# OlegArenz/gmmvi

Measured on AMD Instinct MI355X. Metric: samples_components_per_sec, higher is better.
Workload: dtype f32; 1 GPU; ns: stm target D=20, K=100 components (100/GPU), 100 samples/component, N=10000 samples/iter, SAMTRON (Stein, fixed K, reuse ratio 0, KL trust regions, improvement-based stepsizes); K=100, D=20, N=10000, parallelism=component-shard x1

## Files before the change

### gmmvi_amd/_lib.py

```python
import ctypes as C
import os

_HERE = os.path.dirname(os.path.abspath(__file__))
LIB_PATH = os.environ.get("GMMVI_HIP_LIB", os.path.join(_HERE, "libgmmvi_hip.so"))

GAUSS, STUDENT_T = 0, 1
SELF_NORMALIZED, OWN_SAMPLES_ONLY, EXPLICIT_ESTIMATE = 1, 2, 4
MAX_DIM = 64
MORE_REGISTER_MAX_DIM = 21
MORE_BLOCKED_MIN_DIM, MORE_BLOCKED_MAX_DIM = 64, 128
MAX_DIM_BLOCKED = 512
MAX_DIM_DIAG = 131072
BLOCKED_ABOVE_DEFAULT = 50


_blocked_above = None


def _atoi(text):
    import re
    m = re.match(r"\s*([+-]?\d+)", text)
    return int(m.group(1)) if m else 0


# ... 34 lines not shown
    "gmmvi_gather_rows": (_i, [_p, _p, _p, _i, _i, _p]),
    "gmmvi_exp_f32": (_i, [_p, _p, _p, _sz]),
    "gmmvi_logaddexp_f32": (_i, [_p, _p, _p, _f, _p, _f, _sz]),
    "gmmvi_segment_lse_f32": (_i, [_p, _i, _p, _p, _p, _i, _p, _sz, _i]),
    "gmmvi_copy_2d_f32": (_i, [_p, _p, _sz, _p, _sz, _i, _i]),
    "gmmvi_copy_batch": (_i, [_p, _i, C.POINTER(_p), C.POINTER(_p), C.POINTER(_sz)]),
    "gmmvi_normalize_logw": (_i, [_p, _p, _i, _p]),
    "gmmvi_add_heuristic_argmax": (_i, [_p, _p, _p, _i, C.c_double, _p]),
    "gmmvi_unpack_gathered": (_i, [_p, _p, _i, _sz, _i, C.POINTER(_sz), C.POINTER(_p)]),
    "gmmvi_fill_strided_f32": (_i, [_p, _p, _sz, _sz, _f]),
    "gmmvi_remove_column_f32": (_i, [_p, _p, _i, _sz, _i, _i]),
    "gmmvi_add_scalar_i32": (_i, [_p, _p, _p, C.c_int32, _sz]),
    "gmmvi_event_create": (_i, [_p, C.POINTER(_p)]),
    "gmmvi_event_destroy": (_i, [_p, _p]),
    "gmmvi_event_record": (_i, [_p, _p]),
    "gmmvi_event_synchronize": (_i, [_p, _p]),
    "gmmvi_host_alloc": (_i, [_p, _sz, C.POINTER(_p)]),
    "gmmvi_vmm_reserve": (_i, [_p, _sz, C.POINTER(_p), C.POINTER(_sz)]),
    "gmmvi_vmm_grow": (_i, [_p, _p, _sz, _sz, _sz]),
    "gmmvi_vmm_release": (_i, [_p, _p, _sz, _sz, _sz]),
    "gmmvi_host_free": (_i, [_p, _p]),
    "gmmvi_download_async": (_i, [_p, _p, _p, _sz]),
    "gmmvi_event_elapsed_ms": (_i, [_p, _p, _p, C.POINTER(_f)]),
    "gmmvi_profile_enable": (_i, [_p, _i]),
    "gmmvi_profile_report": (_i, [_p, C.c_char_p, _sz]),
    "gmmvi_packed_stride": (_sz, [_i]),
    "gmmvi_pack_components": (_i, [_p, _i, _f, _i, _i, _p, _p, _p, _p]),
    "gmmvi_cholesky": (_i, [_p, _i, _i, _p, _p, _p]),
    "gmmvi_mixture_eval": (_i, [_p, _i, _f, _i, _i, _p, _p, _p, _i, _p, _p, _p]),
    "gmmvi_mixture_eval_dual": (_i, [_p, _i, _f, _i, _i, _p, _p, _p, _p, _i, _p, _p, _p, _p]),
    "gmmvi_target_planar": (_i, [_p, _i, _p, _i, _p, _f, _p, _i, _p, _p]),
    "gmmvi_target_logreg": (_i, [_p, _i, _i, _p, _f, _f, _p, _i, _p, _p]),
    "gmmvi_target_logreg_mb": (_i, [_p, _i, _i, _p, _i, _i, _u64, _u32, _f, _f, _p, _i, _p, _p]),
    "gmmvi_target_bnn": (_i, [_p, _i, _i, _i, _i, _p, _p, _u64, _u32, _i, _f, _f, _p, _i, _p, _p]),
    "gmmvi_bnn_predict": (_i, [_p, _i, _i, _i, _p, _i, _p, _i, _p]),
    "gmmvi_target_talos": (_i, [_p, _p, _p, _p, _i, _p, _p]),
    "gmmvi_talos_fk": (_i, [_p, _p, _p, _i, _p, _p]),
    "gmmvi_sample_components": (_i, [_p, _i, _i, _p, _p, _p, _i, _u64, _u64, _i, _p, _p, _p]),
    "gmmvi_philox_normals": (_i, [_p, _u64, _u64, _i, _i, _i, _p]),
    "gmmvi_philox_uniforms": (_i, [_p, _u64, _u64, _i, _i, _p]),
    "gmmvi_stein": (_i, [_p, _i, _i, _p, _p, _i, _p, _p, _p, _p, _p, _i, _i, _p, _p]),
    "gmmvi_more": (_i, [_p, _i, _i, _p, _p, _p, _i, _p, _p, _p, _p, _p, _i, _i, _p, _p, _p]),
    "gmmvi_more_blocked": (_i, [_p, _i, _i, _p, _p, _p, _i, _p, _p, _p, _p, _p, _i, _i, _p, _p, _p]),
    "gmmvi_update_components_kl": (_i, [_p, _i, _i, _p, _p, _p, _p, _p, _f, _f, _p, _p, _p, _p, _p, _p, _p]),
    "gmmvi_update_components_kl_reference": (_i, [_p, _i, _i, _p, _p, _p, _p, _p, _f, _f, _p, _p, _p, _p, _p, _p]),
    "gmmvi_update_components_direct": (_i, [_p, _i, _i, _p, _p, _p, _p, _p, _f, _p, _p, _p]),
    "gmmvi_update_components_iblr": (_i, [_p, _i, _i, _p, _p, _p, _p, _p, _f, _p, _p, _p]),
    "gmmvi_expected_log_ratios": (_i, [_p, _i, _i, _p, _p, _p, _p, _f, _p, _i, _p, _p, _p]),
    "gmmvi_update_weights_kl": (_i, [_p, _i, _p, _p, _p, _f, _p]),
    "gmmvi_update_weights_direct": (_i, [_p, _i, _p, _p, _p, _f]),
    "gmmvi_component_stepsize_improvement": (_i, [_p, _i, _p, _p, _p, _f, _f, _f, _f]),
    "gmmvi_weight_stepsize_improvement": (_i, [_p, _i, _p, _p, _p, _f, _f, _f, _f]),
    "gmmvi_train_iter_samtron": (_i, [_p, _p]),
    "gmmvi_sharded_scratch_floats": (_sz, [_i, _i, _i]),
    "gmmvi_train_iter_sharded_phase": (_i, [_p, _p, _i]),
    "gmmvi_comm_unique_id": (_i, [C.c_char_p]),
    "gmmvi_comm_init": (_i, [_p, C.c_char_p, _i, _i]),
    "gmmvi_comm_destroy": (_i, [_p]),
    "gmmvi_allgather_f32": (_i, [_p, _p, _p, _sz]),
    "gmmvi_allreduce_f32": (_i, [_p, _p, _sz, _i]),
    "gmmvi_combine_partials": (_i, [_p, _i, _i, _i, _p, _p, _p, _p]),
    "gmmvi_diag_packed_stride": (_sz, [_i]),
    "gmmvi_diag_pack": (_i, [_p, _i, _i, _p, _p, _p]),
    "gmmvi_diag_mixture_eval": (_i, [_p, _i, _i, _p, _p, _p, _p, _i, _p, _p, _p, _p]),
    "gmmvi_diag_sample": (_i, [_p, _i, _i, _p, _p, _p, _i, _u64, _u64, _i, _p, _p, _p]),
    "gmmvi_diag_stein": (_i, [_p, _i, _i, _p, _p, _i, _p, _p, _p, _p, _p, _i, _i, _p, _p]),
    "gmmvi_diag_embed": (_i, [_p, _i, _i, _p, _p]),
    "gmmvi_diag_extract": (_i, [_p, _i, _i, _p, _p]),
    "gmmvi_reciprocal_f32": (_i, [_p, _p, _sz, _p]),
    "gmmvi_update_components_diag_kl": (_i, [_p, _i, _i, _p, _p, _p, _p, _p, _f, _f, _p, _p, _p, _p, _p, _p]),
    "gmmvi_update_components_diag_iblr": (_i, [_p, _i, _i, _p, _p, _p, _p, _p, _f, _p, _p, _p]),
    "gmmvi_mmd_scratch_doubles": (_sz, [_i, _i]),
    "gmmvi_mmd_pair_sum": (_i, [_p, _p, _i, _p, _i, _i, _p, _p, _p]),
}

EXPORTED_SYMBOLS = tuple(_PROTOS.keys())


def load():
    global _lib
    if _lib is not None:
        return _lib
    if not os.path.exists(LIB_PATH):
        raise GmmviError(
            f"{LIB_PATH} not found: build it with `make -C gmmvi_amd/csrc` (or __graft_entry__.build()). "
            "There is no CPU fallback for the gmmvi hot path.")
    lib = C.CDLL(LIB_PATH, mode=C.RTLD_GLOBAL)
    for name, (res, args) in _PROTOS.items():
        fn = getattr(lib, name)
        fn.restype = res
        fn.argtypes = args
    _lib = lib
    return lib


def device_count():
    return int(load().gmmvi_device_count())


def check(ctx_handle, rc):
    if rc != 0:
        msg = load().gmmvi_last_error(ctx_handle)
        raise GmmviError(f"libgmmvi_hip error {rc}: {msg.decode() if msg else '?'}")
```

### gmmvi_amd/csrc/api.hip

```cpp
#include "common.h"
#include <cstring>
#include "blocked.h"

std::string g_gmmvi_global_err;

int gmmvi_ws_reserve(gmmvi_ctx* ctx, size_t nbytes) {
    ++ctx->ws_epoch;
    if (nbytes <= ctx->ws_bytes) return GMMVI_OK;
    GMMVI_HIP_CHECK(ctx, hipStreamSynchronize(ctx->stream));
    if (ctx->ws) GMMVI_HIP_CHECK(ctx, hipFree(ctx->ws));
    ctx->ws = nullptr;
    ctx->ws_bytes = 0;
    size_t want = nbytes + nbytes / 2;
    GMMVI_HIP_CHECK(ctx, hipMalloc(&ctx->ws, want));
    ctx->ws_bytes = want;
    return GMMVI_OK;
}

extern "C" {

int gmmvi_device_count(void) {
    int n = 0;
    if (hipGetDeviceCount(&n) != hipSuccess) return 0;
    return n;
}

int gmmvi_ctx_create(gmmvi_ctx** out, int device) {
    if (!out) return gmmvi_fail(nullptr, GMMVI_ERR_ARG, "gmmvi_ctx_create: out is NULL");
    *out = nullptr;
    int n = 0;
    hipError_t e = hipGetDeviceCount(&n);
    if (e != hipSuccess || n == 0)
        return gmmvi_fail(nullptr, GMMVI_ERR_HIP, std::string("no HIP device: ") + hipGetErrorString(e));
    if (device < 0 || device >= n) return gmmvi_fail(nullptr, GMMVI_ERR_ARG, "device index out of range");
    gmmvi_ctx* ctx = new gmmvi_ctx();
    ctx->device = device;
    e = hipSetDevice(device);
    if (e == hipSuccess) e = hipStreamCreateWithFlags(&ctx->stream, hipStreamNonBlocking);
    if (e != hipSuccess) {
        g_gmmvi_global_err = std::string("gmmvi_ctx_create: ") + hipGetErrorString(e);
        delete ctx;
        return GMMVI_ERR_HIP;
    }
    hipDeviceProp_t prop;
    if (hipGetDeviceProperties(&prop, device) == hipSuccess) ctx->num_cus = prop.multiProcessorCount;
    *out = ctx;
    return GMMVI_OK;
}

void gmmvi_ctx_destroy(gmmvi_ctx* ctx) {
    if (!ctx) return;
    gmmvi_comm_destroy(ctx);
    if (ctx->stream) {
        (void)hipStreamSynchronize(ctx->stream);
        (void)hipStreamDestroy(ctx->stream);
    }
    if (ctx->ws) (void)hipFree(ctx->ws);
    if (ctx->arena) (void)hipFree(ctx->arena);
    if (ctx->bimg) (void)hipFree(ctx->bimg);
    if (ctx->up_ring) {
        for (int i = 0; i < gmmvi_ctx::UP_SLOTS; ++i) (void)hipEventDestroy(ctx->up_event[i]);
        (void)hipHostFree(ctx->up_ring);
    }
    if (ctx->defer_ws) (void)hipFree(ctx->defer_ws);
    delete ctx;
}

const char* gmmvi_last_error(gmmvi_ctx* ctx) { return ctx ? ctx->err.c_str() : g_gmmvi_global_err.c_str(); }

int gmmvi_sync(gmmvi_ctx* ctx) {
    GMMVI_HIP_CHECK(ctx, hipStreamSynchronize(ctx->stream));
    return GMMVI_OK;
}

int gmmvi_malloc(gmmvi_ctx* ctx, size_t nbytes, void** out_dev) {
    GMMVI_ARG_CHECK(ctx, out_dev != nullptr);
    *out_dev = nullptr;
    if (nbytes == 0) nbytes = 4;
    GMMVI_HIP_CHECK(ctx, hipSetDevice(ctx->device));
    GMMVI_HIP_CHECK(ctx, hipMalloc(out_dev, nbytes));
    return GMMVI_OK;
}

int gmmvi_free(gmmvi_ctx* ctx, void* dev) {
    if (!dev) return GMMVI_OK;
    GMMVI_HIP_CHECK(ctx, hipFree(dev));
    return GMMVI_OK;
}

int gmmvi_upload(gmmvi_ctx* ctx, void* dst_dev, const void* src_host, size_t nbytes) {
    if (nbytes == 0) return GMMVI_OK;
    GMMVI_ARG_CHECK(ctx, dst_dev && src_host);
    if (nbytes <= gmmvi_ctx::UP_SLOT_BYTES) {
        if (ctx->up_ring == nullptr) {
            GMMVI_HIP_CHECK(ctx, hipHostMalloc((void**)&ctx->up_ring, gmmvi_ctx::UP_SLOTS * gmmvi_ctx::UP_SLOT_BYTES, hipHostMallocDefault));
            for (int i = 0; i < gmmvi_ctx::UP_SLOTS; ++i)
                GMMVI_HIP_CHECK(ctx, hipEventCreateWithFlags(&ctx->up_event[i], hipEventDisableTiming));
        }
        const int slot = ctx->up_next;
        ctx->up_next = (slot + 1) % gmmvi_ctx::UP_SLOTS;
        if (ctx->up_used[slot]) GMMVI_HIP_CHECK(ctx, hipEventSynchronize(ctx->up_event[slot]));
        unsigned char* stage = ctx->up_ring + (size_t)slot * gmmvi_ctx::UP_SLOT_BYTES;
        memcpy(stage, src_host, nbytes);
        GMMVI_HIP_CHECK(ctx, hipMemcpyAsync(dst_dev, stage, nbytes, hipMemcpyHostToDevice, ctx->stream));
        GMMVI_HIP_CHECK(ctx, hipEventRecord(ctx->up_event[slot], ctx->stream));
        ctx->up_used[slot] = true;
        return GMMVI_OK;
    }
    GMMVI_HIP_CHECK(ctx, hipMemcpyAsync(dst_dev, src_host, nbytes, hipMemcpyHostToDevice, ctx->stream));
    GMMVI_HIP_CHECK(ctx, hipStreamSynchronize(ctx->stream));
    return GMMVI_OK;
}

int gmmvi_download(gmmvi_ctx* ctx, void* dst_host, const void* src_dev, size_t nbytes) {
    if (nbytes == 0) return GMMVI_OK;
    GMMVI_ARG_CHECK(ctx, dst_host && src_dev);
    GMMVI_HIP_CHECK(ctx, hipMemcpyAsync(dst_host, src_dev, nbytes, hipMemcpyDeviceToHost, ctx->stream));
// ... 458 lines not shown
```

### gmmvi_amd/csrc/combine.h

```cpp
#pragma once
#include "common.h"

template <int R>
__device__ __forceinline__ float combine_log_values_n(const float* __restrict__ parts, int N, int n) {
    float v[R];
#pragma unroll
    for (int r = 0; r < R; ++r) v[r] = parts[(size_t)r * N + n];
    float m = -3.0e38f;
#pragma unroll
    for (int r = 0; r < R; ++r) m = fmaxf(m, v[r]);
    float s = 0.f;
#pragma unroll
    for (int r = 0; r < R; ++r) s += __expf(v[r] - m);
    return m + __logf(s);
}

__device__ __forceinline__ float combine_log_values(const float* __restrict__ parts, int R, int N, int n) {
    switch (R) {
        case 2: return combine_log_values_n<2>(parts, N, n);
        case 3: return combine_log_values_n<3>(parts, N, n);
        case 4: return combine_log_values_n<4>(parts, N, n);
        case 5: return combine_log_values_n<5>(parts, N, n);
        case 6: return combine_log_values_n<6>(parts, N, n);
        case 7: return combine_log_values_n<7>(parts, N, n);
// ... 39 lines not shown
            for (int r = 0; r < R; ++r) g = fmaf(__expf(lv[r] - lp), gv[r], g);
        } else {
            for (int r = 0; r < Rr; ++r)
                g = fmaf(__expf(j.lp_parts[(size_t)r * ps + n] - lp), j.grad_parts[(size_t)r * gs + (size_t)n * j.D + i], g);
        }
        j.grad_out[(size_t)n * j.D + i] = g;
    }
}

__device__ __forceinline__ void combine_element(const CombineJob& j, long e) {
    switch (j.R) {
        case 2: combine_element_n<2>(j, e); break;
        case 3: combine_element_n<3>(j, e); break;
        case 4: combine_element_n<4>(j, e); break;
        case 5: combine_element_n<5>(j, e); break;
        case 6: combine_element_n<6>(j, e); break;
        case 7: combine_element_n<7>(j, e); break;
        case 8: combine_element_n<8>(j, e); break;
        case 10: combine_element_n<10>(j, e); break;
        case 12: combine_element_n<12>(j, e); break;
        case 16: combine_element_n<16>(j, e); break;
        default: combine_element_n<0>(j, e); break;
    }
}

template <int R>
__device__ __forceinline__ void combine_carried_n(const CombineJob& j) {
    const bool with_grad = j.grad_out != nullptr && j.grad_parts != nullptr;
    const long elems = (long)j.N * (with_grad ? j.D : 1);
    const long stride = (long)j.blocks * blockDim.x;
    for (long e = (long)((int)blockIdx.x - j.first_block) * blockDim.x + threadIdx.x; e < elems; e += stride)
        combine_element_n<R>(j, e);
}

__device__ __forceinline__ bool combine_carried(const CombineJob& j) {
    if (j.blocks == 0 || (int)blockIdx.x < j.first_block) return false;
    if (blockIdx.y == 0 && blockIdx.z == 0) {
        switch (j.R) {
            case 2: combine_carried_n<2>(j); break;
            case 3: combine_carried_n<3>(j); break;
            case 4: combine_carried_n<4>(j); break;
            case 5: combine_carried_n<5>(j); break;
            case 6: combine_carried_n<6>(j); break;
            case 7: combine_carried_n<7>(j); break;
            case 8: combine_carried_n<8>(j); break;
            case 10: combine_carried_n<10>(j); break;
            case 12: combine_carried_n<12>(j); break;
            case 16: combine_carried_n<16>(j); break;
            default: combine_carried_n<0>(j); break;
        }
    }
    return true;
}
```

### gmmvi_amd/csrc/comm.hip

```cpp
#include "common.h"
#include "combine.h"
#include <rccl/rccl.h>

#define GMMVI_NCCL_CHECK(ctx, call)                                                                        \
    do {                                                                                                   \
        ncclResult_t r__ = (call);                                                                         \
        if (r__ != ncclSuccess)                                                                            \
            return gmmvi_fail(ctx, GMMVI_ERR_RCCL, std::string(#call) + ": " + ncclGetErrorString(r__));   \
    } while (0)

__global__ __launch_bounds__(256) void combine_partials_kernel(CombineJob j) {
    combine_element(j, (long)blockIdx.x * blockDim.x + threadIdx.x);
}

int gmmvi_combine_partials_internal(gmmvi_ctx* ctx, int R, int N, int D, const float* lp_parts_dev,
                                    const float* grad_parts_dev, float* lp_out_dev, float* grad_out_dev,
                                    const float* lp2_parts_dev, float* lp2_out_dev, long part_stride) {
    GMMVI_ARG_CHECK(ctx, R >= 1 && N >= 0 && D >= 1 && lp_parts_dev && part_stride >= 0);
    if (N == 0) return GMMVI_OK;
    CombineJob j;
    j.R = R; j.N = N; j.D = D; j.part_stride = part_stride;
    j.lp_parts = lp_parts_dev; j.grad_parts = grad_parts_dev; j.lp2_parts = lp2_parts_dev;
    j.lp_out = lp_out_dev; j.grad_out = grad_out_dev; j.lp2_out = lp2_parts_dev ? lp2_out_dev : nullptr;
    const long elems = (long)N * ((grad_out_dev && grad_parts_dev) ? D : 1);
    hipLaunchKernelGGL(combine_partials_kernel, dim3((unsigned)((elems + 255) / 256)), dim3(256), 0, ctx->stream, j);
    GMMVI_LAUNCH_CHECK(ctx);
    return GMMVI_OK;
}

int gmmvi_defer_reserve(gmmvi_ctx* ctx, size_t nbytes) {
    if (ctx->pending.R > 0) return gmmvi_fail(ctx, GMMVI_ERR_ARG, "gmmvi_defer_reserve: a merge is still pending");
    if (nbytes <= ctx->defer_bytes) return GMMVI_OK;
    GMMVI_HIP_CHECK(ctx, hipStreamSynchronize(ctx->stream));
    if (ctx->defer_ws) GMMVI_HIP_CHECK(ctx, hipFree(ctx->defer_ws));
    ctx->defer_ws = nullptr;
    ctx->defer_bytes = 0;
    const size_t want = nbytes + nbytes / 2;
    GMMVI_HIP_CHECK(ctx, hipMalloc(&ctx->defer_ws, want));
    ctx->defer_bytes = want;
    return GMMVI_OK;
}

int gmmvi_flush_pending_combine(gmmvi_ctx* ctx) {
    if (ctx->pending.R == 0) return GMMVI_OK;
    const CombineJob j = ctx->pending;
    ctx->pending = CombineJob();
    GMMVI_PROF(ctx, "mixture_combine");
    return gmmvi_combine_partials_internal(ctx, j.R, j.N, j.D, j.lp_parts, j.grad_parts, j.lp_out, j.grad_out, j.lp2_parts,
                                           j.lp2_out);
}

CombineJob gmmvi_take_pending_combine(gmmvi_ctx* ctx, int threads, int first_block, bool light) {
    CombineJob j = ctx->pending;
    ctx->pending = CombineJob();
    if (j.R == 0) return j;
    const long elems = (long)j.N * ((j.grad_out && j.grad_parts) ? j.D : 1);
    long blocks;
    if (light) {
        blocks = (elems + 2L * threads - 1) / (2L * threads);
        if (blocks > 16L * ctx->num_cus) blocks = 16L * ctx->num_cus;
    } else {
        blocks = ctx->num_cus - first_block % ctx->num_cus;
        if (blocks < ctx->num_cus / 4) blocks += ctx->num_cus;
        const long useful = (elems + threads - 1) / threads;
        if (blocks > useful) blocks = useful;
    }
    if (blocks < 1) blocks = 1;
    j.first_block = first_block;
    j.blocks = (int)blocks;
    return j;
}

extern "C" {

int gmmvi_comm_unique_id(char* out_id_128) {
    if (!out_id_128) return gmmvi_fail(nullptr, GMMVI_ERR_ARG, "gmmvi_comm_unique_id: NULL buffer");
    static_assert(sizeof(ncclUniqueId) == 128, "ncclUniqueId is expected to be 128 bytes");
    ncclUniqueId id;
    ncclResult_t r = ncclGetUniqueId(&id);
    if (r != ncclSuccess) return gmmvi_fail(nullptr, GMMVI_ERR_RCCL, std::string("ncclGetUniqueId: ") + ncclGetErrorString(r));
    memcpy(out_id_128, &id, 128);
    return GMMVI_OK;
}

int gmmvi_comm_init(gmmvi_ctx* ctx, const char* unique_id_128, int n_ranks, int rank) {
    GMMVI_ARG_CHECK(ctx, unique_id_128 && n_ranks >= 1 && rank >= 0 && rank < n_ranks);
    if (ctx->comm) return gmmvi_fail(ctx, GMMVI_ERR_STATE, "communicator already initialised");
    ncclUniqueId id;
    memcpy(&id, unique_id_128, 128);
    GMMVI_HIP_CHECK(ctx, hipSetDevice(ctx->device));
    ncclComm_t comm;
    GMMVI_NCCL_CHECK(ctx, ncclCommInitRank(&comm, n_ranks, id, rank));
    ctx->comm = (void*)comm;
    ctx->n_ranks = n_ranks;
    ctx->rank = rank;
    return GMMVI_OK;
}

int gmmvi_comm_destroy(gmmvi_ctx* ctx) {
    if (ctx && ctx->comm) {
        (void)hipStreamSynchronize(ctx->stream);
        ncclCommDestroy((ncclComm_t)ctx->comm);
        ctx->comm = nullptr;
        ctx->n_ranks = 1;
        ctx->rank = 0;
    }
    return GMMVI_OK;
}

int gmmvi_allgather_f32(gmmvi_ctx* ctx, const float* send_dev, float* recv_dev, size_t count_per_rank) {
    GMMVI_ARG_CHECK(ctx, send_dev && recv_dev);
    if (ctx->n_ranks == 1 || !ctx->comm) {
        if (send_dev != recv_dev)
            GMMVI_HIP_CHECK(ctx, hipMemcpyAsync(recv_dev, send_dev, count_per_rank * sizeof(float),
                                                hipMemcpyDeviceToDevice, ctx->stream));
        return GMMVI_OK;
    }
    GMMVI_NCCL_CHECK(ctx, ncclAllGather(send_dev, recv_dev, count_per_rank, ncclFloat, (ncclComm_t)ctx->comm,
                                        ctx->stream));
    return GMMVI_OK;
}

int gmmvi_allreduce_f32(gmmvi_ctx* ctx, float* buf_dev, size_t count, int op) {
    GMMVI_ARG_CHECK(ctx, buf_dev && (op == 0 || op == 1));
    if (ctx->n_ranks == 1 || !ctx->comm) return GMMVI_OK;
    GMMVI_NCCL_CHECK(ctx, ncclAllReduce(buf_dev, buf_dev, count, ncclFloat, op == 0 ? ncclSum : ncclMax,
// ... 12 lines not shown
```

### gmmvi_amd/csrc/common.h

```cpp
#pragma once
#include <hip/hip_runtime.h>
#include <cstdio>
#include <cstring>
#include <cstdint>
#include <string>
#include <vector>
#include "../../include/gmmvi_hip.h"
#include "iter_prep.h"

struct CombineJob {
    int R = 0, N = 0, D = 0;
    long part_stride = 0;
    int first_block = 0, blocks = 0;
    const float* lp_parts = nullptr;
    const float* grad_parts = nullptr;
    const float* lp2_parts = nullptr;
    float* lp_out = nullptr;
    float* grad_out = nullptr;
    float* lp2_out = nullptr;
};

struct SampleJob {
    int K = 0, D = 0, uniform_count = 0;
    const float* means = nullptr; const float* chols = nullptr; const int32_t* offsets = nullptr;
    unsigned long long seed = 0, first_index = 0;
    float* X = nullptr; int32_t* mapping = nullptr; int32_t mapping_base = 0;
};

struct Riders {
    int first_block = 0;
    int prep_blocks = 0;
    int sample_blocks = 0;
    PrepArgs prep;
    SampleJob sample;
};

inline size_t riders_lds_bytes(const Riders& r) {
    return r.sample_blocks > 0 ? ((size_t)r.sample.D * r.sample.D + r.sample.D + 256 * (size_t)(r.sample.D | 1)) * sizeof(float) : 0;
}

struct gmmvi_ctx {
    int device = 0;
    hipStream_t stream = nullptr;
    std::string err;
    void* ws = nullptr;
    size_t ws_bytes = 0;
    uint64_t ws_epoch = 0;
    void* arena = nullptr;
    size_t arena_bytes = 0;
    static constexpr int UP_SLOTS = 64;
    static constexpr size_t UP_SLOT_BYTES = 64 * 1024;
    unsigned char* up_ring = nullptr;
    hipEvent_t up_event[UP_SLOTS] = {};
    bool up_used[UP_SLOTS] = {};
    int up_next = 0;
    void* bimg = nullptr;
    size_t bimg_bytes = 0;
    bool defer_combine = false;
    CombineJob pending;
    Riders riders;
    void* defer_ws = nullptr;
    size_t defer_bytes = 0;
    void* comm = nullptr;
    int n_ranks = 1, rank = 0;
    int num_cus = 256;
    unsigned func_attr_done = 0;
    bool prof = false;
    const char* prof_tag = nullptr;
    struct ProfRec { const char* name; hipEvent_t start, stop; double units; };
    std::vector<ProfRec> prof_recs;
};

struct GmmviProfScope {
    gmmvi_ctx* ctx; hipEvent_t stop = nullptr;
    GmmviProfScope(gmmvi_ctx* c, const char* name, double units = 0.0) : ctx(c) {
        if (!c->prof) return;
        hipEvent_t start;
        if (hipEventCreate(&start) != hipSuccess || hipEventCreate(&stop) != hipSuccess) { stop = nullptr; return; }
        (void)hipEventRecord(start, c->stream);
        c->prof_recs.push_back({name, start, stop, units});
    }
    ~GmmviProfScope() { if (stop) (void)hipEventRecord(stop, ctx->stream); }
};
#define GMMVI_PROF(ctx, name) GmmviProfScope prof_scope__(ctx, name)
#define GMMVI_PROF_UNITS(ctx, name, units) GmmviProfScope prof_scope__(ctx, name, units)

extern std::string g_gmmvi_global_err;

inline int gmmvi_fail(gmmvi_ctx* ctx, int code, const std::string& msg) {
    if (ctx) ctx->err = msg; else g_gmmvi_global_err = msg;
    return code;
}

#define GMMVI_HIP_CHECK(ctx, call)                                                                    \
    do {                                                                                              \
        hipError_t e__ = (call);                                                                      \
        if (e__ != hipSuccess)                                                                        \
            return gmmvi_fail(ctx, GMMVI_ERR_HIP,                                                     \
                              std::string(#call) + ": " + hipGetErrorString(e__) + " (" + __FILE__ +  \
                                  ":" + std::to_string(__LINE__) + ")");                              \
    } while (0)

#define GMMVI_ARG_CHECK(ctx, cond)                                                                    \
    do {                                                                                              \
        if (!(cond))                                                                                  \
            return gmmvi_fail(ctx, GMMVI_ERR_ARG, std::string("invalid argument: ") + #cond + " (" +  \
                                                      __FILE__ + ":" + std::to_string(__LINE__) + ")"); \
    } while (0)

#define GMMVI_LAUNCH_CHECK(ctx) GMMVI_HIP_CHECK(ctx, hipGetLastError())

int gmmvi_ws_reserve(gmmvi_ctx* ctx, size_t nbytes);
int gmmvi_pack_register_layout(gmmvi_ctx* ctx, int K, int D, const float* means_dev, const float* chols_dev, float* packed_dev);
int gmmvi_sample_components_bounded(gmmvi_ctx* ctx, int K, int D, const float* means_dev, const float* chols_dev,
                                    const int32_t* offsets_dev, int N, int max_per_component, uint64_t seed,
                                    uint64_t first_index, int stream_id, const float* eps_dev, float* X_out_dev,
                                    int32_t* mapping_out_dev);
int gmmvi_sample_components_prep(gmmvi_ctx* ctx, int K, int D, const float* means_dev, const float* chols_dev,
                                 const int32_t* offsets_dev, int N, int max_per_component, uint64_t seed, uint64_t first_index,
                                 float* X_out_dev, int32_t* mapping_out_dev, int32_t mapping_base, const PrepArgs& prep);
int gmmvi_combine_partials_internal(gmmvi_ctx* ctx, int R, int N, int D, const float* lp_parts_dev,
                                    const float* grad_parts_dev, float* lp_out_dev, float* grad_out_dev,
                                    const float* lp2_parts_dev, float* lp2_out_dev, long part_stride = 0);
int gmmvi_defer_reserve(gmmvi_ctx* ctx, size_t nbytes);
int gmmvi_flush_pending_combine(gmmvi_ctx* ctx);
CombineJob gmmvi_take_pending_combine(gmmvi_ctx* ctx, int threads, int first_block, bool light = false);
Riders gmmvi_take_pending_riders(gmmvi_ctx* ctx, int first_block, int threads, bool prep_only = false);
int gmmvi_flush_pending_riders(gmmvi_ctx* ctx);
struct SteinSlab;
int gmmvi_stein_partials(gmmvi_ctx* ctx, int K, int D, const float* packed_dev, const float* X_dev, int N, const float* ld_dev,
                         const float* qgrad_dev, const float* bg_dev, const float* tgrad_dev, int flags, SteinSlab* slab);
int gmmvi_stein_finalize_slab(gmmvi_ctx* ctx, int K, int D, const SteinSlab& slab, int N, int flags, const float* packed_dev,
                              float* H_neg_out_dev, float* g_neg_out_dev);
int gmmvi_update_components_kl_from_slab(gmmvi_ctx* ctx, int K, int D, const SteinSlab& slab, int N, int stein_flags,
                                         const float* packed_old_dev, float* H_neg_dev, float* g_neg_dev, float* means_dev,
                                         float* chols_dev, const float* stepsizes_dev, float temperature, float l2_init,
                                         float* last_eta_dev, float* l2_dev, float* num_received_updates_dev,
                                         int32_t* success_out_dev, float* packed_out_dev);
int gmmvi_update_weights_internal(gmmvi_ctx* ctx, int mode, int K, float* logw_dev, const float* E_dev,
                                  const float* stepsize_dev, float beta, float* kl_eta_out_dev, float* exp_out_dev);

inline int gmmvi_padded_dim(int D) {
    static const int dps[] = {2, 4, 8, 10, 12, 16, 20, 24, 32, 40, 50, 64};
    for (int dp : dps) if (D <= dp) return dp;
    return -1;
}

#define GMMVI_DISPATCH_DP(DPVAL, ...)                  \
    switch (DPVAL) {                                   \
        case 2:  { constexpr int DP = 2;  __VA_ARGS__; } break;  \
        case 4:  { constexpr int DP = 4;  __VA_ARGS__; } break;  \
        case 8:  { constexpr int DP = 8;  __VA_ARGS__; } break;  \
        case 10: { constexpr int DP = 10; __VA_ARGS__; } break;  \
        case 12: { constexpr int DP = 12; __VA_ARGS__; } break;  \
        case 16: { constexpr int DP = 16; __VA_ARGS__; } break;  \
        case 20: { constexpr int DP = 20; __VA_ARGS__; } break;  \
        case 24: { constexpr int DP = 24; __VA_ARGS__; } break;  \
        case 32: { constexpr int DP = 32; __VA_ARGS__; } break;  \
        case 40: { constexpr int DP = 40; __VA_ARGS__; } break;  \
        case 50: { constexpr int DP = 50; __VA_ARGS__; } break;  \
        case 64: { constexpr int DP = 64; __VA_ARGS__; } break;  \
        default: return gmmvi_fail(ctx, GMMVI_ERR_ARG, "unsupported dimension (D must be <= 64)"); \
    }

#ifndef GMMVI_MFMA_DENSITY_FROM_DP
#define GMMVI_MFMA_DENSITY_FROM_DP 32
#endif

template <int DP>
struct Pack {
    static constexpr int T = DP * (DP - 1) / 2;
    static constexpr int MU = 0;
    static constexpr int RD = DP;
    static constexpr int LROW = 2 * DP;
    static constexpr int LCOL = 2 * DP + T;
    static constexpr int CONST = 2 * DP + 2 * T;
    static constexpr bool FRAGS = DP >= GMMVI_MFMA_DENSITY_FROM_DP;
    static constexpr int MT = (DP + 15) / 16;
    static constexpr int KS = (DP + 3) / 4;
    __host__ __device__ static constexpr int nf(int mt) { return 4 * mt + 4 < KS ? 4 * mt + 4 : KS; }
    __host__ __device__ static constexpr int nbk(int mt) { return KS - 4 * mt > 0 ? KS - 4 * mt : 0; }
    __host__ __device__ static constexpr int fwd_base(int mt) { int a = 0; for (int m = 0; m < mt; ++m) a += nf(m); return a; }
    __host__ __device__ static constexpr int bwd_base(int mt) { int a = 0; for (int m = 0; m < mt; ++m) a += nbk(m); return a; }
    __host__ __device__ static constexpr int fwd_index(int mt, int s) { return fwd_base(mt) + s; }
// ... 74 lines not shown
```

### gmmvi_amd/csrc/density.hip

```cpp
#include "common.h"
#include "combine.h"
#include "riders.h"
#include "subst.h"
#include "subst_phased.h"
#include "subst_pk.h"
#include "blocked.h"
#include <cmath>
#include <cstdlib>

template <int DP>
__global__ __launch_bounds__(64) void pack_kernel(int family, float nu, int K, int D, const float* __restrict__ means,
                                                  const float* __restrict__ chols, float* __restrict__ packed,
                                                  float* __restrict__ inv_chols) {
    using P = Pack<DP>;
    const int k = blockIdx.x;
    const int t = threadIdx.x;
    const float* L = chols + (size_t)k * D * D;
    float* out = packed + (size_t)k * P::STRIDE;
    for (int i = t; i < DP; i += 64) {
        out[P::MU + i] = i < D ? means[(size_t)k * D + i] : 0.f;
        out[P::RD + i] = i < D ? 1.f / L[i * D + i] : 1.f;
    }
    for (int e = t; e < DP * DP; e += 64) {
        int i = e / DP, j = e % DP;
// ... 22 lines not shown
#pragma unroll
        for (int i = 0; i < DP; ++i) {
            float sacc = (i == t) ? 1.f : 0.f;
            if (i < D && t < D) {
                for (int j = 0; j < i; ++j) sacc -= L[i * D + j] * x[j];
                x[i] = sacc / L[i * D + i];
            } else {
                x[i] = 0.f;
            }
        }
        if (t < DP) {
#pragma unroll
            for (int i = 0; i < DP; ++i) Li[i * DP + t] = (i >= t) ? x[i] : 0.f;
        }
    }
    __syncthreads();
    if (P::FRAGS) gmmvi_write_inverse_fragments(out, DP, D, Li, DP, t, 64);
    if (inv_chols != nullptr) {
        float* inv = inv_chols + (size_t)k * D * D;
        for (int e = t; e < D * D; e += 64) inv[e] = Li[(e / D) * DP + (e % D)];
    }
}

__global__ __launch_bounds__(64) void cholesky_kernel(int D, const float* __restrict__ covs, float* __restrict__ chols,
                                                      int32_t* __restrict__ ok) {
    extern __shared__ float sm[];
    const int k = blockIdx.x, t = threadIdx.x;
    const int ld = D + 1;
    for (int e = t; e < D * D; e += 64) sm[(e / D) * ld + (e % D)] = covs[(size_t)k * D * D + e];
    __syncthreads();
    bool good = true;
    for (int j = 0; j < D; ++j) {
        float s = 0.f;
        if (t >= j && t < D) {
            s = sm[t * ld + j];
            for (int c = 0; c < j; ++c) s -= sm[t * ld + c] * sm[j * ld + c];
        }
        float p = __shfl(s, j);
        if (!(p > 0.f)) { good = false; break; }
        float d = sqrtf(p);
        __syncthreads();
        if (t == j) sm[t * ld + j] = d;
        else if (t > j && t < D) sm[t * ld + j] = s / d;
        __syncthreads();
    }
    for (int e = t; e < D * D; e += 64) {
        int i = e / D, j = e % D;
        float v = (j <= i) ? sm[i * ld + j] : 0.f;
        chols[(size_t)k * D * D + e] = good ? v : __builtin_nanf("");
    }
    if (t == 0 && ok) ok[k] = good ? 1 : 0;
}

typedef float me_f32x4 __attribute__((ext_vector_type(4)));
#define ME_LDS_BARRIER()                                       \
    do {                                                       \
        asm volatile("s_waitcnt lgkmcnt(0)" ::: "memory");     \
        __builtin_amdgcn_s_barrier();                          \
        asm volatile("" ::: "memory");                         \
    } while (0)
__host__ __device__ constexpr int me_rem_rows(int dp) { return (dp % 16 != 0 && dp % 16 <= 4 && dp > 16) ? dp % 16 : 0; }
template <int R>
__device__ __forceinline__ float me_row_bcast(float v) {
    return __int_as_float(__builtin_amdgcn_update_dpp(0, __float_as_int(v), 0x150 + R, 0xf, 0xf, false));
}
template <int N, int I = 0, class F>
__device__ __forceinline__ void me_static_rows(F&& f) {
    if constexpr (I < N) {
        f(std::integral_constant<int, I>{});
        me_static_rows<N, I + 1>(f);
    }
}
#ifndef GMMVI_ME_THREADS
#define GMMVI_ME_THREADS 1024
#define GMMVI_ME_MINW 1
#endif
#ifndef GMMVI_ME_WIDE_DP
#define GMMVI_ME_WIDE_DP 40
#endif
#ifdef GMMVI_ME_STAMPS
__device__ long long g_me_wg[2 * 8192];
__device__ unsigned long long g_me_hw[8192];
extern "C" int gmmvi_debug_wg_times(long long* out, int n) {
    return hipMemcpyFromSymbol(out, HIP_SYMBOL(g_me_wg), sizeof(long long) * (size_t)n) == hipSuccess ? 0 : -1;
}
extern "C" int gmmvi_debug_wg_hw(unsigned long long* out, int n) {
    return hipMemcpyFromSymbol(out, HIP_SYMBOL(g_me_hw), sizeof(unsigned long long) * (size_t)n) == hipSuccess ? 0 : -1;
}
__device__ long long g_me_ph[1024 * 16 * 16];
extern "C" int gmmvi_debug_wg_phases(long long* out, int n) {
    return hipMemcpyFromSymbol(out, HIP_SYMBOL(g_me_ph), sizeof(long long) * (size_t)n) == hipSuccess ? 0 : -1;
}
#endif
template <int DP, int FAMILY, bool GRAD>
__global__ __launch_bounds__(DP >= GMMVI_ME_WIDE_DP ? 512 : GMMVI_ME_THREADS, GMMVI_ME_MINW) void mixture_eval_kernel(float nu, int K_total, int D, const float* __restrict__ packed,
                                                            const float* __restrict__ logw, const float* __restrict__ X,
                                                            int N, float* __restrict__ ld_out, float* __restrict__ lp_out,
                                                            float* __restrict__ grad_out, const float* __restrict__ logw2,
                                                            float* __restrict__ lp2_out, CombineJob carried, Riders riders) {
    using PK = Pack<DP>;
    extern __shared__ __align__(16) float sm[];
    if (combine_carried(carried) || riders_carried<DP>(riders, sm)) return;
    const int kchunk = (K_total + gridDim.y - 1) / gridDim.y;
    const int k_lo = blockIdx.y * kchunk;
    const int K = min(K_total, k_lo + kchunk);
    if (gridDim.y > 1) {
        if (lp_out) lp_out += (size_t)blockIdx.y * N;
        if (lp2_out) lp2_out += (size_t)blockIdx.y * N;
        if (GRAD && grad_out) grad_out += (size_t)blockIdx.y * N * D;
    }
    const int lane = threadIdx.x & 63;
    const int wave = __builtin_amdgcn_readfirstlane(threadIdx.x >> 6);
    const int nwaves = blockDim.x >> 6;
    const int n0 = blockIdx.x * 64;
    const int n_here = min(64, N - n0);
    const int n = n0 + lane;
    const bool valid = lane < n_here;
    float* sm_merge = sm;
#ifdef GMMVI_ME_STAMPS
    if (threadIdx.x == 0) {
        g_me_wg[2 * (blockIdx.y * gridDim.x + blockIdx.x)] = wall_clock64();
        unsigned hw, xcc;
        asm volatile("s_getreg_b32 %0, hwreg(HW_REG_HW_ID)" : "=s"(hw));
        asm volatile("s_getreg_b32 %0, hwreg(HW_REG_XCC_ID)" : "=s"(xcc));
        g_me_hw[blockIdx.y * gridDim.x + blockIdx.x] = ((unsigned long long)xcc << 32) | hw;
    }
    unsigned long long stamp[16];
    int nstamp = 0, nbackward = 0;
    const long long wc0 = wall_clock64();
#define ME_STAMP() do { asm volatile("s_waitcnt lgkmcnt(0)" ::: "memory"); if (nstamp < 16) stamp[nstamp++] = __builtin_amdgcn_s_memtime(); } while (0)
    ME_STAMP();
#else
#define ME_STAMP()
#endif

    const int ldx = D | 1;
    float x[DP];
    if (DP % 4 == 0 && D == DP && (reinterpret_cast<uintptr_t>(X) & 15) == 0) {
        const float4* xrow = reinterpret_cast<const float4*>(X + (size_t)min(n, N - 1) * D);
#pragma unroll
        for (int q4 = 0; q4 < DP / 4; ++q4) {
            const float4 v4 = xrow[q4];
            x[4 * q4] = v4.x; x[4 * q4 + 1] = v4.y; x[4 * q4 + 2] = v4.z; x[4 * q4 + 3] = v4.w;
        }
        if (!valid) {
#pragma unroll
            for (int i = 0; i < DP; ++i) x[i] = 0.f;
        }
    } else if (DP % 2 == 0 && D == DP && (reinterpret_cast<uintptr_t>(X) & 7) == 0) {
        const float2* xrow = reinterpret_cast<const float2*>(X + (size_t)min(n, N - 1) * D);
#pragma unroll
        for (int q2 = 0; q2 < DP / 2; ++q2) {
            const float2 v2 = xrow[q2];
            x[2 * q2] = v2.x; x[2 * q2 + 1] = v2.y;
        }
        if (!valid) {
#pragma unroll
            for (int i = 0; i < DP; ++i) x[i] = 0.f;
        }
    } else {
        for (int e = threadIdx.x; e < n_here * D; e += blockDim.x) sm_merge[(e / D) * ldx + (e % D)] = X[(size_t)n0 * D + e];
        __syncthreads();
#pragma unroll
        for (int i = 0; i < DP; ++i) x[i] = (valid && i < D) ? sm_merge[lane * ldx + i] : 0.f;
        __syncthreads();
    }

    float m = -3.0e38f, s = 0.f;
    float m2 = -3.0e38f, s2 = 0.f;
    const bool dual = logw2 != nullptr;
    float acc[GRAD ? DP : 1];
    if (GRAD) {
#pragma unroll
        for (int i = 0; i < DP; ++i) acc[i] = 0.f;
    }
    const float nud = nu + (float)D;
    ME_STAMP();

    for (int k = k_lo + wave; k < K; k += nwaves) {
        ME_STAMP();
        const sp_block_ptr blk = sp_block(packed + (size_t)k * PK::STRIDE);
        const float lw = ((sp_const_f32)(uintptr_t)logw)[k];
        const float lw2 = dual ? ((sp_const_f32)(uintptr_t)logw2)[k] : 0.f;
        float z[DP], vrd[DP], q, cst;
        float pc[2][32];
        SpPass<DP>::forward(blk, x, z, vrd, q, cst, pc);
        sp_block_ptr blkb = blk;
        asm volatile("" : "+s"(blkb));
        if constexpr (GRAD) SpPass<DP>::backward_prefetch(blkb, pc);
        float ld, coef;
        if (FAMILY == GMMVI_GAUSS) {
            ld = fmaf(-0.5f, q, cst);
            coef = -1.f;
        } else {
            ld = cst - 0.5f * nud * log1pf(q / nu);
            coef = -nud / (nu + q);
        }
        const float a = ld + lw;
        const float mn = fmaxf(m, a);
        const float sc = __expf(m - mn);
        const float e = __expf(a - mn);
        s = fmaf(s, sc, e);
        m = mn;
        if (dual) {
            const float a2 = ld + lw2;
            const float mn2 = fmaxf(m2, a2);
            s2 = fmaf(s2, __expf(m2 - mn2), __expf(a2 - mn2));
            m2 = mn2;
        }
        if constexpr (GRAD) {
            SpPass<DP>::backward(blkb, z, vrd, pc);
            const float ec = e * coef;
#pragma unroll
            for (int i = 0; i < DP; ++i) acc[i] = fmaf(acc[i], sc, ec * z[i]);
            sp_pin<DP>(acc);
        }
        if (ld_out != nullptr && valid) ld_out[(size_t)k * N + n] = ld;
    }
    ME_STAMP();
    if (lp_out == nullptr && !GRAD) return;

    constexpr int NQ = (DP + 3) / 4;
    float* sm_m = sm_merge;
    float* sm_s = sm_merge + nwaves * 64;
    me_f32x4* sm_acc = reinterpret_cast<me_f32x4*>(sm_merge + 2 * nwaves * 64);
    float* outt = sm_merge + 2 * nwaves * 64 + (GRAD ? (size_t)nwaves * NQ * 256 : 0);
    float* sm_m2 = outt + (GRAD ? 64 * ldx : 0);
    float* sm_s2 = sm_m2 + nwaves * 64;
    sm_m[wave * 64 + lane] = m;
    if (dual) sm_m2[wave * 64 + lane] = m2;
    ME_LDS_BARRIER();
    ME_STAMP();
    float M = -3.0e38f, M2 = -3.0e38f;
    for (int w = 0; w < nwaves; ++w) M = fmaxf(M, sm_m[w * 64 + lane]);
    const float f = __expf(m - M);
    sm_s[wave * 64 + lane] = s * f;
    if (dual) {
        for (int w = 0; w < nwaves; ++w) M2 = fmaxf(M2, sm_m2[w * 64 + lane]);
        sm_s2[wave * 64 + lane] = s2 * __expf(m2 - M2);
    }
    if (GRAD) {
#pragma unroll
        for (int q4 = 0; q4 < NQ; ++q4) {
            me_f32x4 v4;
#pragma unroll
            for (int c = 0; c < 4; ++c) v4[c] = 4 * q4 + c < DP ? acc[4 * q4 + c] * f : 0.f;
            sm_acc[(wave * NQ + q4) * 64 + lane] = v4;
        }
    }
    ME_STAMP();
    ME_LDS_BARRIER();
    ME_STAMP();
    float S = 0.f;
    for (int w = 0; w < nwaves; ++w) S += sm_s[w * 64 + lane];
    if (wave == 0 && valid && lp_out != nullptr) lp_out[n] = M + __logf(S);
    if (dual && wave == (nwaves > 1 ? 1 : 0) && valid && lp2_out != nullptr) {
        float S2 = 0.f;
        for (int w = 0; w < nwaves; ++w) S2 += sm_s2[w * 64 + lane];
        lp2_out[n] = M2 + __logf(S2);
    }
    if (GRAD && grad_out != nullptr) {
        const float inv = 1.f / S;
        for (int q4 = wave; q4 < NQ; q4 += nwaves) {
            me_f32x4 g4 = {0.f, 0.f, 0.f, 0.f};
            for (int w = 0; w < nwaves; ++w) g4 += sm_acc[(w * NQ + q4) * 64 + lane];
#pragma unroll
            for (int c = 0; c < 4; ++c)
                if (4 * q4 + c < D) outt[lane * ldx + 4 * q4 + c] = g4[c] * inv;
        }
        ME_STAMP();
        ME_LDS_BARRIER();
        ME_STAMP();
        for (int e = threadIdx.x; e < n_here * D; e += blockDim.x)
            grad_out[(size_t)n0 * D + e] = outt[(e / D) * ldx + (e % D)];
    }
#ifdef GMMVI_ME_STAMPS
    ME_STAMP();
    if (threadIdx.x == 0) g_me_wg[2 * (blockIdx.y * gridDim.x + blockIdx.x) + 1] = wall_clock64();
    if (GRAD && logw2 && blockIdx.x == 60 && blockIdx.y == 1 && threadIdx.x == 64 * 3 && (g_me_wg[2 * 8192 - 1]++ & 15) == 12) {
        const long long wc1 = wall_clock64();
        printf("me stamps (shader cycles; kernel %lld x 10 ns by the 100 MHz clock):", wc1 - wc0);
        for (int i = 1; i < nstamp; ++i) printf(" %llu", stamp[i] - stamp[i - 1]);
        printf("  total %llu, backward passes %d\n", stamp[nstamp - 1] - stamp[0], nbackward);
    }
#endif
}

template <int DP, int FAMILY, bool GRAD>
__global__ __launch_bounds__(DP > 24 ? 512 : 1024) void mixture_eval_pk_kernel(float nu, int K_total, int D, const float* __restrict__ packed,
                                                               const float* __restrict__ logw, const float* __restrict__ X, int N,
                                                               float* __restrict__ ld_out, float* __restrict__ lp_out,
                                                               float* __restrict__ grad_out, const float* __restrict__ logw2,
                                                               float* __restrict__ lp2_out, CombineJob carried, Riders riders) {
    using PK = Pack<DP>;
    static_assert(DP % 2 == 0, "padded dimensions are even");
    constexpr int NP2 = DP / 2;
    extern __shared__ __align__(16) float sm[];
    if (combine_carried(carried) || riders_carried<DP>(riders, sm)) return;
    const int kchunk = (K_total + gridDim.y - 1) / gridDim.y;
    const int k_lo = blockIdx.y * kchunk;
    const int K = min(K_total, k_lo + kchunk);
    if (gridDim.y > 1) {
        if (lp_out) lp_out += (size_t)blockIdx.y * N;
        if (lp2_out) lp2_out += (size_t)blockIdx.y * N;
        if (GRAD && grad_out) grad_out += (size_t)blockIdx.y * N * D;
    }
    const int lane = threadIdx.x & 63;
    const int wave = __builtin_amdgcn_readfirstlane(threadIdx.x >> 6);
    const int nwaves = blockDim.x >> 6;
    const int n0 = blockIdx.x * 128;
    const int nA = n0 + lane, nB = n0 + 64 + lane;
    const bool validA = nA < N, validB = nB < N;
#ifdef GMMVI_ME_STAMPS
    const int wg_lin = blockIdx.y * gridDim.x + blockIdx.x;
    if (threadIdx.x == 0 && wg_lin < 8192) {
        g_me_wg[2 * wg_lin] = wall_clock64();
        unsigned hw, xcc;
        asm volatile("s_getreg_b32 %0, hwreg(HW_REG_HW_ID)" : "=s"(hw));
        asm volatile("s_getreg_b32 %0, hwreg(HW_REG_XCC_ID)" : "=s"(xcc));
        g_me_hw[wg_lin] = ((unsigned long long)xcc << 32) | hw;
    }
    int pk_ns = 0;
#define PK_STAMP() do { if (lane == 0 && wg_lin < 1024 && pk_ns < 16) g_me_ph[(wg_lin * 16 + wave) * 16 + pk_ns] = wall_clock64(); ++pk_ns; } while (0)
    PK_STAMP();
#else
#define PK_STAMP()
#endif

    me_f32x4* xs4 = reinterpret_cast<me_f32x4*>(sm);
    {
        const int n_here = min(128, N - n0);
        for (int e = threadIdx.x; e < 128 * DP; e += blockDim.x) {
            const int sl = e / DP, i = e - sl * DP;
            const float v = (sl < n_here && i < D) ? X[(size_t)(n0 + sl) * D + i] : 0.f;
            sm[(((i >> 1) * 64) + (sl & 63)) * 4 + ((i & 1) << 1) + (sl >> 6)] = v;
        }
    }
    float* sm_merge = sm + NP2 * 64 * 4;
    ME_LDS_BARRIER();
    PK_STAMP();

    pk_f32x2 mld = pk_splat(-3.0e38f), s = pk_splat(0.f), mld2 = pk_splat(-3.0e38f), s2 = pk_splat(0.f);
    const bool dual = logw2 != nullptr;
    pk_f32x2 acc[GRAD ? DP : 1];
    if (GRAD) {
#pragma unroll
// ... 69 lines not shown
    sm_max[wave * 64 + lane] = mld;
    if (dual) sm_max[(nwaves + wave) * 64 + lane] = mld2;
    ME_LDS_BARRIER();
    PK_STAMP();
    pk_f32x2 M = mld, M2 = mld2;
    for (int wv = 0; wv < nwaves; ++wv) {
        const pk_f32x2 o = sm_max[wv * 64 + lane];
        M = pk_f32x2{fmaxf(M.x, o.x), fmaxf(M.y, o.y)};
    }
    if (dual) {
        for (int wv = 0; wv < nwaves; ++wv) {
            const pk_f32x2 o = sm_max[(nwaves + wv) * 64 + lane];
            M2 = pk_f32x2{fmaxf(M2.x, o.x), fmaxf(M2.y, o.y)};
        }
        s2 = s2 * pk_f32x2{__expf(mld2.x - M2.x), __expf(mld2.y - M2.y)};
    }
    {
        const pk_f32x2 f = pk_f32x2{__expf(mld.x - M.x), __expf(mld.y - M.y)};
        s = s * f;
        if (GRAD) {
#pragma unroll
            for (int i = 0; i < DP; ++i) acc[i] = acc[i] * f;
        }
    }
#pragma unroll
    for (int half = 8; half >= 1; half >>= 1) {
        if (half < nwaves) {
            const bool writer = wave >= half && wave < 2 * half;
            const bool reader = wave < half && wave + half < nwaves;
            const int slot_w = half == half0 ? wave - half : wave;
            const int slot_r = half == half0 ? wave : wave + half;
            if (writer) {
                pk_f32x2* dst = slots + (size_t)slot_w * NV * 64 + lane;
                dst[0] = s;
                dst[64] = s2;
                if (GRAD) {
#pragma unroll
                    for (int i = 0; i < DP; ++i) dst[(2 + i) * 64] = acc[i];
                }
            }
            ME_LDS_BARRIER();
            if (reader) {
                const pk_f32x2* src = slots + (size_t)slot_r * NV * 64 + lane;
                s = s + src[0];
                s2 = s2 + src[64];
                if (GRAD) {
#pragma unroll
                    for (int i = 0; i < DP; ++i) acc[i] = acc[i] + src[(2 + i) * 64];
                }
            }
        }
    }
    PK_STAMP();
    if (wave != 0) return;
    if (lp_out != nullptr) {
        if (validA) lp_out[nA] = M.x + __logf(s.x);
        if (validB) lp_out[nB] = M.y + __logf(s.y);
    }
    if (dual && lp2_out != nullptr) {
        if (validA) lp2_out[nA] = M2.x + __logf(s2.x);
        if (validB) lp2_out[nB] = M2.y + __logf(s2.y);
    }
    if (GRAD && grad_out != nullptr) {
        const pk_f32x2 inv = pk_f32x2{1.f / s.x, 1.f / s.y};
#pragma unroll
        for (int i = 0; i < DP; ++i) acc[i] = acc[i] * inv;
        if (D == DP && DP % 4 == 0 && (reinterpret_cast<uintptr_t>(grad_out) & 15) == 0) {
#pragma unroll
            for (int q4 = 0; q4 < DP / 4; ++q4) {
                if (validA) reinterpret_cast<float4*>(grad_out + (size_t)nA * D)[q4] =
                    make_float4(acc[4 * q4].x, acc[4 * q4 + 1].x, acc[4 * q4 + 2].x, acc[4 * q4 + 3].x);
                if (validB) reinterpret_cast<float4*>(grad_out + (size_t)nB * D)[q4] =
                    make_float4(acc[4 * q4].y, acc[4 * q4 + 1].y, acc[4 * q4 + 2].y, acc[4 * q4 + 3].y);
            }
        } else {
#pragma unroll
            for (int i = 0; i < DP; ++i) {
                if (i < D) {
                    if (validA) grad_out[(size_t)nA * D + i] = acc[i].x;
                    if (validB) grad_out[(size_t)nB * D + i] = acc[i].y;
                }
            }
        }
    }
    PK_STAMP();
#ifdef GMMVI_ME_STAMPS
    if (threadIdx.x == 0 && wg_lin < 8192) g_me_wg[2 * wg_lin + 1] = wall_clock64();
#endif
#undef PK_STAMP
}


#define ME_WAVE_LDS_SYNC()                                     \
    do {                                                       \
        asm volatile("s_waitcnt lgkmcnt(0)" ::: "memory");     \
        __builtin_amdgcn_wave_barrier();                       \
    } while (0)

template <int DP, int FAMILY, bool GRAD, int NTS>
__global__ __launch_bounds__(512) void mixture_eval_mfma_kernel(float nu, int K_total, int D, const float* __restrict__ packed,
                                                                const float* __restrict__ logw, const float* __restrict__ X,
                                                                int N, float* __restrict__ ld_out, float* __restrict__ lp_out,
                                                                float* __restrict__ grad_out, const float* __restrict__ logw2,
                                                                float* __restrict__ lp2_out, CombineJob carried, Riders riders) {
    using PK = Pack<DP>;
    constexpr int MT = PK::MT, KS = PK::KS;
    extern __shared__ __align__(16) float sm[];
    if (combine_carried(carried) || riders_carried<DP>(riders, sm)) return;
    constexpr int TS = 16 * NTS;
    constexpr int KSP = ((KS + 3) / 4) * 4;
    constexpr int ZW = 4 * KSP + 4;
    const int kchunk = (K_total + gridDim.y - 1) / gridDim.y;
    const int k_lo = blockIdx.y * kchunk;
    const int K = min(K_total, k_lo + kchunk);
    if (gridDim.y > 1) {
        if (lp_out) lp_out += (size_t)blockIdx.y * N;
        if (lp2_out) lp2_out += (size_t)blockIdx.y * N;
        if (GRAD && grad_out) grad_out += (size_t)blockIdx.y * N * D;
    }
    const int lane = threadIdx.x & 63;
    const int wave = __builtin_amdgcn_readfirstlane(threadIdx.x >> 6);
    const int nwaves = blockDim.x >> 6;
    const int g = lane >> 4, n16 = lane & 15;
    const int n0 = blockIdx.x * TS;
    const int n_here = min(TS, N - n0);
    float* Zw = sm + (size_t)wave * (GRAD ? NTS * 16 * ZW : 0);
    float* sm_merge = sm + (size_t)nwaves * (GRAD ? NTS * 16 * ZW : 0);

    const int ldx = D | 1;
    for (int e = threadIdx.x; e < n_here * D; e += blockDim.x) sm_merge[(e / D) * ldx + (e % D)] = X[(size_t)n0 * D + e];
    __syncthreads();
    float xb[NTS][KS];
#pragma unroll
    for (int t = 0; t < NTS; ++t)
#pragma unroll
        for (int s = 0; s < KS; ++s)
            xb[t][s] = (16 * t + n16 < n_here && 4 * s + g < D) ? sm_merge[(16 * t + n16) * ldx + 4 * s + g] : 0.f;
    __syncthreads();
// ... 649 lines not shown
    GMMVI_LAUNCH_CHECK(ctx);
    if (defer) {
        CombineJob& j = ctx->pending;
        j.R = ky; j.N = N; j.D = D;
        j.lp_parts = lp_k; j.grad_parts = grad_k; j.lp2_parts = lp2_k;
        j.lp_out = lp; j.grad_out = grad; j.lp2_out = lp2_k ? lp2 : nullptr;
    } else if (ky > 1 && want_merge) {
        GMMVI_PROF(ctx, "mixture_combine");
        int rc = gmmvi_combine_partials_internal(ctx, ky, N, D, lp_k, grad_k, lp, grad, lp2_k, lp2);
        if (rc != GMMVI_OK) return rc;
    }
    return GMMVI_OK;
}

template <int DP>
static int launch_mixture_eval_pk(gmmvi_ctx* ctx, int family, float nu, int K, int D, const float* packed,
                                  const float* logw, const float* X, int N, float* ld, float* lp, float* grad,
                                  const float* logw2, float* lp2) {
    const bool want_grad = grad != nullptr;
    const bool want_merge = want_grad || lp != nullptr;
    static const int env_ky = getenv("GMMVI_ME_PK_KY") ? atoi(getenv("GMMVI_ME_PK_KY")) : 0;
    static const int env_nw = getenv("GMMVI_ME_PK_NW") ? atoi(getenv("GMMVI_ME_PK_NW")) : 0;
    const int tiles = (N + 127) / 128;
    const long cus = ctx->num_cus;
    auto chunks_for = [&](long slots) {
        long c = slots / tiles;
        if (c > (K + 3) / 4) c = (K + 3) / 4;
        return (int)(c < 1 ? 1 : c);
    };
    auto fill = [&](int c, long slots) {
        const long wgs = (long)tiles * c, rounds = (wgs + slots - 1) / slots;
        return (double)wgs / (double)(rounds * slots);
    };
    const int ky16 = chunks_for(cus), ky8 = chunks_for(2 * cus);
    bool wide = fill(ky16, cus) + 0.05 >= fill(ky8, 2 * cus);
    int ky = wide ? ky16 : ky8;
    if (DP > 24) ky = want_grad ? ky16 : ky8;
    if (env_ky > 0) ky = env_ky;
    if (ky > K) ky = K;
    if (ky < 1) ky = 1;
    const int kchunk = (K + ky - 1) / ky;
    ky = (K + kchunk - 1) / kchunk;
    int nw = wide && DP <= 24 ? 16 : 8;
    if (env_nw > 0) nw = env_nw;
    if (DP > 24 && nw > 8) nw = 8;
    if (nw > kchunk) nw = kchunk;
    if (nw > 16) nw = 16;
    const int nv = (want_grad ? DP : 0) + 2;
    size_t shmem = (size_t)(DP / 2) * 64 * 16 + (size_t)nw * 64 * 8 * (logw2 ? 2 : 1) +
                   (want_merge ? (size_t)(nw > 8 ? 8 : 4) * nv * 64 * 8 : 0);
    float* lp_k = lp;
    float* grad_k = grad;
    float* lp2_k = lp2;
    const bool defer = ctx->defer_combine && ky > 1 && want_merge;
    if (defer) {
        int rc = gmmvi_flush_pending_combine(ctx);
        if (rc != GMMVI_OK) return rc;
    }
    if (ky > 1 && want_merge) {
        size_t need = ((size_t)ky * N * (logw2 ? 2 : 1) + (want_grad ? (size_t)ky * N * D : 0)) * sizeof(float);
        int rc = defer ? gmmvi_defer_reserve(ctx, need) : gmmvi_ws_reserve(ctx, need);
        if (rc != GMMVI_OK) return rc;
        lp_k = (float*)(defer ? ctx->defer_ws : ctx->ws);
        lp2_k = logw2 ? lp_k + (size_t)ky * N : nullptr;
        grad_k = want_grad ? lp_k + (size_t)ky * N * (logw2 ? 2 : 1) : nullptr;
    }
    const Riders riders = gmmvi_take_pending_riders(ctx, tiles, nw * 64);
    const CombineJob carried = gmmvi_take_pending_combine(ctx, nw * 64, tiles + riders.prep_blocks + riders.sample_blocks);
    if (riders_lds_bytes(riders) > shmem) shmem = riders_lds_bytes(riders);
    dim3 grid(tiles + carried.blocks + riders.prep_blocks + riders.sample_blocks, ky), block(nw * 64);
    {
        GMMVI_PROF_UNITS(ctx, sweep_prof_name(ctx, want_grad, logw2 != nullptr), (double)N * K);
#define GMMVI_LAUNCH_MEPK(FAM, G)                                                                                      \
    do {                                                                                                               \
        if (shmem > 64 * 1024)                                                                                         \
            GMMVI_HIP_CHECK(ctx, hipFuncSetAttribute((const void*)mixture_eval_pk_kernel<DP, FAM, G>,               \
                                                     hipFuncAttributeMaxDynamicSharedMemorySize, (int)shmem));         \
        hipLaunchKernelGGL((mixture_eval_pk_kernel<DP, FAM, G>), grid, block, shmem, ctx->stream, nu, K, D, packed, \
                           logw, X, N, ld, lp_k, grad_k, logw2, lp2_k, carried, riders);                                         \
    } while (0)
        if constexpr (DP <= 40) {
            if (family == GMMVI_GAUSS) {
                if (want_grad) GMMVI_LAUNCH_MEPK(GMMVI_GAUSS, true); else GMMVI_LAUNCH_MEPK(GMMVI_GAUSS, false);
            } else {
                if (want_grad) GMMVI_LAUNCH_MEPK(GMMVI_STUDENT_T, true); else GMMVI_LAUNCH_MEPK(GMMVI_STUDENT_T, false);
            }
        } else {
            if (want_grad) return gmmvi_fail(ctx, GMMVI_ERR_ARG, "mixture_eval_pk: no gradient instance for this dimension");
            if (family == GMMVI_GAUSS) GMMVI_LAUNCH_MEPK(GMMVI_GAUSS, false); else GMMVI_LAUNCH_MEPK(GMMVI_STUDENT_T, false);
        }
#undef GMMVI_LAUNCH_MEPK
    }
    GMMVI_LAUNCH_CHECK(ctx);
    if (defer) {
        CombineJob& j = ctx->pending;
        j.R = ky; j.N = N; j.D = D;
        j.lp_parts = lp_k; j.grad_parts = grad_k; j.lp2_parts = lp2_k;
        j.lp_out = lp; j.grad_out = grad; j.lp2_out = lp2_k ? lp2 : nullptr;
    } else if (ky > 1 && want_merge) {
        GMMVI_PROF(ctx, "mixture_combine");
        int rc = gmmvi_combine_partials_internal(ctx, ky, N, D, lp_k, grad_k, lp, grad, lp2_k, lp2);
        if (rc != GMMVI_OK) return rc;
    }
    return GMMVI_OK;
}

template <int DP>
static int launch_mixture_eval(gmmvi_ctx* ctx, int family, float nu, int K, int D, const float* packed,
                               const float* logw, const float* X, int N, float* ld, float* lp, float* grad,
                               const float* logw2 = nullptr, float* lp2 = nullptr) {
    using PK = Pack<DP>;
    {
        static const int env_pk = getenv("GMMVI_ME_PK") ? atoi(getenv("GMMVI_ME_PK")) : -1;
        static const long env_pk_min = getenv("GMMVI_ME_PK_MIN") ? atol(getenv("GMMVI_ME_PK_MIN")) : 4096;
        static const int env_pk_wide = getenv("GMMVI_ME_PK_WIDE") ? atoi(getenv("GMMVI_ME_PK_WIDE")) : 1;
        const long passes = (long)((N + 127) / 128) * K;
        const bool shape_ok = !PK::FRAGS || (env_pk_wide && (grad == nullptr || DP <= 40));
        if constexpr (DP <= 50) {
            if (shape_ok && env_pk != 0 && (env_pk == 1 || passes >= env_pk_min))
                return launch_mixture_eval_pk<DP>(ctx, family, nu, K, D, packed, logw, X, N, ld, lp, grad, logw2, lp2);
        }
    }
    if constexpr (PK::FRAGS) {
        static const int env_ws = getenv("GMMVI_ME_WS") ? atoi(getenv("GMMVI_ME_WS")) : -1;
        const bool ws = env_ws >= 0 ? env_ws != 0 : true;
        if (ws && N >= 2048 && K >= 16) {
            if (grad != nullptr) return launch_mixture_eval_mfma_ws<DP, 2>(ctx, family, nu, K, D, packed, logw, X, N, ld, lp, grad, logw2, lp2);
            if (env_ws == 2) return launch_mixture_eval_mfma_ws<DP, 4>(ctx, family, nu, K, D, packed, logw, X, N, ld, lp, grad, logw2, lp2);
        }
        if constexpr (DP >= 40) {
            if (grad != nullptr) return launch_mixture_eval_mfma<DP, 2>(ctx, family, nu, K, D, packed, logw, X, N, ld, lp, grad, logw2, lp2);
        }
        return launch_mixture_eval_mfma<DP, 4>(ctx, family, nu, K, D, packed, logw, X, N, ld, lp, grad, logw2, lp2);
    } else {
    const bool want_grad = grad != nullptr;
    const bool want_merge = want_grad || lp != nullptr;
    static const int env_nw = getenv("GMMVI_ME_NW") ? atoi(getenv("GMMVI_ME_NW")) : 0;
    static const int env_ky = getenv("GMMVI_ME_KY") ? atoi(getenv("GMMVI_ME_KY")) : 0;
    auto lds_floats = [&](int nw) {
        size_t merge = (size_t)nw * 64 * ((want_grad ? (DP + 3) / 4 * 4 : 0) + 2) + (want_grad ? 64 * (size_t)(D | 1) : 0) +
                       (logw2 ? (size_t)nw * 128 : 0);
        size_t stage = 64 * (size_t)(D | 1);
        return merge > stage ? merge : stage;
    };
    const int tiles = (N + 63) / 64;
    const int nw_max = DP >= GMMVI_ME_WIDE_DP ? 8 : 16;
    int ky = 1, nw = K < nw_max ? K : nw_max;
    if (env_ky > 0) ky = env_ky < K ? env_ky : K;
    else if (K >= 16 && 2L * tiles <= 3L * ctx->num_cus) {
        ky = (int)((2L * ctx->num_cus + tiles / 2) / tiles);
        if (ky > K / 8) ky = K / 8;
        if (ky < 1) ky = 1;
        if (ky > 1) nw = 8;
    }
    const int kchunk = (K + ky - 1) / ky;
    ky = (K + kchunk - 1) / kchunk;
    if (nw > kchunk) nw = kchunk;
    if (env_nw > 0) nw = env_nw < kchunk ? env_nw : kchunk;
    if (nw > nw_max) nw = nw_max;
    while (nw > 1 && lds_floats(nw) * 4 > 96 * 1024) --nw;
    size_t shmem = lds_floats(nw) * 4;
    static const size_t env_shmem_min = getenv("GMMVI_ME_SHMEM_MIN") ? (size_t)atol(getenv("GMMVI_ME_SHMEM_MIN")) : 0;
    if (shmem < env_shmem_min) shmem = env_shmem_min;
    float* lp_k = lp;
    float* grad_k = grad;
    float* lp2_k = lp2;
    const bool defer = ctx->defer_combine && ky > 1 && want_merge;
    if (defer) {
        int rc = gmmvi_flush_pending_combine(ctx);
        if (rc != GMMVI_OK) return rc;
    }
    if (ky > 1 && want_merge) {
        size_t need = ((size_t)ky * N * (logw2 ? 2 : 1) + (want_grad ? (size_t)ky * N * D : 0)) * sizeof(float);
        int rc = defer ? gmmvi_defer_reserve(ctx, need) : gmmvi_ws_reserve(ctx, need);
        if (rc != GMMVI_OK) return rc;
        lp_k = (float*)(defer ? ctx->defer_ws : ctx->ws);
        lp2_k = logw2 ? lp_k + (size_t)ky * N : nullptr;
        grad_k = want_grad ? lp_k + (size_t)ky * N * (logw2 ? 2 : 1) : nullptr;
    }
    const Riders riders = gmmvi_take_pending_riders(ctx, tiles, nw * 64);
    const CombineJob carried = gmmvi_take_pending_combine(ctx, nw * 64, tiles + riders.prep_blocks + riders.sample_blocks);
    if (riders_lds_bytes(riders) > shmem) shmem = riders_lds_bytes(riders);
    dim3 grid(tiles + carried.blocks + riders.prep_blocks + riders.sample_blocks, ky), block(nw * 64);
    {
        GMMVI_PROF_UNITS(ctx, sweep_prof_name(ctx, want_grad, logw2 != nullptr), (double)N * K);
#define GMMVI_LAUNCH_ME(FAM, G)                                                                                     \
    do {                                                                                                            \
        if (shmem > 64 * 1024)                                                                                      \
            GMMVI_HIP_CHECK(ctx, hipFuncSetAttribute((const void*)mixture_eval_kernel<DP, FAM, G>,               \
                                                     hipFuncAttributeMaxDynamicSharedMemorySize, (int)shmem));      \
        hipLaunchKernelGGL((mixture_eval_kernel<DP, FAM, G>), grid, block, shmem, ctx->stream, nu, K, D, packed, \
                           logw, X, N, ld, lp_k, grad_k, logw2, lp2_k, carried, riders);                                      \
    } while (0)
        if (family == GMMVI_GAUSS) {
            if (want_grad) GMMVI_LAUNCH_ME(GMMVI_GAUSS, true); else GMMVI_LAUNCH_ME(GMMVI_GAUSS, false);
        } else {
            if (want_grad) GMMVI_LAUNCH_ME(GMMVI_STUDENT_T, true); else GMMVI_LAUNCH_ME(GMMVI_STUDENT_T, false);
        }
#undef GMMVI_LAUNCH_ME
    }
    GMMVI_LAUNCH_CHECK(ctx);
    if (defer) {
        CombineJob& j = ctx->pending;
        j.R = ky; j.N = N; j.D = D;
        j.lp_parts = lp_k; j.grad_parts = grad_k; j.lp2_parts = lp2_k;
        j.lp_out = lp; j.grad_out = grad; j.lp2_out = lp2_k ? lp2 : nullptr;
    } else if (ky > 1 && want_merge) {
        GMMVI_PROF(ctx, "mixture_combine");
        int rc = gmmvi_combine_partials_internal(ctx, ky, N, D, lp_k, grad_k, lp, grad, lp2_k, lp2);
        if (rc != GMMVI_OK) return rc;
    }
    return GMMVI_OK;
    }
}

int gmmvi_pack_register_layout(gmmvi_ctx* ctx, int K, int D, const float* means_dev, const float* chols_dev, float* packed_dev) {
    GMMVI_ARG_CHECK(ctx, K >= 1 && D >= 1 && D <= GMMVI_MAX_DIM && means_dev && chols_dev && packed_dev);
    int dp = gmmvi_padded_dim(D);
    GMMVI_DISPATCH_DP(dp, hipLaunchKernelGGL((pack_kernel<DP>), dim3(K), dim3(64), 0, ctx->stream, (int)GMMVI_GAUSS, 0.f, K, D,
                                             means_dev, chols_dev, packed_dev, (float*)nullptr));
    GMMVI_LAUNCH_CHECK(ctx);
    return GMMVI_OK;
}

extern "C" {

int gmmvi_pack_components(gmmvi_ctx* ctx, int family, float nu, int K, int D, const float* means_dev,
                          const float* chols_dev, float* packed_dev, float* inv_chols_dev) {
    GMMVI_ARG_CHECK(ctx, K >= 0 && D >= 1 && D <= GMMVI_BLOCKED_MAX_DIM);
    GMMVI_ARG_CHECK(ctx, family == GMMVI_GAUSS || family == GMMVI_STUDENT_T);
    if (K == 0) return GMMVI_OK;
    GMMVI_ARG_CHECK(ctx, means_dev && chols_dev && packed_dev);
    if (gmmvi_is_blocked_dim(D)) return gmmvi_blocked_pack(ctx, family, nu, K, D, means_dev, chols_dev, packed_dev, inv_chols_dev);
    int dp = gmmvi_padded_dim(D);
    GMMVI_PROF(ctx, "pack_components");
    GMMVI_DISPATCH_DP(dp, hipLaunchKernelGGL((pack_kernel<DP>), dim3(K), dim3(64), 0, ctx->stream, family, nu, K, D,
                                             means_dev, chols_dev, packed_dev, inv_chols_dev));
    GMMVI_LAUNCH_CHECK(ctx);
    return GMMVI_OK;
}

int gmmvi_cholesky(gmmvi_ctx* ctx, int K, int D, const float* covs_dev, float* chols_dev, int32_t* ok_dev) {
    GMMVI_ARG_CHECK(ctx, K >= 0 && D >= 1 && D <= GMMVI_BLOCKED_MAX_DIM);
    if (K == 0) return GMMVI_OK;
    GMMVI_ARG_CHECK(ctx, covs_dev && chols_dev);
    if (gmmvi_is_blocked_dim(D)) return gmmvi_blocked_cholesky(ctx, K, D, covs_dev, chols_dev, ok_dev);
    hipLaunchKernelGGL(cholesky_kernel, dim3(K), dim3(64), (size_t)D * (D + 1) * 4, ctx->stream, D, covs_dev,
                       chols_dev, ok_dev);
    GMMVI_LAUNCH_CHECK(ctx);
    return GMMVI_OK;
}

int gmmvi_mixture_eval(gmmvi_ctx* ctx, int family, float nu, int K, int D, const float* packed_dev,
                       const float* logw_dev, const float* X_dev, int N, float* ld_out_dev, float* lp_out_dev,
                       float* grad_out_dev) {
    GMMVI_ARG_CHECK(ctx, K >= 1 && D >= 1 && D <= GMMVI_BLOCKED_MAX_DIM && N >= 0);
    GMMVI_ARG_CHECK(ctx, family == GMMVI_GAUSS || family == GMMVI_STUDENT_T);
    if (N == 0) return GMMVI_OK;
    GMMVI_ARG_CHECK(ctx, packed_dev && logw_dev && X_dev);
    GMMVI_ARG_CHECK(ctx, ld_out_dev || lp_out_dev || grad_out_dev);
    if (gmmvi_is_blocked_dim(D))
        return gmmvi_blocked_mixture_eval(ctx, family, nu, K, D, packed_dev, logw_dev, nullptr, X_dev, N, ld_out_dev, lp_out_dev,
                                          grad_out_dev, nullptr);
    int dp = gmmvi_padded_dim(D);
    GMMVI_DISPATCH_DP(dp, return launch_mixture_eval<DP>(ctx, family, nu, K, D, packed_dev, logw_dev, X_dev, N,
                                                         ld_out_dev, lp_out_dev, grad_out_dev));
// ... 21 lines not shown
```

### gmmvi_amd/csrc/fused.hip

```cpp
#include "common.h"
#include "stepsize_rules.h"
#include "iter_prep.h"
#include "stein_finalize.h"

namespace {
struct Arena {
    float *ld, *lq, *qgrad, *bg, *H, *g, *E;
    int32_t *mapping, *success;
};

}

static int arena_reserve(gmmvi_ctx* ctx, size_t floats) {
    if (floats * sizeof(float) <= ctx->arena_bytes) return GMMVI_OK;
    GMMVI_HIP_CHECK(ctx, hipStreamSynchronize(ctx->stream));
    if (ctx->arena) GMMVI_HIP_CHECK(ctx, hipFree(ctx->arena));
    ctx->arena = nullptr;
    ctx->arena_bytes = 0;
    size_t want = floats * sizeof(float) * 3 / 2;
    GMMVI_HIP_CHECK(ctx, hipMalloc(&ctx->arena, want));
    ctx->arena_bytes = want;
    return GMMVI_OK;
}

#define GMMVI_TRY(call)                \
    do {                               \
        int rc__ = (call);             \
        if (rc__ != GMMVI_OK) return rc__; \
    } while (0)

static int train_iter_samtron_body(gmmvi_ctx* ctx, const gmmvi_samtron_plan* p);

extern "C" int gmmvi_train_iter_samtron(gmmvi_ctx* ctx, const gmmvi_samtron_plan* p) {
    GMMVI_ARG_CHECK(ctx, ctx != nullptr);
    int rc = gmmvi_flush_pending_combine(ctx);
    if (rc == GMMVI_OK) rc = train_iter_samtron_body(ctx, p);
    if (rc != GMMVI_OK) {
        ctx->pending = CombineJob();
        ctx->riders.prep_blocks = ctx->riders.sample_blocks = 0;
        ctx->defer_combine = false;
        ctx->prof_tag = nullptr;
    }
    return rc;
}

static int train_iter_samtron_body(gmmvi_ctx* ctx, const gmmvi_samtron_plan* p) {
    GMMVI_ARG_CHECK(ctx, p != nullptr);
    GMMVI_ARG_CHECK(ctx, (p->target_kind >= 0 && p->target_kind <= 2) || p->target_kind == 4);
    GMMVI_ARG_CHECK(ctx, p->target_kind != 2 || (p->logreg_A && p->logreg_M >= 1 && p->logreg_prior_std > 0.f));
    GMMVI_ARG_CHECK(ctx, p->target_kind != 4 || (p->talos_model && p->talos_context && p->D == 34));
    const int K = p->K, D = p->D, N = p->N;
    GMMVI_ARG_CHECK(ctx, K >= 1 && D >= 1 && D < GMMVI_MAX_DIM && N >= 1);
    GMMVI_ARG_CHECK(ctx, p->means && p->chols && p->logw && p->packed && p->packed_new && p->stepsizes && p->last_eta &&
                             p->l2 && p->num_updates && p->offsets && p->bg_logw && p->db_samples && p->db_tlp &&
                             p->db_tgrad && p->db_mapping && p->reward_next && p->wstate);
    GMMVI_ARG_CHECK(ctx, p->n_old >= 0 && p->max_per_component >= 0 && p->phase >= 0 && p->phase <= 2);
    GMMVI_ARG_CHECK(ctx, p->n_old == 0 || (p->bg_packed != nullptr && p->bg_K >= 1 && p->bg_old != nullptr && p->bg_logw_new != nullptr));
    const int n_old = p->n_old;
    const int Na = n_old + N;
    const size_t KN = (size_t)K * Na, ND = (size_t)Na * D;
    const size_t floats = KN + 4 * (size_t)Na + ND + (size_t)K * D * D + (size_t)K * D + 3 * (size_t)K + Na + 64;
    GMMVI_TRY(arena_reserve(ctx, floats));
    Arena a;
    float* base = (float*)ctx->arena;
    a.ld = base; base += KN;
    a.lq = base; base += Na;
    a.bg = base; base += Na;
    a.qgrad = base; base += ND;
    a.H = base; base += (size_t)K * D * D;
    a.g = base; base += (size_t)K * D;
    a.E = base; base += K;
    a.success = (int32_t*)base; base += K;
    a.mapping = (int32_t*)base; base += Na;
    float* bg_a = base; base += Na;
    float* bg_b = base; base += Na;

    const int phase = p->phase;
    float* x = p->db_samples;
    float* xa = x - (size_t)n_old * D;
    const float* tlp_a = p->db_tlp - n_old;
    const float* tgrad_a = p->db_tgrad - (size_t)n_old * D;
    if (phase != 2) {
    PrepArgs prep_later{};
    bool prep_pending = false;
    {
        PrepArgs q{};
        if (p->db_means && p->db_chols && p->db_packed) {
            q.cdst[0] = (uint32_t*)p->db_means; q.csrc[0] = (const uint32_t*)p->means; q.cwords[0] = (size_t)K * D;
            q.cdst[1] = (uint32_t*)p->db_chols; q.csrc[1] = (const uint32_t*)p->chols; q.cwords[1] = (size_t)K * D * D;
            q.cdst[2] = (uint32_t*)p->db_packed; q.csrc[2] = (const uint32_t*)p->packed;
            q.cwords[2] = (size_t)K * gmmvi_packed_stride(D);
        }
        q.K = K; q.cs_mode = p->component_stepsize_mode; q.stepsizes = p->stepsizes;
        q.reward_prev = p->reward_prev; q.reward_last = p->reward_last;
        q.cs_min = p->cs_min; q.cs_max = p->cs_max; q.cs_inc = p->cs_inc; q.cs_dec = p->cs_dec;
        q.ws_mode = p->weight_stepsize_mode; q.logw = p->logw; q.wstate = p->wstate;
        q.ws_min = p->ws_min; q.ws_max = p->ws_max; q.ws_inc = p->ws_inc; q.ws_dec = p->ws_dec;
        const int max_pc = p->max_per_component > 0 ? p->max_per_component : (N + K - 1) / K;
        if (p->presampled && n_old == 0) {
            prep_later = q;
            prep_pending = true;
        } else {
            GMMVI_TRY(gmmvi_sample_components_prep(ctx, K, D, p->means, p->chols, p->offsets, N, max_pc, p->seed,
                                                   p->first_index, x, p->db_mapping, p->mapping_base, q));
        }
    }
    if (p->bg_packed == nullptr) {
        ctx->defer_combine = true;
        ctx->prof_tag = "sweep_dual";
        int rc_dual = gmmvi_mixture_eval_dual(ctx, GMMVI_GAUSS, 0.f, K, D, p->packed, p->logw, p->bg_logw, x, N, a.ld, a.lq,
                                              a.qgrad, a.bg);
        ctx->defer_combine = false;
        ctx->prof_tag = nullptr;
        GMMVI_TRY(rc_dual);
    } else {
        ctx->prof_tag = "sweep_background";
        int rc_bg = gmmvi_mixture_eval(ctx, GMMVI_GAUSS, 0.f, p->bg_K, D, p->bg_packed, p->bg_logw, x, N, nullptr, bg_a + n_old,
                                       nullptr);
        if (rc_bg == GMMVI_OK)
            rc_bg = gmmvi_mixture_eval(ctx, GMMVI_GAUSS, 0.f, K, D, p->packed, p->bg_logw_new, xa, Na, nullptr, bg_b, nullptr);
        ctx->prof_tag = nullptr;
        GMMVI_TRY(rc_bg);
        GMMVI_HIP_CHECK(ctx, hipMemcpyAsync(bg_a, p->bg_old, (size_t)n_old * sizeof(float), hipMemcpyDeviceToDevice, ctx->stream));
        GMMVI_TRY(gmmvi_logaddexp_f32(ctx, a.bg, bg_a, p->bg_log_share_old, bg_b, p->bg_log_share_new, (size_t)Na));
        ctx->defer_combine = true;
        ctx->prof_tag = "sweep_model";
        int rc_m = gmmvi_mixture_eval(ctx, GMMVI_GAUSS, 0.f, K, D, p->packed, p->logw, xa, Na, a.ld, a.lq, a.qgrad);
        ctx->defer_combine = false;
        ctx->prof_tag = nullptr;
        GMMVI_TRY(rc_m);
    }
    if (prep_pending) {
        ctx->riders.prep = prep_later;
        ctx->riders.prep_blocks = K < 64 ? K : 64;
    }
    if (p->target_kind == 1) {
        GMMVI_TRY(gmmvi_target_planar(ctx, D, p->planar_prior_std, p->planar_goals_count, p->planar_goals,
                                      p->planar_likelihood_std, x, N, p->db_tlp, p->db_tgrad));
    } else if (p->target_kind == 2) {
        GMMVI_TRY(gmmvi_target_logreg(ctx, D, p->logreg_M, p->logreg_A, p->logreg_prior_mean, p->logreg_prior_std, x, N,
                                      p->db_tlp, p->db_tgrad));
    } else if (p->target_kind == 4) {
        GMMVI_TRY(gmmvi_target_talos(ctx, p->talos_model, p->talos_context, x, N, p->db_tlp, p->db_tgrad));
    } else {
        ctx->prof_tag = "sweep_target";
        int rc_t = gmmvi_mixture_eval(ctx, p->target_family, p->target_nu, p->target_K, D, p->target_packed,
                                      p->target_logw, x, N, nullptr, p->db_tlp, p->db_tgrad);
        ctx->prof_tag = nullptr;
        GMMVI_TRY(rc_t);
    }
    GMMVI_TRY(gmmvi_flush_pending_combine(ctx));
    GMMVI_TRY(gmmvi_flush_pending_riders(ctx));
    SteinSlab slab{nullptr, nullptr, 0};
    GMMVI_TRY(gmmvi_stein_partials(ctx, K, D, p->packed, xa, Na, a.ld, a.qgrad, a.bg, tgrad_a, p->stein_flags, &slab));
    GMMVI_TRY(gmmvi_update_components_kl_from_slab(ctx, K, D, slab, Na, p->stein_flags, p->packed, a.H, a.g, p->means, p->chols,
                                                   p->stepsizes, p->temperature, p->l2_init, p->last_eta, p->l2, p->num_updates,
                                                   p->success_out ? p->success_out : a.success, p->packed_new));
    }
    if (phase == 1) return GMMVI_OK;
    ctx->defer_combine = true;
    ctx->prof_tag = "sweep_post";
    int rc_post = gmmvi_mixture_eval(ctx, GMMVI_GAUSS, 0.f, K, D, p->packed_new, p->logw, xa, Na, a.ld, a.lq, nullptr);
    ctx->defer_combine = false;
    ctx->prof_tag = nullptr;
    GMMVI_TRY(rc_post);
    if (p->presample_next && n_old == 0) {
        const int max_pc = p->max_per_component > 0 ? p->max_per_component : (N + K - 1) / K;
        SampleJob& sj = ctx->riders.sample;
        sj.K = K; sj.D = D; sj.uniform_count = (long)K * max_pc == N ? max_pc : 0;
        sj.means = p->means; sj.chols = p->chols; sj.offsets = p->offsets;
        sj.seed = p->seed; sj.first_index = p->first_index + (uint64_t)N;
        sj.X = x + (size_t)N * D; sj.mapping = p->db_mapping + N; sj.mapping_base = p->mapping_base + K;
        ctx->riders.sample_blocks = K * ((max_pc + 255) / 256);
    }
    GMMVI_TRY(gmmvi_expected_log_ratios(ctx, K, Na, a.ld, a.bg, tlp_a, a.lq, p->temperature, p->logw,
                                        (p->stein_flags & GMMVI_SELF_NORMALIZED) ? 1 : 0, a.E, p->reward_next, nullptr));
    GMMVI_TRY(gmmvi_flush_pending_riders(ctx));
    if (K > 1) {
        GMMVI_TRY(gmmvi_update_weights_internal(ctx, p->weight_update_mode == 0 ? 0 : 1, K, p->logw, a.E, p->wstate,
                                                p->temperature, nullptr, p->weight_slot));
    }
    return GMMVI_OK;
}


namespace {
struct ShardArena { float *ld, *lq, *bg, *qgrad, *H, *g, *E; int32_t* success; };
}
extern "C" size_t gmmvi_sharded_scratch_floats(int K, int D, int N) {
    if (K < 1 || D < 1 || N < 1) return 0;
    return (size_t)K * N + 2 * (size_t)N + (size_t)N * D + (size_t)K * D * D + (size_t)K * D + 2 * (size_t)K + 64;
}
static void shard_arena(float* base, int K, int D, int N, ShardArena& a) {
    a.ld = base; base += (size_t)K * N;
    a.lq = base; base += N;
    a.bg = base; base += N;
    a.qgrad = base; base += (size_t)N * D;
    a.H = base; base += (size_t)K * D * D;
    a.g = base; base += (size_t)K * D;
    a.E = base; base += K;
    a.success = (int32_t*)base;
}

static int sharded_phase_body(gmmvi_ctx* ctx, const gmmvi_sharded_plan* p, int phase) {
    const int R = p->n_ranks, K = p->K, D = p->D, N = p->N;
    const int Nl = N / R, Kt = K * R;
    const size_t s1 = (size_t)Nl * (2 * D + 1) + 2 * (size_t)K, s2 = (size_t)N * (D + 2), s3 = (size_t)N;
    float* my1 = p->e1 + (size_t)p->rank * s1;
    float* x_loc = my1;
    float* tlp_loc = my1 + (size_t)Nl * D;
    float* tgrad_loc = tlp_loc + Nl;
    float* E_loc = tgrad_loc + (size_t)Nl * D;
    float* reward_loc = E_loc + K;
    float* my2 = p->e2 + (size_t)p->rank * s2;
    float* my3 = p->e3 + (size_t)p->rank * s3;
    float* logw_loc = p->logw_all + (size_t)p->rank * K;
    ShardArena a;
    shard_arena(p->scratch, K, D, N, a);
    const int max_pc = p->max_per_component > 0 ? p->max_per_component : (Nl + K - 1) / K;
    if (phase == 1) {
        if (!p->presampled)
            GMMVI_TRY(gmmvi_sample_components_bounded(ctx, K, D, p->means, p->chols, p->offsets, Nl, max_pc, p->seed, p->first_index, 0,
                                                      nullptr, x_loc, nullptr));
        if (p->target_kind == 1) {
            GMMVI_TRY(gmmvi_target_planar(ctx, D, p->planar_prior_std, p->planar_goals_count, p->planar_goals,
                                          p->planar_likelihood_std, x_loc, Nl, tlp_loc, tgrad_loc));
        } else if (p->target_kind == 2) {
            GMMVI_TRY(gmmvi_target_logreg(ctx, D, p->logreg_M, p->logreg_A, p->logreg_prior_mean, p->logreg_prior_std, x_loc, Nl,
                                          tlp_loc, tgrad_loc));
// ... 108 lines not shown
```

### gmmvi_amd/csrc/stein.hip

```cpp
#include "common.h"
#include "blocked.h"
#include "wave_reduce.h"
#include "stein_finalize.h"
#include "stein_tile.h"
#include <cstdlib>

typedef float f32x4 __attribute__((ext_vector_type(4)));

__device__ __forceinline__ float wave_max(float v) { return gmmvi_wave_max(v); }

template <int DP>
__global__ __launch_bounds__(1024) void stein_finalize_kernel(int D, int R, int N, int flags, const float* __restrict__ part,
                                                             const float* __restrict__ part_m, float* __restrict__ H_neg,
                                                             float* __restrict__ g_neg, const float* __restrict__ packed) {
    extern __shared__ float fin_lds[];
    stein_finalize_component<DP>(fin_lds, blockIdx.x, D, R, N, flags, part, part_m, H_neg, g_neg, packed);
}

template <int DP>
static int launch_stein_finalize(gmmvi_ctx* ctx, int K, int D, int R, int N, int flags, const float* part,
                                 const float* part_m, float* H_neg, float* g_neg, const float* packed) {
    const size_t shmem = stein_finalize_lds_floats(DP, D, R) * sizeof(float);
    static size_t attr = 64 * 1024;
    if (shmem > attr) {
        GMMVI_HIP_CHECK(ctx, hipFuncSetAttribute((const void*)stein_finalize_kernel<DP>,
                                                 hipFuncAttributeMaxDynamicSharedMemorySize, (int)shmem));
        attr = shmem;
    }
    const int threads = Pack<DP>::FRAGS ? 1024 : 256;
    GMMVI_PROF(ctx, "stein_finalize");
    hipLaunchKernelGGL(stein_finalize_kernel<DP>, dim3(K), dim3(threads), shmem, ctx->stream, D, R, N, flags, part, part_m, H_neg,
                       g_neg, packed);
    GMMVI_LAUNCH_CHECK(ctx);
    return GMMVI_OK;
}

template <int DP, int VW>
__device__ __forceinline__ void sm_load_row(const float* __restrict__ row, int D, float (&v)[DP]) {
#pragma unroll
    for (int f = 0; f < DP; f += VW) {
        if (VW > 1 || f < SteinTile<DP>::PREV + 1 || f < D) {
            if constexpr (VW == 4) {
                const float4 t = *reinterpret_cast<const float4*>(row + f);
                v[f] = t.x; v[f + 1] = t.y; v[f + 2] = t.z; v[f + 3] = t.w;
            } else if constexpr (VW == 2) {
                const float2 t = *reinterpret_cast<const float2*>(row + f);
                v[f] = t.x; v[f + 1] = t.y;
            } else {
                v[f] = row[f];
            }
        } else {
            v[f] = 0.f;
        }
    }
}

template <int DP, bool EXACT>
__device__ __forceinline__ void sm_store_rows(float* t, int D, const float (&v)[DP]) {
#pragma unroll
    for (int f = 0; f < DP; ++f)
        if (EXACT || f < SteinTile<DP>::PREV + 1 || f < D) t[f * SM_RS] = v[f];
}

template <int DP, int VW>
__global__ __launch_bounds__(256, (SteinTile<DP>::MT <= 2 ? 2 : 1))
void stein_moment_kernel(int K, int D_rt, int N, int wave_range, int stacks, int R, const float* __restrict__ packed,
                         const float* __restrict__ X, const float* __restrict__ TG, const float* __restrict__ QG,
                         const float* __restrict__ ld, const float* __restrict__ bg, const int32_t* __restrict__ mapping,
                         int map_offset, int own_rt, float* __restrict__ part, float* __restrict__ part_m) {
    using ST = SteinTile<DP>;
    constexpr int MT = ST::MT, NT = ST::NT, NB = ST::NB;
    constexpr bool EXACT = VW > 1;
    const int D = EXACT ? DP : D_rt;
    const bool own = EXACT ? false : own_rt != 0;
    extern __shared__ float sm[];
    __shared__ float sm_m[4][NB];
    const int tid = threadIdx.x;
    const int lane = tid & 63;
    const int wave = __builtin_amdgcn_readfirstlane(tid >> 6);
    const int D1 = D + 1;
    const int per_xcd = (stacks * R + 7) / 8;
    const int item = ((int)blockIdx.x & 7) * per_xcd + ((int)blockIdx.x >> 3);
    if (item >= stacks * R) return;
    const int range_id = item / stacks;
    const int k0 = (item - range_id * stacks) * NB;
    const int nb = min(NB, K - k0);
    const int rows_g = D1 + 1, rows_x = D1;
    constexpr int rows_e = NB + 1;
    const int wave_floats = (rows_g + rows_x + rows_e) * SM_RS;
    const int wave_stride = max(wave_floats, 16 * MT * (16 * NT + 1));
    float* Tg = sm + (size_t)wave * wave_stride;
    float* Tx = Tg + rows_g * SM_RS;
    float* Te = Tx + rows_x * SM_RS;
    for (int e = lane; e < SM_RS; e += 64) { Tg[D1 * SM_RS + e] = 0.f; Te[NB * SM_RS + e] = 0.f; Tx[D * SM_RS + e] = 1.f; }

    const int q = lane >> 4, c16 = lane & 15;
    int a_off[MT], x_off[NT], e_off[NT], cidx[NT];
    float mu[NT];
#pragma unroll
    for (int mt = 0; mt < MT; ++mt) {
        const int row = 16 * mt + c16;
        a_off[mt] = (row < D1 ? row : D1) * SM_RS + 4 * q;
    }
#pragma unroll
    for (int nt = 0; nt < NT; ++nt) {
        const int c = 16 * nt + c16;
        const int comp = c / D1, j = c - comp * D1;
        const bool valid = comp < nb;
        cidx[nt] = valid ? comp : NB;
        x_off[nt] = (valid ? j : 0) * SM_RS + 4 * q;
        e_off[nt] = (valid ? comp : NB) * SM_RS + 4 * q;
        mu[nt] = (valid && j < D) ? packed[(size_t)(k0 + comp) * Pack<DP>::STRIDE + j] : 0.f;
    }
    const int w_begin = min(N, (range_id * 4 + wave) * wave_range);
    const int w_end = min(N, w_begin + wave_range);

    float c_lim[NB];
#pragma unroll
    for (int c = 0; c < NB; ++c) c_lim[c] = c < nb ? 3.0e38f : -3.0e38f;
    auto log_weights = [&](int n0, float (&a)[NB]) {
        const int n = min(n0 + lane, N - 1);
        const float lim = (n0 + lane < w_end) ? 3.0e38f : -3.0e38f;
// ... 99 lines not shown
                    const int i = el / D1, j = el - i * D1;
                    const float* src = sm + i * CW + c * D1 + j;
                    dst[el] = fmaf(src[3 * wave_stride], f3, fmaf(src[2 * wave_stride], f2, fmaf(src[wave_stride], f1, src[0] * f0)));
                }
                if (tid == 0) part_m[(size_t)(k0 + c) * R + range_id] = Mall;
            }
        }
    } else {
        if (lane == 0) {
    #pragma unroll
            for (int c = 0; c < NB; ++c) sm_m[wave][c] = M[c];
        }
        __syncthreads();
        float Mall[NB], fsc[NB];
    #pragma unroll
        for (int c = 0; c < NB; ++c) {
            Mall[c] = fmaxf(fmaxf(sm_m[0][c], sm_m[1][c]), fmaxf(sm_m[2][c], sm_m[3][c]));
            fsc[c] = __expf(M[c] - Mall[c]);
        }
        constexpr int CW = 16 * NT + 1;
        float* C = sm;
        for (int w = 0; w < 4; ++w) {
            if (wave == w) {
    #pragma unroll
                for (int nt = 0; nt < NT; ++nt) {
                    float fs = 1.f;
    #pragma unroll
                    for (int c = 0; c < NB; ++c) fs = (cidx[nt] == c) ? fsc[c] : fs;
    #pragma unroll
                    for (int mt = 0; mt < MT; ++mt)
    #pragma unroll
                        for (int r = 0; r < 4; ++r) {
                            float* dst = C + (16 * mt + 4 * q + r) * CW + 16 * nt + c16;
                            const float v = acc[mt][nt][r] * fs;
                            *dst = (w == 0) ? v : *dst + v;
                        }
                }
            }
            __syncthreads();
        }
        const int DD = D1 * D1;
        for (int el = tid; el < nb * DD; el += 256) {
            const int comp = el / DD, rem = el - comp * DD;
            const int i = rem / D1, j = rem - i * D1;
            part[((size_t)(k0 + comp) * R + range_id) * DD + rem] = C[i * CW + comp * D1 + j];
        }
        if (tid < nb) part_m[(size_t)(k0 + tid) * R + range_id] = Mall[tid];
    }
}

template <int DP, int VW>
static int launch_stein_moment(gmmvi_ctx* ctx, int K, int D, const float* packed, const float* X, int N, const float* ld,
                               const float* qgrad, const float* bg, const float* tgrad, const int32_t* mapping,
                               int map_offset, int flags, float* H_neg, float* g_neg, SteinSlab* slab_out) {
    using ST = SteinTile<DP>;
    const int D1 = D + 1;
    const int stacks = (K + ST::NB - 1) / ST::NB;
    const int wgs_per_cu = ST::MT == 1 ? 2 : 1;
    static const int env_wgs = getenv("GMMVI_STEIN_WGS_PER_CU") ? atoi(getenv("GMMVI_STEIN_WGS_PER_CU")) : 0;
    int R = ((env_wgs > 0 ? env_wgs : wgs_per_cu) * ctx->num_cus) / stacks;
    if (R > (N + 255) / 256) R = (N + 255) / 256;
    if (R < 1) R = 1;
    int wave_range = (((N + R - 1) / R + 3) / 4 + 3) / 4 * 4;
    R = (N + 4 * wave_range - 1) / (4 * wave_range);
    const size_t part_floats = (size_t)K * R * D1 * D1;
    int rc = gmmvi_ws_reserve(ctx, (part_floats + (size_t)K * R) * sizeof(float));
    if (rc != GMMVI_OK) return rc;
    float* part = (float*)ctx->ws;
    float* part_m = part + part_floats;
    const int per_xcd = (stacks * R + 7) / 8;
    {
        size_t floats = (size_t)(2 * D1 + ST::NB + 2) * SM_RS;
        if (floats < (size_t)16 * ST::MT * (16 * ST::NT + 1)) floats = (size_t)16 * ST::MT * (16 * ST::NT + 1);
        const size_t shmem = 4 * floats * sizeof(float);
        static size_t attr = 64 * 1024;
        if (shmem > attr) {
            GMMVI_HIP_CHECK(ctx, hipFuncSetAttribute((const void*)stein_moment_kernel<DP, VW>,
                                                     hipFuncAttributeMaxDynamicSharedMemorySize, (int)shmem));
            attr = shmem;
        }
        GMMVI_PROF(ctx, "stein_partial");
        hipLaunchKernelGGL((stein_moment_kernel<DP, VW>), dim3(8 * per_xcd), dim3(256), shmem, ctx->stream, K, D, N, wave_range,
                           stacks, R, packed, X, tgrad, qgrad, ld, bg, mapping, map_offset,
                           (flags & GMMVI_OWN_SAMPLES_ONLY) ? 1 : 0, part, part_m);
    }
    GMMVI_LAUNCH_CHECK(ctx);
    if (slab_out != nullptr) {
        slab_out->part = part; slab_out->part_m = part_m; slab_out->R = R;
        return GMMVI_OK;
    }
    return launch_stein_finalize<DP>(ctx, K, D, R, N, flags, part, part_m, H_neg, g_neg, packed);
}

static int stein_moment(gmmvi_ctx* ctx, int K, int D, const float* packed, const float* X, int N, const float* ld,
                        const float* qgrad, const float* bg, const float* tgrad, const int32_t* mapping, int map_offset,
                        int flags, float* H_neg, float* g_neg, SteinSlab* slab_out) {
    const int dp = gmmvi_padded_dim(D);
    const uintptr_t bases = reinterpret_cast<uintptr_t>(X) | reinterpret_cast<uintptr_t>(tgrad) | reinterpret_cast<uintptr_t>(qgrad);
    const int vw_nat = (dp % 4 == 0) ? 4 : 2;
    const bool fast = D == dp && !(flags & GMMVI_OWN_SAMPLES_ONLY) && bases % (4 * vw_nat) == 0;
#define GMMVI_SM(DPV)                                                                                                  \
    case DPV:                                                                                                          \
        if (fast)                                                                                                      \
            return launch_stein_moment<DPV, (DPV % 4 == 0 ? 4 : 2)>(ctx, K, D, packed, X, N, ld, qgrad, bg, tgrad, mapping, \
                                                                    map_offset, flags, H_neg, g_neg, slab_out);         \
        return launch_stein_moment<DPV, 1>(ctx, K, D, packed, X, N, ld, qgrad, bg, tgrad, mapping, map_offset, flags, H_neg, g_neg, slab_out)
    switch (dp) {
        GMMVI_SM(2); GMMVI_SM(4); GMMVI_SM(8); GMMVI_SM(10); GMMVI_SM(12); GMMVI_SM(16); GMMVI_SM(20); GMMVI_SM(24);
        GMMVI_SM(32); GMMVI_SM(40); GMMVI_SM(50); GMMVI_SM(64);
        default: break;
    }
#undef GMMVI_SM
    return gmmvi_fail(ctx, GMMVI_ERR_ARG, "gmmvi_stein: unsupported dimension (D must be <= 63)");
}

extern "C" int gmmvi_stein(gmmvi_ctx* ctx, int K, int D, const float* packed_dev, const float* X_dev, int N,
                           const float* ld_dev, const float* qgrad_dev, const float* bg_dev, const float* tgrad_dev,
                           const int32_t* mapping_dev, int map_offset, int flags, float* H_neg_out_dev,
                           float* g_neg_out_dev) {
    GMMVI_ARG_CHECK(ctx, K >= 1 && D >= 1 && (D < GMMVI_MAX_DIM || gmmvi_is_blocked_dim(D)) && N >= 1);
    GMMVI_ARG_CHECK(ctx, packed_dev && X_dev && qgrad_dev && tgrad_dev && H_neg_out_dev && g_neg_out_dev);
    if (flags & GMMVI_OWN_SAMPLES_ONLY) GMMVI_ARG_CHECK(ctx, mapping_dev != nullptr);
    else GMMVI_ARG_CHECK(ctx, ld_dev && bg_dev);
    if (gmmvi_is_blocked_dim(D))
        return gmmvi_blocked_stein(ctx, K, D, packed_dev, X_dev, N, ld_dev, qgrad_dev, bg_dev, tgrad_dev, mapping_dev,
                                   map_offset, flags, H_neg_out_dev, g_neg_out_dev);
    return stein_moment(ctx, K, D, packed_dev, X_dev, N, ld_dev, qgrad_dev, bg_dev, tgrad_dev, mapping_dev, map_offset, flags,
                        H_neg_out_dev, g_neg_out_dev, nullptr);
}

int gmmvi_stein_partials(gmmvi_ctx* ctx, int K, int D, const float* packed_dev, const float* X_dev, int N, const float* ld_dev,
                         const float* qgrad_dev, const float* bg_dev, const float* tgrad_dev, int flags, SteinSlab* slab) {
    GMMVI_ARG_CHECK(ctx, K >= 1 && D >= 1 && D < GMMVI_MAX_DIM && !gmmvi_is_blocked_dim(D) && N >= 1 && slab != nullptr);
    GMMVI_ARG_CHECK(ctx, packed_dev && X_dev && qgrad_dev && tgrad_dev && ld_dev && bg_dev && !(flags & GMMVI_OWN_SAMPLES_ONLY));
    return stein_moment(ctx, K, D, packed_dev, X_dev, N, ld_dev, qgrad_dev, bg_dev, tgrad_dev, nullptr, 0, flags, nullptr, nullptr,
                        slab);
}

int gmmvi_stein_finalize_slab(gmmvi_ctx* ctx, int K, int D, const SteinSlab& slab, int N, int flags, const float* packed_dev,
                              float* H_neg_out_dev, float* g_neg_out_dev) {
    switch (gmmvi_padded_dim(D)) {
#define GMMVI_FIN(DPV) case DPV: return launch_stein_finalize<DPV>(ctx, K, D, slab.R, N, flags, slab.part, slab.part_m,       \
                                                                  H_neg_out_dev, g_neg_out_dev, packed_dev)
        GMMVI_FIN(2); GMMVI_FIN(4); GMMVI_FIN(8); GMMVI_FIN(10); GMMVI_FIN(12); GMMVI_FIN(16); GMMVI_FIN(20); GMMVI_FIN(24);
        GMMVI_FIN(32); GMMVI_FIN(40); GMMVI_FIN(50); GMMVI_FIN(64);
#undef GMMVI_FIN
        default: return gmmvi_fail(ctx, GMMVI_ERR_ARG, "stein_finalize: unsupported dimension");
    }
}
```

### gmmvi_amd/csrc/weights.hip

```cpp
#include "common.h"
#include "riders.h"
#include "stepsize_rules.h"
#include "wave_reduce.h"
#include "combine.h"
#include <cfloat>

namespace {

__device__ __forceinline__ float wsum(float v) { return gmmvi_wave_sum(v); }
__device__ __forceinline__ float wmax(float v) { return gmmvi_wave_max(v); }

__device__ float block_max(float v, float* red) {
    v = wmax(v);
    __syncthreads();
    if ((threadIdx.x & 63) == 0) red[threadIdx.x >> 6] = v;
    __syncthreads();
    return fmaxf(fmaxf(red[0], red[1]), fmaxf(red[2], red[3]));
}
__device__ float block_sum(float v, float* red) {
    v = wsum(v);
    __syncthreads();
    if ((threadIdx.x & 63) == 0) red[threadIdx.x >> 6] = v;
    __syncthreads();
    return (red[0] + red[1]) + (red[2] + red[3]);
}

template <int R>
__device__ __forceinline__ void elr_accumulate(int N, const float* __restrict__ row, const float* __restrict__ bg,
                                               const float* __restrict__ tlp, const float* __restrict__ logq, int Rrt, float beta,
                                               float& m, float& s, float& se, float& s2) {
    constexpr int B = 4;
    for (int n0 = threadIdx.x; n0 < N; n0 += 1024 * B) {
        float av[B], rv[B];
#pragma unroll
        for (int u = 0; u < B; ++u) {
            const int n = min(n0 + 1024 * u, N - 1);
            av[u] = row[n] - bg[n];
            float lq;
            if constexpr (R == 0) lq = logq[n];
            else if constexpr (R > 0) lq = combine_log_values_n<R>(logq, N, n);
            else lq = combine_log_values(logq, Rrt, N, n);
            rv[u] = tlp[n] - beta * lq;
        }
#pragma unroll
        for (int u = 0; u < B; ++u) {
            if (n0 + 1024 * u < N) {
                const float a = av[u], rho = rv[u];
                const float mn = fmaxf(m, a);
                const float sc = __expf(m - mn), e = __expf(a - mn);
                s = fmaf(s, sc, e);
                se = fmaf(se, sc, e * rho);
                s2 = fmaf(s2, sc * sc, e * e);
                m = mn;
            }
// ... 4 lines not shown
__device__ __forceinline__ void elr_body(int N, const float* __restrict__ ld, const float* __restrict__ bg,
                                         const float* __restrict__ tlp, const float* __restrict__ logq, int logq_R,
                                         float beta, const float* __restrict__ logw, int self_normalized,
                                         float* __restrict__ E_out, float* __restrict__ reward_out,
                                         float* __restrict__ ess_out) {
    __shared__ float red[4][16];
    const int k = blockIdx.x;
    const float* row = ld + (size_t)k * N;
    float m = -3.0e38f, s = 0.f, se = 0.f, s2 = 0.f;
    switch (logq_R) {
        case 0: elr_accumulate<0>(N, row, bg, tlp, logq, 0, beta, m, s, se, s2); break;
        case 2: elr_accumulate<2>(N, row, bg, tlp, logq, 2, beta, m, s, se, s2); break;
        case 3: elr_accumulate<3>(N, row, bg, tlp, logq, 3, beta, m, s, se, s2); break;
        case 4: elr_accumulate<4>(N, row, bg, tlp, logq, 4, beta, m, s, se, s2); break;
        case 5: elr_accumulate<5>(N, row, bg, tlp, logq, 5, beta, m, s, se, s2); break;
        case 6: elr_accumulate<6>(N, row, bg, tlp, logq, 6, beta, m, s, se, s2); break;
        case 7: elr_accumulate<7>(N, row, bg, tlp, logq, 7, beta, m, s, se, s2); break;
        case 8: elr_accumulate<8>(N, row, bg, tlp, logq, 8, beta, m, s, se, s2); break;
        case 10: elr_accumulate<10>(N, row, bg, tlp, logq, 10, beta, m, s, se, s2); break;
        case 12: elr_accumulate<12>(N, row, bg, tlp, logq, 12, beta, m, s, se, s2); break;
        case 16: elr_accumulate<16>(N, row, bg, tlp, logq, 16, beta, m, s, se, s2); break;
        default: elr_accumulate<-1>(N, row, bg, tlp, logq, logq_R, beta, m, s, se, s2); break;
    }
    const float mw = wmax(m);
    const float f = __expf(m - mw);
    s = wsum(s * f); se = wsum(se * f); s2 = wsum(s2 * f * f);
    const int lane = threadIdx.x & 63, wave = threadIdx.x >> 6;
    if (lane == 0) { red[0][wave] = mw; red[1][wave] = s; red[2][wave] = se; red[3][wave] = s2; }
    __syncthreads();
    if (threadIdx.x == 0) {
        float M = -3.0e38f;
        for (int w = 0; w < 16; ++w) M = fmaxf(M, red[0][w]);
        float S = 0.f, SE = 0.f, S2 = 0.f;
        for (int w = 0; w < 16; ++w) {
            const float g = __expf(red[0][w] - M);
            S = fmaf(red[1][w], g, S); SE = fmaf(red[2][w], g, SE); S2 = fmaf(red[3][w], g * g, S2);
        }
        const float E = self_normalized ? SE / S : SE * __expf(M) / (float)N;
        if (E_out) E_out[k] = E;
        if (reward_out) reward_out[k] = beta * logw[k] + E;
        if (ess_out) ess_out[k] = (S * S) / S2;
    }
}

__global__ __launch_bounds__(1024) void elr_kernel(int N, const float* __restrict__ ld, const float* __restrict__ bg,
                                                   const float* __restrict__ tlp, const float* __restrict__ logq, int logq_R,
                                                   float beta, const float* __restrict__ logw, int self_normalized,
                                                   float* __restrict__ E_out, float* __restrict__ reward_out,
                                                   float* __restrict__ ess_out) {
    elr_body(N, ld, bg, tlp, logq, logq_R, beta, logw, self_normalized, E_out, reward_out, ess_out);
}

template <int DP>
__global__ __launch_bounds__(1024) void elr_riders_kernel(int N, const float* __restrict__ ld, const float* __restrict__ bg,
                                                          const float* __restrict__ tlp, const float* __restrict__ logq,
                                                          int logq_R, float beta, const float* __restrict__ logw,
                                                          int self_normalized, float* __restrict__ E_out,
                                                          float* __restrict__ reward_out, float* __restrict__ ess_out,
                                                          Riders riders) {
    extern __shared__ __align__(16) float sm_riders[];
    if (riders_carried<DP>(riders, sm_riders)) return;
    elr_body(N, ld, bg, tlp, logq, logq_R, beta, logw, self_normalized, E_out, reward_out, ess_out);
}

__device__ float wave_lse(const float* v, int K) {
    const int t = threadIdx.x;
    float m = -3.0e38f;
    for (int i = t; i < K; i += 64) m = fmaxf(m, v[i]);
    m = wmax(m);
    float s = 0.f;
    for (int i = t; i < K; i += 64) s += __expf(v[i] - m);
    s = wsum(s);
    return m + __logf(s);
}

__device__ float weights_kl(float eta, float beta, const float* lw, const float* E, float* nl, int K) {
    const int t = threadIdx.x;
    const float a = (eta + 1.f) / (beta + eta), b = 1.f / (beta + eta);
    for (int i = t; i < K; i += 64) nl[i] = a * lw[i] + b * E[i];
    __syncthreads();
    float l = wave_lse(nl, K);
    for (int i = t; i < K; i += 64) nl[i] = fmaxf(nl[i] - l, -69.07f);
    __syncthreads();
    l = wave_lse(nl, K);
    float kl = 0.f;
    for (int i = t; i < K; i += 64) {
        const float v = nl[i] - l;
        nl[i] = v;
        kl = fmaf(__expf(v), v - lw[i], kl);
    }
    __syncthreads();
    return wsum(kl);
}

template <int NE>
__device__ __forceinline__ float weights_kl_reg(float eta, float beta, const float (&lw)[NE], const float (&E)[NE],
                                               const bool (&h)[NE], float (&v)[NE]) {
    const float a = (eta + 1.f) / (beta + eta), b = 1.f / (beta + eta);
    float nv[NE];
#pragma unroll
    for (int e = 0; e < NE; ++e) nv[e] = a * lw[e] + b * E[e];
    auto lse = [&](const float (&x)[NE]) {
        float m = -3.0e38f;
#pragma unroll
        for (int e = 0; e < NE; ++e)
            if (h[e]) m = fmaxf(m, x[e]);
        m = wmax(m);
        float s = 0.f;
#pragma unroll
        for (int e = 0; e < NE; ++e)
            if (h[e]) s += __expf(x[e] - m);
        s = wsum(s);
        return m + __logf(s);
    };
// ... 102 lines not shown
        }
    }
    if (!updated) {
        for (int i = t; i < K; i += 64) nl[i] = lw[i];
        __syncthreads();
    }
    const float l = wave_lse(nl, K);
    for (int i = t; i < K; i += 64) {
        const float v = nl[i] - l;
        logw[i] = v;
        if (exp_out) exp_out[i] = expf(v);
    }
    if (t == 0 && kl_eta_out) { kl_eta_out[0] = kl; kl_eta_out[1] = eta; }
}

__global__ void component_stepsize_kernel(int K, float* __restrict__ stepsizes, const float* __restrict__ prev,
                                          const float* __restrict__ last, float mn, float mx, float inc, float dec) {
    const int k = blockIdx.x * blockDim.x + threadIdx.x;
    if (k >= K) return;
    stepsizes[k] = component_stepsize_rule(stepsizes[k], prev[k], last[k], mn, mx, inc, dec);
}

__global__ __launch_bounds__(64) void weight_stepsize_kernel(int K, const float* __restrict__ logw,
                                                             const float* __restrict__ rewards_last, float* __restrict__ state,
                                                             float mn, float mx, float inc, float dec) {
    weight_stepsize_wave(K, logw, rewards_last, state, mn, mx, inc, dec, threadIdx.x);
}

}

extern "C" {

int gmmvi_expected_log_ratios(gmmvi_ctx* ctx, int K, int N, const float* ld_dev, const float* bg_dev,
                              const float* tlp_dev, const float* logq_dev, float beta, const float* logw_dev,
                              int self_normalized, float* E_out_dev, float* reward_out_dev, float* ess_out_dev) {
    GMMVI_ARG_CHECK(ctx, K >= 1 && N >= 1);
    GMMVI_ARG_CHECK(ctx, ld_dev && bg_dev && tlp_dev && logq_dev && logw_dev);
    int logq_R = 0;
    {
        const CombineJob& j = ctx->pending;
        if (j.R > 0 && j.lp_out == logq_dev && j.N == N && !j.grad_out && !j.lp2_out) {
            logq_R = j.R;
            logq_dev = j.lp_parts;
            ctx->pending = CombineJob();
        } else {
            int rc = gmmvi_flush_pending_combine(ctx);
            if (rc != GMMVI_OK) return rc;
        }
    }
    GMMVI_PROF(ctx, "expected_log_ratios");
    const Riders riders = gmmvi_take_pending_riders(ctx, K, 1024);
    if (riders.prep_blocks + riders.sample_blocks > 0) {
        const int dp = gmmvi_padded_dim(riders.sample_blocks > 0 ? riders.sample.D : 2);
        GMMVI_DISPATCH_DP(dp, hipLaunchKernelGGL((elr_riders_kernel<DP>), dim3(K + riders.prep_blocks + riders.sample_blocks),
                                                 dim3(1024), riders_lds_bytes(riders), ctx->stream, N, ld_dev, bg_dev, tlp_dev,
                                                 logq_dev, logq_R, beta, logw_dev, self_normalized, E_out_dev, reward_out_dev,
                                                 ess_out_dev, riders));
    } else {
        hipLaunchKernelGGL(elr_kernel, dim3(K), dim3(1024), 0, ctx->stream, N, ld_dev, bg_dev, tlp_dev, logq_dev, logq_R, beta,
                           logw_dev, self_normalized, E_out_dev, reward_out_dev, ess_out_dev);
    }
    GMMVI_LAUNCH_CHECK(ctx);
    return GMMVI_OK;
}

}

int gmmvi_update_weights_internal(gmmvi_ctx* ctx, int mode, int K, float* logw_dev, const float* E_dev,
                                  const float* stepsize_dev, float beta, float* kl_eta_out_dev, float* exp_out_dev) {
    GMMVI_ARG_CHECK(ctx, K >= 1 && K <= 4096);
    GMMVI_ARG_CHECK(ctx, logw_dev && E_dev && stepsize_dev);
    GMMVI_PROF(ctx, "update_weights");
    hipLaunchKernelGGL(update_weights_kernel, dim3(1), dim3(64), (size_t)3 * K * sizeof(float), ctx->stream, mode, K,
                       logw_dev, E_dev, stepsize_dev, beta, kl_eta_out_dev, exp_out_dev);
    GMMVI_LAUNCH_CHECK(ctx);
    return GMMVI_OK;
}

extern "C" {

int gmmvi_update_weights_kl(gmmvi_ctx* ctx, int K, float* logw_dev, const float* E_dev, const float* stepsize_dev,
                            float beta, float* kl_eta_out_dev) {
    return gmmvi_update_weights_internal(ctx, 0, K, logw_dev, E_dev, stepsize_dev, beta, kl_eta_out_dev, nullptr);
}

int gmmvi_update_weights_direct(gmmvi_ctx* ctx, int K, float* logw_dev, const float* E_dev,
                                const float* stepsize_dev, float beta) {
    return gmmvi_update_weights_internal(ctx, 1, K, logw_dev, E_dev, stepsize_dev, beta, nullptr, nullptr);
}

int gmmvi_component_stepsize_improvement(gmmvi_ctx* ctx, int K, float* stepsizes_dev, const float* rewards_prev_dev,
                                         const float* rewards_last_dev, float min_stepsize, float max_stepsize,
                                         float inc_factor, float dec_factor) {
    GMMVI_ARG_CHECK(ctx, K >= 1 && stepsizes_dev && rewards_prev_dev && rewards_last_dev);
    GMMVI_PROF(ctx, "component_stepsize");
    hipLaunchKernelGGL(component_stepsize_kernel, dim3((K + 127) / 128), dim3(128), 0, ctx->stream, K, stepsizes_dev,
                       rewards_prev_dev, rewards_last_dev, min_stepsize, max_stepsize, inc_factor, dec_factor);
    GMMVI_LAUNCH_CHECK(ctx);
    return GMMVI_OK;
}

int gmmvi_weight_stepsize_improvement(gmmvi_ctx* ctx, int K, const float* logw_dev, const float* rewards_last_dev,
                                      float* state_dev, float min_stepsize, float max_stepsize, float inc_factor,
                                      float dec_factor) {
    GMMVI_ARG_CHECK(ctx, K >= 1 && logw_dev && rewards_last_dev && state_dev);
    GMMVI_PROF(ctx, "weight_stepsize");
// ... 8 lines not shown
```

### gmmvi_amd/optimization/fused.py

```python
import ctypes as C
import os

import numpy as np

from .. import _lib, hip_ops
from .gmmvi_modules.sample_selector import VipsSampleSelector
from .gmmvi_modules.ng_estimator import SteinNgEstimator
from .gmmvi_modules.ng_based_component_updater import KLConstrainedNgBasedComponentUpdater
from .gmmvi_modules.component_stepsize_adaptation import (FixedComponentStepsizeAdaptation,
                                                          ImprovementBasedComponentStepsizeAdaptation)
from .gmmvi_modules.weight_stepsize_adaptation import (FixedWeightStepsizeAdaptation,
                                                       ImprovementBasedWeightStepsizeAdaptation)
from .gmmvi_modules.weight_updater import DirectWeightUpdater, TrustRegionBasedWeightUpdater
from .gmmvi_modules.component_adaptation import FixedComponentAdaptation

_f, _i, _p = C.c_float, C.c_int32, C.c_void_p


class SamtronPlan(C.Structure):
    _fields_ = [
        ("K", _i), ("D", _i), ("N", _i), ("target_kind", _i), ("target_family", _i), ("target_K", _i),
        ("target_nu", _f), ("target_packed", _p), ("target_logw", _p), ("planar_prior_std", _p), ("planar_goals", _p),
        ("planar_goals_count", _i), ("planar_likelihood_std", _f),
        ("means", _p), ("chols", _p), ("logw", _p), ("packed", _p), ("packed_new", _p),
        ("stepsizes", _p), ("last_eta", _p), ("l2", _p), ("num_updates", _p), ("success_out", _p),
        ("offsets", _p), ("max_per_component", _i), ("n_old", _i), ("bg_K", _i), ("bg_packed", _p), ("bg_logw", _p),
        ("bg_old", _p), ("bg_logw_new", _p), ("bg_log_share_old", _f), ("bg_log_share_new", _f),
        ("seed", C.c_uint64), ("first_index", C.c_uint64),
        ("db_samples", _p), ("db_tlp", _p), ("db_tgrad", _p), ("db_mapping", _p), ("mapping_base", _i),
        ("db_means", _p), ("db_chols", _p), ("db_packed", _p),
        ("reward_prev", _p), ("reward_last", _p), ("reward_next", _p), ("weight_slot", _p), ("wstate", _p),
        ("temperature", _f), ("l2_init", _f),
        ("component_stepsize_mode", _i), ("cs_min", _f), ("cs_max", _f), ("cs_inc", _f), ("cs_dec", _f),
        ("weight_stepsize_mode", _i), ("ws_min", _f), ("ws_max", _f), ("ws_inc", _f), ("ws_dec", _f),
        ("weight_update_mode", _i), ("stein_flags", _i), ("presample_next", _i), ("presampled", _i), ("phase", _i),
        ("logreg_A", _p), ("logreg_M", _i), ("logreg_prior_mean", _f), ("logreg_prior_std", _f),
        ("talos_model", _p), ("talos_context", _p),
    ]


class SamtronFastPath:
    def __init__(self, gmmvi):
        self.g = gmmvi
        self.plan = SamtronPlan()
        self.enabled = os.environ.get("GMMVI_FAST_PATH", "1") != "0"
        self._static_ok = None
        self.explicit_estimate = os.environ.get("GMMVI_EXPLICIT_ESTIMATE", "0") == "1"
        self.presample = os.environ.get("GMMVI_PRESAMPLE", "1") != "0"
        self._presample_token = None
        self.prefetch_counts = os.environ.get("GMMVI_PREFETCH_COUNTS", "1") != "0"
        self._prefetch = None
        self._pinned = None
        self._event = None
        lib = _lib.load()
        lib.gmmvi_train_iter_samtron.restype = C.c_int
        lib.gmmvi_train_iter_samtron.argtypes = [C.c_void_p, C.POINTER(SamtronPlan)]
        self._fn = lib.gmmvi_train_iter_samtron

    def _check_static(self):
        g = self.g
        sel, est, upd = g.sample_selector, g.ng_estimator, g.ng_based_updater
        wu, cs, ws = g.weight_updater, g.component_stepsize_adapter, g.weight_stepsize_adapter
        tgt = sel.target_distribution
        ok = (type(sel) is VipsSampleSelector and type(est) is SteinNgEstimator
              and type(upd) is KLConstrainedNgBasedComponentUpdater
              and type(cs) in (FixedComponentStepsizeAdaptation, ImprovementBasedComponentStepsizeAdaptation)
              and type(ws) in (FixedWeightStepsizeAdaptation, ImprovementBasedWeightStepsizeAdaptation)
              and type(wu) in (DirectWeightUpdater, TrustRegionBasedWeightUpdater)
              and hasattr(tgt, "_fast_path_target")
              and not est._only_use_own_samples
              and est._use_self_normalized_importance_weights == wu.use_self_normalized_importance_weights
              and g.sample_db.keep_samples and g.model.num_dimensions < _lib.MAX_DIM
              and g.model.num_dimensions <= _lib.blocked_above()
              and not g.model.diagonal_covs)
        return bool(ok)

    def eligible(self):
        ok = self._eligible()
        if not ok and self._prefetch is not None:
            self.drop_prefetch()
        return ok

    def _eligible(self):
        if not self.enabled:
            return False
        if self._static_ok is None:
            self._static_ok = self._check_static()
        if not self._static_ok:
            return False
        g = self.g
        sel, db = g.sample_selector, g.sample_db
        if sel.eps_override is not None or not sel.fuse_background:
            return False
        if g.ng_based_updater.want_info or g.weight_updater.want_info:
            return False
        n_new = sel.desired_samples_per_component * g.model.num_components
        if db.max_samples is not None and n_new + db._samples.n > db.max_samples:
            return False
        return sel.desired_samples_per_component >= 1

    def _state_token(self):
        g = self.g
        sel, db, model = g.sample_selector, g.sample_db, g.model.model
        return (db._samples.n, db._means.n, db._epoch, int(db._num_samples_written), db._samples.buf.ptr, model.num_components,
                id(model._packed), model.means.ptr, model.chol_cov.ptr, sel.desired_samples_per_component,
                sel.reused_samples_per_component)

    def drop_prefetch(self):
        pf, self._prefetch = self._prefetch, None
        if pf is not None:
# ... 68 lines not shown
        p.num_updates, p.success_out = m.num_received_updates.ptr, success.ptr
        p.seed = int(model.seed) & 0xFFFFFFFFFFFFFFFF
        p.reward_prev, p.reward_last = m.reward_slot(1).ptr, m.reward_slot(0).ptr
        p.reward_next = m.next_reward_slot().ptr
        p.weight_slot = m.next_weight_slot().ptr
        ws, cs, wu = g.weight_stepsize_adapter, g.component_stepsize_adapter, g.weight_updater
        p.wstate = ws._state.ptr
        p.temperature, p.l2_init = float(g.temperature), float(m.initial_regularizer)
        if type(cs) is ImprovementBasedComponentStepsizeAdaptation:
            p.component_stepsize_mode = 1
            p.cs_min, p.cs_max = cs.min_stepsize, cs.max_stepsize
            p.cs_inc, p.cs_dec = cs.stepsize_inc_factor, cs.stepsize_dec_factor
        else:
            p.component_stepsize_mode = 0
        if type(ws) is ImprovementBasedWeightStepsizeAdaptation:
            p.weight_stepsize_mode = 1
            p.ws_min, p.ws_max = ws.min_stepsize, ws.max_stepsize
            p.ws_inc, p.ws_dec = ws.stepsize_inc_factor, ws.stepsize_dec_factor
        else:
            p.weight_stepsize_mode = 0
        p.weight_update_mode = 0 if type(wu) is TrustRegionBasedWeightUpdater else 1
        p.stein_flags = _lib.SELF_NORMALIZED if g.ng_estimator._use_self_normalized_importance_weights else 0
        if self.explicit_estimate:
            p.stein_flags |= _lib.EXPLICIT_ESTIMATE

    def step(self):
        g = self.g
        m = g.model
        model = m.model
        ctx = model.ctx
        sel, db = g.sample_selector, g.sample_db
        k, d = model.num_components, model.num_dimensions
        p = self.plan

        stride = db._packed.inner[0]
        packed_cur = model.packed
        packed_new = ctx.empty((k, stride))
        success = ctx.empty((k,), np.int32)
        self._fill_static(p, packed_cur, packed_new, success)

        counts, n_old = self._new_sample_counts()
        n = int(counts.sum())
        key = counts.tobytes()
        offsets = np.concatenate([[0], np.cumsum(counts)]).astype(np.int32)
        offsets_dev = ctx.cached_const(("offsets", offsets.tobytes()), lambda: ctx.asarray(offsets, np.int32))
        if getattr(sel, "_mapping_key", None) != key:
            sel._mapping_key = key
            sel._last_mapping_host = np.repeat(np.arange(k, dtype=np.int32), counts)
        sel._last_counts = counts

        presample_next = (self.presample and n_old == 0 and sel.reused_samples_per_component == 0
                          and type(g.num_component_adapter) is FixedComponentAdaptation
                          and (db.max_samples is None or db._samples.n + 2 * n <= db.max_samples))
        for grow, rows in ((db._samples, 2 * n if presample_next else n), (db._target_lnpdfs, n), (db._target_grads, n),
                           (db._mapping_dev, 2 * n if presample_next else n), (db._means, k), (db._chols, k), (db._packed, k)):
            grow.reserve(rows)
        s0, c0 = db._samples.n, db._means.n

        db._mapping_host.append(sel._last_mapping_host + np.int32(c0))
        db._segments.append((s0, c0, counts))
        if n_old == 0:
            bg_logw = ctx.cached_const(("bg_logw", key), lambda: ctx.asarray(np.log(counts / counts.sum()).astype(np.float32)))
            p.n_old, p.bg_K, p.bg_packed = 0, 0, None
        else:
            mix = self._bg_mix() if callable(self._bg_mix) else self._bg_mix
            assert int(mix.active.max()) < c0, "the reused samples come from earlier appends"
            self._bg_keepalive = (mix.packed, mix.logw_dev)
            bg_packed_ptr, bg_logw = mix.packed.ptr, mix.logw_dev
            bg_logw_new = ctx.cached_const(("bg_logw", key), lambda: ctx.asarray(np.log(counts / counts.sum()).astype(np.float32)))
            self._bg_logw_new_keepalive = bg_logw_new
            p.n_old, p.bg_K, p.bg_packed = n_old, len(mix.active), bg_packed_ptr
            p.bg_old, p.bg_logw_new = self._bg_old.ptr, bg_logw_new.ptr
            p.bg_log_share_old, p.bg_log_share_new = db.log_shares(n_old, n)
        p.max_per_component = int(counts.max())

        p.K, p.D, p.N = k, d, n
        p.offsets, p.bg_logw = offsets_dev.ptr, bg_logw.ptr
        p.first_index = int(db._num_samples_written)
        p.db_samples = db._samples.buf.ptr + s0 * d * 4
        p.db_tlp = db._target_lnpdfs.buf.ptr + s0 * 4
        p.db_tgrad = db._target_grads.buf.ptr + s0 * d * 4
        p.db_mapping, p.mapping_base = db._mapping_dev.buf.ptr + s0 * 4, c0
        p.db_means = db._means.buf.ptr + c0 * d * 4
        p.db_chols = db._chols.buf.ptr + c0 * d * d * 4
        p.db_packed = db._packed.buf.ptr + c0 * stride * 4

        here = (db._samples.buf.ptr, db._mapping_dev.buf.ptr, s0, c0, n, k, key, int(db._num_samples_written),
                int(model.seed), model.means.ptr, model.chol_cov.ptr, offsets_dev.ptr)
        tok, self._presample_token = self._presample_token, None
        p.presampled = int(tok is not None and n_old == 0 and tok[0] == here and tok[1] is model._packed)
        p.presample_next = int(presample_next)

        prefetch_next = self.prefetch_counts and sel.reused_samples_per_component > 0
        p.phase = 1 if prefetch_next else 0
        try:
            ctx.check(self._fn(ctx.handle, C.byref(p)))
        except Exception:
            db._mapping_host.n -= len(sel._last_mapping_host)
            db._segments.pop()
            db._seg_start, db._seg_size, db._seg_info = [], [], {}
            raise

        for grow, rows in ((db._samples, n), (db._target_lnpdfs, n), (db._target_grads, n), (db._mapping_dev, n),
                           (db._means, k), (db._chols, k), (db._packed, k)):
            grow.n += rows
        db._num_samples_written += n
        if n_old > 0:
            db._bg_cache = None
        model._packed = packed_new
        model._eval_cache = None
        if prefetch_next:
            caches = (db._bg_cache, db._pd)
            ess, bg_old_next, bg_mix_next, n_old_next = self._issue_counts()
            pinned = self._pinned_floats(k)
            ctx.check(ctx.lib.gmmvi_download_async(ctx.handle, pinned[0], ess.ptr, 4 * k))
            ctx.record(self._event)
            p.phase = 2
            ctx.check(self._fn(ctx.handle, C.byref(p)))
            p.phase = 0
            self._prefetch = {"ess": ess, "bg_old": bg_old_next, "bg_mix": bg_mix_next, "n_old": n_old_next,
                              "db_caches": caches, "token": None}
        m.commit_rewards()
        if k > 1:
            m._t_weight += 1
        if presample_next:
            self._presample_token = ((db._samples.buf.ptr, db._mapping_dev.buf.ptr, s0 + n, c0 + k, n, k, key,
                                      int(db._num_samples_written), int(model.seed), model.means.ptr, model.chol_cov.ptr,
                                      offsets_dev.ptr), packed_new)
        g.ng_based_updater.last_success = success
        g.num_updates.assign_add(1)
        if self._prefetch is not None:
            self._prefetch["token"] = self._state_token()
```

### include/gmmvi_hip.h

```cpp
#ifndef GMMVI_HIP_H
#define GMMVI_HIP_H

#include <stddef.h>
#include <stdint.h>

#ifdef __cplusplus
extern "C" {
#endif

typedef struct gmmvi_ctx gmmvi_ctx;

enum gmmvi_status {
    GMMVI_OK = 0,
    GMMVI_ERR_HIP = -1,
    GMMVI_ERR_ARG = -2,
    GMMVI_ERR_RCCL = -3,
    GMMVI_ERR_STATE = -4
};

enum gmmvi_family {
    GMMVI_GAUSS = 0,
    GMMVI_STUDENT_T = 1
};

// ... 138 lines not shown
int gmmvi_update_weights_direct(gmmvi_ctx* ctx, int K, float* logw_dev, const float* E_dev,
                                const float* stepsize_dev, float beta);
int gmmvi_component_stepsize_improvement(gmmvi_ctx* ctx, int K, float* stepsizes_dev, const float* rewards_prev_dev,
                                         const float* rewards_last_dev, float min_stepsize, float max_stepsize,
                                         float inc_factor, float dec_factor);
int gmmvi_weight_stepsize_improvement(gmmvi_ctx* ctx, int K, const float* logw_dev, const float* rewards_last_dev,
                                      float* state_dev, float min_stepsize, float max_stepsize, float inc_factor,
                                      float dec_factor);

typedef struct gmmvi_samtron_plan {
    int32_t K, D, N;
    int32_t target_kind;
    int32_t target_family, target_K;
    float target_nu;
    const float* target_packed;
    const float* target_logw;
    const float* planar_prior_std;
    const float* planar_goals;
    int32_t planar_goals_count;
    float planar_likelihood_std;
    float* means; float* chols; float* logw;
    const float* packed;
    float* packed_new;
    float* stepsizes; float* last_eta; float* l2; float* num_updates;
    int32_t* success_out;
    const int32_t* offsets;
    int32_t max_per_component;
    int32_t n_old;
    int32_t bg_K;
    const float* bg_packed;
    const float* bg_logw;
    const float* bg_old;
    const float* bg_logw_new;
    float bg_log_share_old, bg_log_share_new;
    uint64_t seed, first_index;
    float* db_samples; float* db_tlp; float* db_tgrad; int32_t* db_mapping; int32_t mapping_base;
    float* db_means; float* db_chols; float* db_packed;
    const float* reward_prev; const float* reward_last; float* reward_next; float* weight_slot;
    float* wstate;
    float temperature, l2_init;
    int32_t component_stepsize_mode;
    float cs_min, cs_max, cs_inc, cs_dec;
    int32_t weight_stepsize_mode;
    float ws_min, ws_max, ws_inc, ws_dec;
    int32_t weight_update_mode;
    int32_t stein_flags;
    int32_t presample_next, presampled;
    int32_t phase;
    const float* logreg_A;
    int32_t logreg_M;
    float logreg_prior_mean, logreg_prior_std;
    const float* talos_model;
    const float* talos_context;
} gmmvi_samtron_plan;
int gmmvi_train_iter_samtron(gmmvi_ctx* ctx, const gmmvi_samtron_plan* plan);

typedef struct gmmvi_sharded_plan {
    int32_t n_ranks, rank;
    int32_t K, D, N;
    int32_t target_kind, target_family, target_K;
    float target_nu;
    const float* target_packed; const float* target_logw;
    const float* planar_prior_std; const float* planar_goals;
    int32_t planar_goals_count; float planar_likelihood_std;
    float* means; float* chols; const float* packed; float* packed_new;
    float* stepsizes; float* last_eta; float* l2; float* num_updates; int32_t* success_out;
    float* logw_all;
    const float* bg_logw;
    const int32_t* offsets;
    int32_t max_per_component;
    uint64_t seed, first_index;
    float* e1;
    float* e2;
    float* e3;
    float* x_all; float* tlp_all; float* tgrad_all;
    float* E_all; float* reward_all;
    int32_t has_pending;
    float* reward_col_pending;
    const float* reward_prev; const float* reward_last;
    const float* reward_last_all;
    float* wstate;
    float temperature, l2_init;
    int32_t component_stepsize_mode; float cs_min, cs_max, cs_inc, cs_dec;
    int32_t weight_stepsize_mode; float ws_min, ws_max, ws_inc, ws_dec;
    int32_t stein_flags;
    int32_t presample_next, presampled;
    float* scratch;
    const float* logreg_A;
    int32_t logreg_M;
    float logreg_prior_mean, logreg_prior_std;
    const float* talos_model;
    const float* talos_context;
} gmmvi_sharded_plan;
size_t gmmvi_sharded_scratch_floats(int K, int D, int N);
int gmmvi_train_iter_sharded_phase(gmmvi_ctx* ctx, const gmmvi_sharded_plan* plan, int phase );

int gmmvi_comm_unique_id(char* out_id_128);
int gmmvi_comm_init(gmmvi_ctx* ctx, const char* unique_id_128, int n_ranks, int rank);
int gmmvi_comm_destroy(gmmvi_ctx* ctx);
int gmmvi_allgather_f32(gmmvi_ctx* ctx, const float* send_dev, float* recv_dev, size_t count_per_rank);
int gmmvi_allreduce_f32(gmmvi_ctx* ctx, float* buf_dev, size_t count, int op );
int gmmvi_combine_partials(gmmvi_ctx* ctx, int R, int N, int D, const float* lp_parts_dev,
                           const float* grad_parts_dev, float* lp_out_dev, float* grad_out_dev);

int gmmvi_diag_embed(gmmvi_ctx* ctx, int K, int D, const float* diag_dev, float* dense_out_dev);
int gmmvi_diag_extract(gmmvi_ctx* ctx, int K, int D, const float* dense_dev, float* diag_out_dev);
int gmmvi_reciprocal_f32(gmmvi_ctx* ctx, const float* src_dev, size_t n, float* dst_dev);
size_t gmmvi_diag_packed_stride(int D);
// ... 30 lines not shown
```

Before: 4.811 billion samples*components/s.

## Fold target evaluation into presample riders and self-merge partials via tickets

```diff
diff --git a/gmmvi_amd/_lib.py b/gmmvi_amd/_lib.py
--- a/gmmvi_amd/_lib.py
+++ b/gmmvi_amd/_lib.py
@@ -110,6 +110,8 @@
     "gmmvi_component_stepsize_improvement": (_i, [_p, _i, _p, _p, _p, _f, _f, _f, _f]),
     "gmmvi_weight_stepsize_improvement": (_i, [_p, _i, _p, _p, _p, _f, _f, _f, _f]),
     "gmmvi_train_iter_samtron": (_i, [_p, _p]),
+    "gmmvi_samtron_early_target_ok": (_i, [_p, _p]),
+    "gmmvi_debug_merge_tickets": (_i, [_p, _p, _i]),
     "gmmvi_sharded_scratch_floats": (_sz, [_i, _i, _i]),
     "gmmvi_train_iter_sharded_phase": (_i, [_p, _p, _i]),
     "gmmvi_comm_unique_id": (_i, [C.c_char_p]),
diff --git a/gmmvi_amd/csrc/api.hip b/gmmvi_amd/csrc/api.hip
--- a/gmmvi_amd/csrc/api.hip
+++ b/gmmvi_amd/csrc/api.hip
@@ -1,5 +1,6 @@
 #include "common.h"
 #include <cstring>
+#include <cstdlib>
 #include "blocked.h"
 
 std::string g_gmmvi_global_err;
@@ -44,6 +45,8 @@
     }
     hipDeviceProp_t prop;
     if (hipGetDeviceProperties(&prop, device) == hipSuccess) ctx->num_cus = prop.multiProcessorCount;
+    const char* six = getenv("GMMVI_SIX_LAUNCHES");
+    ctx->six_launches = !(six && six[0] == '0');
     *out = ctx;
     return GMMVI_OK;
 }
@@ -63,6 +66,7 @@
         (void)hipHostFree(ctx->up_ring);
     }
     if (ctx->defer_ws) (void)hipFree(ctx->defer_ws);
+    if (ctx->tickets) (void)hipFree(ctx->tickets);
     delete ctx;
 }
 
diff --git a/gmmvi_amd/csrc/combine.h b/gmmvi_amd/csrc/combine.h
--- a/gmmvi_amd/csrc/combine.h
+++ b/gmmvi_amd/csrc/combine.h
@@ -115,3 +115,39 @@
     }
     return true;
 }
+
+template <int R>
+__device__ __forceinline__ void combine_rows_n(const CombineJob& j, int n0, int rows) {
+    const bool with_grad = j.grad_out != nullptr && j.grad_parts != nullptr;
+    const int width = with_grad ? j.D : 1;
+    const long lo = (long)n0 * width, hi = (long)min(n0 + rows, j.N) * width;
+    for (long e = lo + threadIdx.x; e < hi; e += blockDim.x) combine_element_n<R>(j, e);
+}
+
+__device__ __forceinline__ void combine_tile(const SelfMerge& sm, int n0, int rows, unsigned* flag) {
+    __threadfence();
+    __syncthreads();
+    if (threadIdx.x == 0) {
+        const unsigned ticket = atomicAdd(&sm.tickets[blockIdx.x], 1u);
+        const unsigned last = ticket == gridDim.y - 1 ? 1u : 0u;
+        if (last) atomicExch(&sm.tickets[blockIdx.x], 0u);
+        *flag = last;
+    }
+    __syncthreads();
+    if (*flag == 0u) return;
+    __threadfence();
+    const CombineJob& j = sm.job;
+    switch (j.R) {
+        case 2: combine_rows_n<2>(j, n0, rows); break;
+        case 3: combine_rows_n<3>(j, n0, rows); break;
+        case 4: combine_rows_n<4>(j, n0, rows); break;
+        case 5: combine_rows_n<5>(j, n0, rows); break;
+        case 6: combine_rows_n<6>(j, n0, rows); break;
+        case 7: combine_rows_n<7>(j, n0, rows); break;
+        case 8: combine_rows_n<8>(j, n0, rows); break;
+        case 10: combine_rows_n<10>(j, n0, rows); break;
+        case 12: combine_rows_n<12>(j, n0, rows); break;
+        case 16: combine_rows_n<16>(j, n0, rows); break;
+        default: combine_rows_n<0>(j, n0, rows); break;
+    }
+}
diff --git a/gmmvi_amd/csrc/comm.hip b/gmmvi_amd/csrc/comm.hip
--- a/gmmvi_amd/csrc/comm.hip
+++ b/gmmvi_amd/csrc/comm.hip
@@ -71,7 +71,35 @@
     return j;
 }
 
+int gmmvi_self_merge_reserve(gmmvi_ctx* ctx, int tiles, SelfMerge* out) {
+    *out = SelfMerge();
+    if (!ctx->six_launches) return GMMVI_OK;
+    if ((size_t)tiles > ctx->tickets_n) {
+        GMMVI_HIP_CHECK(ctx, hipStreamSynchronize(ctx->stream));
+        if (ctx->tickets) GMMVI_HIP_CHECK(ctx, hipFree(ctx->tickets));
+        ctx->tickets = nullptr;
+        ctx->tickets_n = 0;
+        const size_t want = (size_t)tiles * 2 > 1024 ? (size_t)tiles * 2 : 1024;
+        GMMVI_HIP_CHECK(ctx, hipMalloc((void**)&ctx->tickets, want * sizeof(unsigned)));
+        ctx->tickets_n = want;
+        GMMVI_HIP_CHECK(ctx, hipMemsetAsync(ctx->tickets, 0, want * sizeof(unsigned), ctx->stream));
+    }
+    out->tickets = ctx->tickets;
+    return GMMVI_OK;
+}
+
 extern "C" {
+
+int gmmvi_debug_merge_tickets(gmmvi_ctx* ctx, unsigned* out_host, int n) {
+    if (!ctx) return -1;
+    const int have = (int)ctx->tickets_n;
+    const int m = n < have ? n : have;
+    if (m > 0 && out_host) {
+        if (hipStreamSynchronize(ctx->stream) != hipSuccess) return -1;
+        if (hipMemcpy(out_host, ctx->tickets, (size_t)m * sizeof(unsigned), hipMemcpyDeviceToHost) != hipSuccess) return -1;
+    }
+    return have;
+}
 
 int gmmvi_comm_unique_id(char* out_id_128) {
     if (!out_id_128) return gmmvi_fail(nullptr, GMMVI_ERR_ARG, "gmmvi_comm_unique_id: NULL buffer");
diff --git a/gmmvi_amd/csrc/common.h b/gmmvi_amd/csrc/common.h
--- a/gmmvi_amd/csrc/common.h
+++ b/gmmvi_amd/csrc/common.h
@@ -27,17 +27,33 @@
     float* X = nullptr; int32_t* mapping = nullptr; int32_t mapping_base = 0;
 };
 
+struct TargetJob {
+    int on = 0, family = 0, K = 0, nw = 0;
+    float nu = 0.f;
+    unsigned lds_bytes = 0;
+    const float* packed = nullptr; const float* logw = nullptr;
+    float* tlp = nullptr; float* tgrad = nullptr;
+};
+
 struct Riders {
     int first_block = 0;
     int prep_blocks = 0;
     int sample_blocks = 0;
     PrepArgs prep;
     SampleJob sample;
+    TargetJob target;
 };
 
 inline size_t riders_lds_bytes(const Riders& r) {
-    return r.sample_blocks > 0 ? ((size_t)r.sample.D * r.sample.D + r.sample.D + 256 * (size_t)(r.sample.D | 1)) * sizeof(float) : 0;
-}
+    if (r.sample_blocks == 0) return 0;
+    const size_t draw = ((size_t)r.sample.D * r.sample.D + r.sample.D + 256 * (size_t)(r.sample.D | 1)) * sizeof(float);
+    return r.target.on && r.target.lds_bytes > draw ? r.target.lds_bytes : draw;
+}
+
+struct SelfMerge {
+    unsigned* tickets = nullptr;
+    CombineJob job;
+};
 
 struct gmmvi_ctx {
     int device = 0;
@@ -61,6 +77,9 @@
     Riders riders;
     void* defer_ws = nullptr;
     size_t defer_bytes = 0;
+    bool six_launches = true;
+    unsigned* tickets = nullptr;
+    size_t tickets_n = 0;
     void* comm = nullptr;
     int n_ranks = 1, rank = 0;
     int num_cus = 256;
@@ -127,9 +146,12 @@
 CombineJob gmmvi_take_pending_combine(gmmvi_ctx* ctx, int threads, int first_block, bool light = false);
 Riders gmmvi_take_pending_riders(gmmvi_ctx* ctx, int first_block, int threads, bool prep_only = false);
 int gmmvi_flush_pending_riders(gmmvi_ctx* ctx);
+int gmmvi_self_merge_reserve(gmmvi_ctx* ctx, int tiles, SelfMerge* out);
+bool gmmvi_target_rider_geometry(gmmvi_ctx* ctx, int K, int D, int N, int* nw, unsigned* lds_bytes);
 struct SteinSlab;
 int gmmvi_stein_partials(gmmvi_ctx* ctx, int K, int D, const float* packed_dev, const float* X_dev, int N, const float* ld_dev,
-                         const float* qgrad_dev, const float* bg_dev, const float* tgrad_dev, int flags, SteinSlab* slab);
+                         const float* qgrad_dev, const float* bg_dev, const float* tgrad_dev, int flags, SteinSlab* slab,
+                         bool carry_prep = false);
 int gmmvi_stein_finalize_slab(gmmvi_ctx* ctx, int K, int D, const SteinSlab& slab, int N, int flags, const float* packed_dev,
                               float* H_neg_out_dev, float* g_neg_out_dev);
 int gmmvi_update_components_kl_from_slab(gmmvi_ctx* ctx, int K, int D, const SteinSlab& slab, int N, int stein_flags,
diff --git a/gmmvi_amd/csrc/density.hip b/gmmvi_amd/csrc/density.hip
--- a/gmmvi_amd/csrc/density.hip
+++ b/gmmvi_amd/csrc/density.hip
@@ -98,13 +98,6 @@
     if (t == 0 && ok) ok[k] = good ? 1 : 0;
 }
 
-typedef float me_f32x4 __attribute__((ext_vector_type(4)));
-#define ME_LDS_BARRIER()                                       \
-    do {                                                       \
-        asm volatile("s_waitcnt lgkmcnt(0)" ::: "memory");     \
-        __builtin_amdgcn_s_barrier();                          \
-        asm volatile("" ::: "memory");                         \
-    } while (0)
 __host__ __device__ constexpr int me_rem_rows(int dp) { return (dp % 16 != 0 && dp % 16 <= 4 && dp > 16) ? dp % 16 : 0; }
 template <int R>
 __device__ __forceinline__ float me_row_bcast(float v) {
@@ -138,13 +131,14 @@
     return hipMemcpyFromSymbol(out, HIP_SYMBOL(g_me_ph), sizeof(long long) * (size_t)n) == hipSuccess ? 0 : -1;
 }
 #endif
+#include "mixture_tile.h"
 template <int DP, int FAMILY, bool GRAD>
 __global__ __launch_bounds__(DP >= GMMVI_ME_WIDE_DP ? 512 : GMMVI_ME_THREADS, GMMVI_ME_MINW) void mixture_eval_kernel(float nu, int K_total, int D, const float* __restrict__ packed,
                                                             const float* __restrict__ logw, const float* __restrict__ X,
                                                             int N, float* __restrict__ ld_out, float* __restrict__ lp_out,
                                                             float* __restrict__ grad_out, const float* __restrict__ logw2,
-                                                            float* __restrict__ lp2_out, CombineJob carried, Riders riders) {
-    using PK = Pack<DP>;
+                                                            float* __restrict__ lp2_out, CombineJob carried, Riders riders,
+                                                            SelfMerge self) {
     extern __shared__ __align__(16) float sm[];
     if (combine_carried(carried) || riders_carried<DP>(riders, sm)) return;
     const int kchunk = (K_total + gridDim.y - 1) / gridDim.y;
@@ -155,181 +149,9 @@
         if (lp2_out) lp2_out += (size_t)blockIdx.y * N;
         if (GRAD && grad_out) grad_out += (size_t)blockIdx.y * N * D;
     }
-    const int lane = threadIdx.x & 63;
-    const int wave = __builtin_amdgcn_readfirstlane(threadIdx.x >> 6);
-    const int nwaves = blockDim.x >> 6;
-    const int n0 = blockIdx.x * 64;
-    const int n_here = min(64, N - n0);
-    const int n = n0 + lane;
-    const bool valid = lane < n_here;
-    float* sm_merge = sm;
-#ifdef GMMVI_ME_STAMPS
-    if (threadIdx.x == 0) {
-        g_me_wg[2 * (blockIdx.y * gridDim.x + blockIdx.x)] = wall_clock64();
-        unsigned hw, xcc;
-        asm volatile("s_getreg_b32 %0, hwreg(HW_REG_HW_ID)" : "=s"(hw));
-        asm volatile("s_getreg_b32 %0, hwreg(HW_REG_XCC_ID)" : "=s"(xcc));
-        g_me_hw[blockIdx.y * gridDim.x + blockIdx.x] = ((unsigned long long)xcc << 32) | hw;
-    }
-    unsigned long long stamp[16];
-    int nstamp = 0, nbackward = 0;
-    const long long wc0 = wall_clock64();
-#define ME_STAMP() do { asm volatile("s_waitcnt lgkmcnt(0)" ::: "memory"); if (nstamp < 16) stamp[nstamp++] = __builtin_amdgcn_s_memtime(); } while (0)
-    ME_STAMP();
-#else
-#define ME_STAMP()
-#endif
-
-    const int ldx = D | 1;
-    float x[DP];
-    if (DP % 4 == 0 && D == DP && (reinterpret_cast<uintptr_t>(X) & 15) == 0) {
-        const float4* xrow = reinterpret_cast<const float4*>(X + (size_t)min(n, N - 1) * D);
-#pragma unroll
-        for (int q4 = 0; q4 < DP / 4; ++q4) {
-            const float4 v4 = xrow[q4];
-            x[4 * q4] = v4.x; x[4 * q4 + 1] = v4.y; x[4 * q4 + 2] = v4.z; x[4 * q4 + 3] = v4.w;
-        }
-        if (!valid) {
-#pragma unroll
-            for (int i = 0; i < DP; ++i) x[i] = 0.f;
-        }
-    } else if (DP % 2 == 0 && D == DP && (reinterpret_cast<uintptr_t>(X) & 7) == 0) {
-        const float2* xrow = reinterpret_cast<const float2*>(X + (size_t)min(n, N - 1) * D);
-#pragma unroll
-        for (int q2 = 0; q2 < DP / 2; ++q2) {
-            const float2 v2 = xrow[q2];
-            x[2 * q2] = v2.x; x[2 * q2 + 1] = v2.y;
-        }
-        if (!valid) {
-#pragma unroll
-            for (int i = 0; i < DP; ++i) x[i] = 0.f;
-        }
-    } else {
-        for (int e = threadIdx.x; e < n_here * D; e += blockDim.x) sm_merge[(e / D) * ldx + (e % D)] = X[(size_t)n0 * D + e];
-        __syncthreads();
-#pragma unroll
-        for (int i = 0; i < DP; ++i) x[i] = (valid && i < D) ? sm_merge[lane * ldx + i] : 0.f;
-        __syncthreads();
-    }
-
-    float m = -3.0e38f, s = 0.f;
-    float m2 = -3.0e38f, s2 = 0.f;
-    const bool dual = logw2 != nullptr;
-    float acc[GRAD ? DP : 1];
-    if (GRAD) {
-#pragma unroll
-        for (int i = 0; i < DP; ++i) acc[i] = 0.f;
-    }
-    const float nud = nu + (float)D;
-    ME_STAMP();
-
-    for (int k = k_lo + wave; k < K; k += nwaves) {
-        ME_STAMP();
-        const sp_block_ptr blk = sp_block(packed + (size_t)k * PK::STRIDE);
-        const float lw = ((sp_const_f32)(uintptr_t)logw)[k];
-        const float lw2 = dual ? ((sp_const_f32)(uintptr_t)logw2)[k] : 0.f;
-        float z[DP], vrd[DP], q, cst;
-        float pc[2][32];
-        SpPass<DP>::forward(blk, x, z, vrd, q, cst, pc);
-        sp_block_ptr blkb = blk;
-        asm volatile("" : "+s"(blkb));
-        if constexpr (GRAD) SpPass<DP>::backward_prefetch(blkb, pc);
-        float ld, coef;
-        if (FAMILY == GMMVI_GAUSS) {
-            ld = fmaf(-0.5f, q, cst);
-            coef = -1.f;
-        } else {
-            ld = cst - 0.5f * nud * log1pf(q / nu);
-            coef = -nud / (nu + q);
-        }
-        const float a = ld + lw;
-        const float mn = fmaxf(m, a);
-        const float sc = __expf(m - mn);
-        const float e = __expf(a - mn);
-        s = fmaf(s, sc, e);
-        m = mn;
-        if (dual) {
-            const float a2 = ld + lw2;
-            const float mn2 = fmaxf(m2, a2);
-            s2 = fmaf(s2, __expf(m2 - mn2), __expf(a2 - mn2));
-            m2 = mn2;
-        }
-        if constexpr (GRAD) {
-            SpPass<DP>::backward(blkb, z, vrd, pc);
-            const float ec = e * coef;
-#pragma unroll
-            for (int i = 0; i < DP; ++i) acc[i] = fmaf(acc[i], sc, ec * z[i]);
-            sp_pin<DP>(acc);
-        }
-        if (ld_out != nullptr && valid) ld_out[(size_t)k * N + n] = ld;
-    }
-    ME_STAMP();
-    if (lp_out == nullptr && !GRAD) return;
-
-    constexpr int NQ = (DP + 3) / 4;
-    float* sm_m = sm_merge;
-    float* sm_s = sm_merge + nwaves * 64;
-    me_f32x4* sm_acc = reinterpret_cast<me_f32x4*>(sm_merge + 2 * nwaves * 64);
-    float* outt = sm_merge + 2 * nwaves * 64 + (GRAD ? (size_t)nwaves * NQ * 256 : 0);
-    float* sm_m2 = outt + (GRAD ? 64 * ldx : 0);
-    float* sm_s2 = sm_m2 + nwaves * 64;
-    sm_m[wave * 64 + lane] = m;
-    if (dual) sm_m2[wave * 64 + lane] = m2;
-    ME_LDS_BARRIER();
-    ME_STAMP();
-    float M = -3.0e38f, M2 = -3.0e38f;
-    for (int w = 0; w < nwaves; ++w) M = fmaxf(M, sm_m[w * 64 + lane]);
-    const float f = __expf(m - M);
-    sm_s[wave * 64 + lane] = s * f;
-    if (dual) {
-        for (int w = 0; w < nwaves; ++w) M2 = fmaxf(M2, sm_m2[w * 64 + lane]);
-        sm_s2[wave * 64 + lane] = s2 * __expf(m2 - M2);
-    }
-    if (GRAD) {
-#pragma unroll
-        for (int q4 = 0; q4 < NQ; ++q4) {
-            me_f32x4 v4;
-#pragma unroll
-            for (int c = 0; c < 4; ++c) v4[c] = 4 * q4 + c < DP ? acc[4 * q4 + c] * f : 0.f;
-            sm_acc[(wave * NQ + q4) * 64 + lane] = v4;
-        }
-    }
-    ME_STAMP();
-    ME_LDS_BARRIER();
-    ME_STAMP();
-    float S = 0.f;
-    for (int w = 0; w < nwaves; ++w) S += sm_s[w * 64 + lane];
-    if (wave == 0 && valid && lp_out != nullptr) lp_out[n] = M + __logf(S);
-    if (dual && wave == (nwaves > 1 ? 1 : 0) && valid && lp2_out != nullptr) {
-        float S2 = 0.f;
-        for (int w = 0; w < nwaves; ++w) S2 += sm_s2[w * 64 + lane];
-        lp2_out[n] = M2 + __logf(S2);
-    }
-    if (GRAD && grad_out != nullptr) {
-        const float inv = 1.f / S;
-        for (int q4 = wave; q4 < NQ; q4 += nwaves) {
-            me_f32x4 g4 = {0.f, 0.f, 0.f, 0.f};
-            for (int w = 0; w < nwaves; ++w) g4 += sm_acc[(w * NQ + q4) * 64 + lane];
-#pragma unroll
-            for (int c = 0; c < 4; ++c)
-                if (4 * q4 + c < D) outt[lane * ldx + 4 * q4 + c] = g4[c] * inv;
-        }
-        ME_STAMP();
-        ME_LDS_BARRIER();
-        ME_STAMP();
-        for (int e = threadIdx.x; e < n_here * D; e += blockDim.x)
-            grad_out[(size_t)n0 * D + e] = outt[(e / D) * ldx + (e % D)];
-    }
-#ifdef GMMVI_ME_STAMPS
-    ME_STAMP();
-    if (threadIdx.x == 0) g_me_wg[2 * (blockIdx.y * gridDim.x + blockIdx.x) + 1] = wall_clock64();
-    if (GRAD && logw2 && blockIdx.x == 60 && blockIdx.y == 1 && threadIdx.x == 64 * 3 && (g_me_wg[2 * 8192 - 1]++ & 15) == 12) {
-        const long long wc1 = wall_clock64();
-        printf("me stamps (shader cycles; kernel %lld x 10 ns by the 100 MHz clock):", wc1 - wc0);
-        for (int i = 1; i < nstamp; ++i) printf(" %llu", stamp[i] - stamp[i - 1]);
-        printf("  total %llu, backward passes %d\n", stamp[nstamp - 1] - stamp[0], nbackward);
-    }
-#endif
+    me_tile<DP, FAMILY, GRAD, false>(sm, nu, k_lo, K, D, packed, logw, X, N, blockIdx.x * 64, N, blockDim.x >> 6, ld_out, lp_out,
+                                     grad_out, logw2, lp2_out);
+    if (GRAD && self.tickets != nullptr) combine_tile(self, blockIdx.x * 64, 64, reinterpret_cast<unsigned*>(sm));
 }
 
 template <int DP, int FAMILY, bool GRAD>
@@ -337,7 +159,8 @@
                                                                const float* __restrict__ logw, const float* __restrict__ X, int N,
                                                                float* __restrict__ ld_out, float* __restrict__ lp_out,
                                                                float* __restrict__ grad_out, const float* __restrict__ logw2,
-                                                               float* __restrict__ lp2_out, CombineJob carried, Riders riders) {
+                                                               float* __restrict__ lp2_out, CombineJob carried, Riders riders,
+                                                               SelfMerge self) {
     using PK = Pack<DP>;
     static_assert(DP % 2 == 0, "padded dimensions are even");
     constexpr int NP2 = DP / 2;
@@ -513,7 +336,9 @@
         }
     }
     PK_STAMP();
-    if (wave != 0) return;
+    const bool self_merge = GRAD && self.tickets != nullptr;
+    if (wave != 0 && !self_merge) return;
+    if (wave == 0) {
     if (lp_out != nullptr) {
         if (validA) lp_out[nA] = M.x + __logf(s.x);
         if (validB) lp_out[nB] = M.y + __logf(s.y);
@@ -545,6 +370,8 @@
         }
     }
     PK_STAMP();
+    }
+    if (self_merge) combine_tile(self, n0, 128, reinterpret_cast<unsigned*>(sm));
 #ifdef GMMVI_ME_STAMPS
     if (threadIdx.x == 0 && wg_lin < 8192) g_me_wg[2 * wg_lin + 1] = wall_clock64();
 #endif
@@ -1300,7 +1127,12 @@
     float* lp_k = lp;
     float* grad_k = grad;
     float* lp2_k = lp2;
-    const bool defer = ctx->defer_combine && ky > 1 && want_merge;
+    SelfMerge self;
+    if (ky > 1 && want_grad) {
+        int rc = gmmvi_self_merge_reserve(ctx, tiles, &self);
+        if (rc != GMMVI_OK) return rc;
+    }
+    const bool defer = ctx->defer_combine && ky > 1 && want_merge && self.tickets == nullptr;
     if (defer) {
         int rc = gmmvi_flush_pending_combine(ctx);
         if (rc != GMMVI_OK) return rc;
@@ -1312,6 +1144,12 @@
         lp_k = (float*)(defer ? ctx->defer_ws : ctx->ws);
         lp2_k = logw2 ? lp_k + (size_t)ky * N : nullptr;
         grad_k = want_grad ? lp_k + (size_t)ky * N * (logw2 ? 2 : 1) : nullptr;
+    }
+    if (self.tickets != nullptr) {
+        CombineJob& j = self.job;
+        j.R = ky; j.N = N; j.D = D;
+        j.lp_parts = lp_k; j.grad_parts = grad_k; j.lp2_parts = lp2_k;
+        j.lp_out = lp; j.grad_out = grad; j.lp2_out = lp2_k ? lp2 : nullptr;
     }
     const Riders riders = gmmvi_take_pending_riders(ctx, tiles, nw * 64);
     const CombineJob carried = gmmvi_take_pending_combine(ctx, nw * 64, tiles + riders.prep_blocks + riders.sample_blocks);
@@ -1325,7 +1163,7 @@
             GMMVI_HIP_CHECK(ctx, hipFuncSetAttribute((const void*)mixture_eval_pk_kernel<DP, FAM, G>,               \
                                                      hipFuncAttributeMaxDynamicSharedMemorySize, (int)shmem));         \
         hipLaunchKernelGGL((mixture_eval_pk_kernel<DP, FAM, G>), grid, block, shmem, ctx->stream, nu, K, D, packed, \
-                           logw, X, N, ld, lp_k, grad_k, logw2, lp2_k, carried, riders);                                         \
+                           logw, X, N, ld, lp_k, grad_k, logw2, lp2_k, carried, riders, self);                            \
     } while (0)
         if constexpr (DP <= 40) {
             if (family == GMMVI_GAUSS) {
@@ -1345,12 +1183,55 @@
         j.R = ky; j.N = N; j.D = D;
         j.lp_parts = lp_k; j.grad_parts = grad_k; j.lp2_parts = lp2_k;
         j.lp_out = lp; j.grad_out = grad; j.lp2_out = lp2_k ? lp2 : nullptr;
-    } else if (ky > 1 && want_merge) {
+    } else if (ky > 1 && want_merge && self.tickets == nullptr) {
         GMMVI_PROF(ctx, "mixture_combine");
         int rc = gmmvi_combine_partials_internal(ctx, ky, N, D, lp_k, grad_k, lp, grad, lp2_k, lp2);
         if (rc != GMMVI_OK) return rc;
     }
     return GMMVI_OK;
+}
+
+template <int DP>
+static bool me_takes_pk(int K, int N, bool with_grad) {
+    using PK = Pack<DP>;
+    static const int env_pk = getenv("GMMVI_ME_PK") ? atoi(getenv("GMMVI_ME_PK")) : -1;
+    static const long env_pk_min = getenv("GMMVI_ME_PK_MIN") ? atol(getenv("GMMVI_ME_PK_MIN")) : 4096;
+    static const int env_pk_wide = getenv("GMMVI_ME_PK_WIDE") ? atoi(getenv("GMMVI_ME_PK_WIDE")) : 1;
+    const long passes = (long)((N + 127) / 128) * K;
+    const bool shape_ok = !PK::FRAGS || (env_pk_wide && (!with_grad || DP <= 40));
+    if constexpr (DP <= 50) return shape_ok && env_pk != 0 && (env_pk == 1 || passes >= env_pk_min);
+    return false;
+}
+
+template <int DP>
+static void me_one_geometry(const gmmvi_ctx* ctx, int K, int D, int N, bool want_grad, bool dual, int& ky, int& nw, size_t& shmem) {
+    static const int env_nw = getenv("GMMVI_ME_NW") ? atoi(getenv("GMMVI_ME_NW")) : 0;
+    static const int env_ky = getenv("GMMVI_ME_KY") ? atoi(getenv("GMMVI_ME_KY")) : 0;
+    auto lds_floats = [&](int nw) {
+        size_t merge = (size_t)nw * 64 * ((want_grad ? (DP + 3) / 4 * 4 : 0) + 2) + (want_grad ? 64 * (size_t)(D | 1) : 0) +
+                       (dual ? (size_t)nw * 128 : 0);
+        size_t stage = 64 * (size_t)(D | 1);
+        return merge > stage ? merge : stage;
+    };
+    const int tiles = (N + 63) / 64;
+    const int nw_max = DP >= GMMVI_ME_WIDE_DP ? 8 : 16;
+    ky = 1; nw = K < nw_max ? K : nw_max;
+    if (env_ky > 0) ky = env_ky < K ? env_ky : K;
+    else if (K >= 16 && 2L * tiles <= 3L * ctx->num_cus) {
+        ky = (int)((2L * ctx->num_cus + tiles / 2) / tiles);
+        if (ky > K / 8) ky = K / 8;
+        if (ky < 1) ky = 1;
+        if (ky > 1) nw = 8;
+    }
+    const int kchunk = (K + ky - 1) / ky;
+    ky = (K + kchunk - 1) / kchunk;
+    if (nw > kchunk) nw = kchunk;
+    if (env_nw > 0) nw = env_nw < kchunk ? env_nw : kchunk;
+    if (nw > nw_max) nw = nw_max;
+    while (nw > 1 && lds_floats(nw) * 4 > 96 * 1024) --nw;
+    shmem = lds_floats(nw) * 4;
+    static const size_t env_shmem_min = getenv("GMMVI_ME_SHMEM_MIN") ? (size_t)atol(getenv("GMMVI_ME_SHMEM_MIN")) : 0;
+    if (shmem < env_shmem_min) shmem = env_shmem_min;
 }
 
 template <int DP>
@@ -1358,16 +1239,9 @@
                                const float* logw, const float* X, int N, float* ld, float* lp, float* grad,
                                const float* logw2 = nullptr, float* lp2 = nullptr) {
     using PK = Pack<DP>;
-    {
-        static const int env_pk = getenv("GMMVI_ME_PK") ? atoi(getenv("GMMVI_ME_PK")) : -1;
-        static const long env_pk_min = getenv("GMMVI_ME_PK_MIN") ? atol(getenv("GMMVI_ME_PK_MIN")) : 4096;
-        static const int env_pk_wide = getenv("GMMVI_ME_PK_WIDE") ? atoi(getenv("GMMVI_ME_PK_WIDE")) : 1;
-        const long passes = (long)((N + 127) / 128) * K;
-        const bool shape_ok = !PK::FRAGS || (env_pk_wide && (grad == nullptr || DP <= 40));
-        if constexpr (DP <= 50) {
-            if (shape_ok && env_pk != 0 && (env_pk == 1 || passes >= env_pk_min))
-                return launch_mixture_eval_pk<DP>(ctx, family, nu, K, D, packed, logw, X, N, ld, lp, grad, logw2, lp2);
-        }
+    if constexpr (DP <= 50) {
+        if (me_takes_pk<DP>(K, N, grad != nullptr))
+            return launch_mixture_eval_pk<DP>(ctx, family, nu, K, D, packed, logw, X, N, ld, lp, grad, logw2, lp2);
     }
     if constexpr (PK::FRAGS) {
         static const int env_ws = getenv("GMMVI_ME_WS") ? atoi(getenv("GMMVI_ME_WS")) : -1;
@@ -1383,37 +1257,19 @@
     } else {
     const bool want_grad = grad != nullptr;
     const bool want_merge = want_grad || lp != nullptr;
-    static const int env_nw = getenv("GMMVI_ME_NW") ? atoi(getenv("GMMVI_ME_NW")) : 0;
-    static const int env_ky = getenv("GMMVI_ME_KY") ? atoi(getenv("GMMVI_ME_KY")) : 0;
-    auto lds_floats = [&](int nw) {
-        size_t merge = (size_t)nw * 64 * ((want_grad ? (DP + 3) / 4 * 4 : 0) + 2) + (want_grad ? 64 * (size_t)(D | 1) : 0) +
-                       (logw2 ? (size_t)nw * 128 : 0);
-        size_t stage = 64 * (size_t)(D | 1);
-        return merge > stage ? merge : stage;
-    };
     const int tiles = (N + 63) / 64;
-    const int nw_max = DP >= GMMVI_ME_WIDE_DP ? 8 : 16;
-    int ky = 1, nw = K < nw_max ? K : nw_max;
-    if (env_ky > 0) ky = env_ky < K ? env_ky : K;
-    else if (K >= 16 && 2L * tiles <= 3L * ctx->num_cus) {
-        ky = (int)((2L * ctx->num_cus + tiles / 2) / tiles);
-        if (ky > K / 8) ky = K / 8;
-        if (ky < 1) ky = 1;
-        if (ky > 1) nw = 8;
-    }
-    const int kchunk = (K + ky - 1) / ky;
-    ky = (K + kchunk - 1) / kchunk;
-    if (nw > kchunk) nw = kchunk;
-    if (env_nw > 0) nw = env_nw < kchunk ? env_nw : kchunk;
-    if (nw > nw_max) nw = nw_max;
-    while (nw > 1 && lds_floats(nw) * 4 > 96 * 1024) --nw;
-    size_t shmem = lds_floats(nw) * 4;
-    static const size_t env_shmem_min = getenv("GMMVI_ME_SHMEM_MIN") ? (size_t)atol(getenv("GMMVI_ME_SHMEM_MIN")) : 0;
-    if (shmem < env_shmem_min) shmem = env_shmem_min;
+    int ky, nw;
+    size_t shmem;
+    me_one_geometry<DP>(ctx, K, D, N, want_grad, logw2 != nullptr, ky, nw, shmem);
     float* lp_k = lp;
     float* grad_k = grad;
     float* lp2_k = lp2;
-    const bool defer = ctx->defer_combine && ky > 1 && want_merge;
+    SelfMerge self;
+    if (ky > 1 && want_grad) {
+        int rc = gmmvi_self_merge_reserve(ctx, tiles, &self);
+        if (rc != GMMVI_OK) return rc;
+    }
+    const bool defer = ctx->defer_combine && ky > 1 && want_merge && self.tickets == nullptr;
     if (defer) {
         int rc = gmmvi_flush_pending_combine(ctx);
         if (rc != GMMVI_OK) return rc;
@@ -1425,6 +1281,12 @@
         lp_k = (float*)(defer ? ctx->defer_ws : ctx->ws);
         lp2_k = logw2 ? lp_k + (size_t)ky * N : nullptr;
         grad_k = want_grad ? lp_k + (size_t)ky * N * (logw2 ? 2 : 1) : nullptr;
+    }
+    if (self.tickets != nullptr) {
+        CombineJob& j = self.job;
+        j.R = ky; j.N = N; j.D = D;
+        j.lp_parts = lp_k; j.grad_parts = grad_k; j.lp2_parts = lp2_k;
+        j.lp_out = lp; j.grad_out = grad; j.lp2_out = lp2_k ? lp2 : nullptr;
     }
     const Riders riders = gmmvi_take_pending_riders(ctx, tiles, nw * 64);
     const CombineJob carried = gmmvi_take_pending_combine(ctx, nw * 64, tiles + riders.prep_blocks + riders.sample_blocks);
@@ -1438,7 +1300,7 @@
             GMMVI_HIP_CHECK(ctx, hipFuncSetAttribute((const void*)mixture_eval_kernel<DP, FAM, G>,               \
                                                      hipFuncAttributeMaxDynamicSharedMemorySize, (int)shmem));      \
         hipLaunchKernelGGL((mixture_eval_kernel<DP, FAM, G>), grid, block, shmem, ctx->stream, nu, K, D, packed, \
-                           logw, X, N, ld, lp_k, grad_k, logw2, lp2_k, carried, riders);                                      \
+                           logw, X, N, ld, lp_k, grad_k, logw2, lp2_k, carried, riders, self);                            \
     } while (0)
         if (family == GMMVI_GAUSS) {
             if (want_grad) GMMVI_LAUNCH_ME(GMMVI_GAUSS, true); else GMMVI_LAUNCH_ME(GMMVI_GAUSS, false);
@@ -1453,13 +1315,32 @@
         j.R = ky; j.N = N; j.D = D;
         j.lp_parts = lp_k; j.grad_parts = grad_k; j.lp2_parts = lp2_k;
         j.lp_out = lp; j.grad_out = grad; j.lp2_out = lp2_k ? lp2 : nullptr;
-    } else if (ky > 1 && want_merge) {
+    } else if (ky > 1 && want_merge && self.tickets == nullptr) {
         GMMVI_PROF(ctx, "mixture_combine");
         int rc = gmmvi_combine_partials_internal(ctx, ky, N, D, lp_k, grad_k, lp, grad, lp2_k, lp2);
         if (rc != GMMVI_OK) return rc;
     }
     return GMMVI_OK;
     }
+}
+
+bool gmmvi_target_rider_geometry(gmmvi_ctx* ctx, int K, int D, int N, int* nw_out, unsigned* lds_bytes) {
+    if (K < 1 || D < 1 || N < 1 || gmmvi_is_blocked_dim(D)) return false;
+    const int dp = gmmvi_padded_dim(D);
+    if (dp < 0 || dp >= GMMVI_MFMA_DENSITY_FROM_DP) return false;
+    int ky = 0, nw = 0;
+    size_t shmem = 0;
+    bool pk = true;
+    switch (dp) {
+#define GMMVI_TRG(DPV) case DPV: pk = me_takes_pk<DPV>(K, N, true); me_one_geometry<DPV>(ctx, K, D, N, true, false, ky, nw, shmem); break
+        GMMVI_TRG(2); GMMVI_TRG(4); GMMVI_TRG(8); GMMVI_TRG(10); GMMVI_TRG(12); GMMVI_TRG(16); GMMVI_TRG(20); GMMVI_TRG(24);
+#undef GMMVI_TRG
+        default: return false;
+    }
+    if (pk || ky != 1 || nw < 1 || nw > 16) return false;
+    *nw_out = nw;
+    *lds_bytes = (unsigned)shmem;
+    return true;
 }
 
 int gmmvi_pack_register_layout(gmmvi_ctx* ctx, int K, int D, const float* means_dev, const float* chols_dev, float* packed_dev) {
diff --git a/gmmvi_amd/csrc/fused.hip b/gmmvi_amd/csrc/fused.hip
--- a/gmmvi_amd/csrc/fused.hip
+++ b/gmmvi_amd/csrc/fused.hip
@@ -31,6 +31,13 @@
 
 static int train_iter_samtron_body(gmmvi_ctx* ctx, const gmmvi_samtron_plan* p);
 
+extern "C" int gmmvi_samtron_early_target_ok(gmmvi_ctx* ctx, const gmmvi_samtron_plan* p) {
+    if (!ctx || !p || !ctx->six_launches || p->target_kind != 0 || !p->target_packed || !p->target_logw) return 0;
+    int nw = 0;
+    unsigned lds = 0;
+    return gmmvi_target_rider_geometry(ctx, p->target_K, p->D, p->N, &nw, &lds) ? 1 : 0;
+}
+
 extern "C" int gmmvi_train_iter_samtron(gmmvi_ctx* ctx, const gmmvi_samtron_plan* p) {
     GMMVI_ARG_CHECK(ctx, ctx != nullptr);
     int rc = gmmvi_flush_pending_combine(ctx);
@@ -38,8 +45,10 @@
     if (rc != GMMVI_OK) {
         ctx->pending = CombineJob();
         ctx->riders.prep_blocks = ctx->riders.sample_blocks = 0;
-        ctx->defer_combine = false;
-        ctx->prof_tag = nullptr;
+        ctx->riders.target = TargetJob();
+        ctx->defer_combine = false;
+        ctx->prof_tag = nullptr;
+        if (ctx->tickets) (void)hipMemsetAsync(ctx->tickets, 0, ctx->tickets_n * sizeof(unsigned), ctx->stream);
     }
     return rc;
 }
@@ -56,6 +65,7 @@
                              p->db_tgrad && p->db_mapping && p->reward_next && p->wstate);
     GMMVI_ARG_CHECK(ctx, p->n_old >= 0 && p->max_per_component >= 0 && p->phase >= 0 && p->phase <= 2);
     GMMVI_ARG_CHECK(ctx, p->n_old == 0 || (p->bg_packed != nullptr && p->bg_K >= 1 && p->bg_old != nullptr && p->bg_logw_new != nullptr));
+    GMMVI_ARG_CHECK(ctx, !p->early_target || (p->presampled && p->n_old == 0 && p->target_kind == 0 && ctx->six_launches));
     const int n_old = p->n_old;
     const int Na = n_old + N;
     const size_t KN = (size_t)K * Na, ND = (size_t)Na * D;
@@ -134,7 +144,9 @@
         ctx->riders.prep = prep_later;
         ctx->riders.prep_blocks = K < 64 ? K : 64;
     }
-    if (p->target_kind == 1) {
+    const bool target_done = p->early_target != 0;
+    if (target_done) {
+    } else if (p->target_kind == 1) {
         GMMVI_TRY(gmmvi_target_planar(ctx, D, p->planar_prior_std, p->planar_goals_count, p->planar_goals,
                                       p->planar_likelihood_std, x, N, p->db_tlp, p->db_tgrad));
     } else if (p->target_kind == 2) {
@@ -150,9 +162,10 @@
         GMMVI_TRY(rc_t);
     }
     GMMVI_TRY(gmmvi_flush_pending_combine(ctx));
+    if (!target_done) GMMVI_TRY(gmmvi_flush_pending_riders(ctx));
+    SteinSlab slab{nullptr, nullptr, 0};
+    GMMVI_TRY(gmmvi_stein_partials(ctx, K, D, p->packed, xa, Na, a.ld, a.qgrad, a.bg, tgrad_a, p->stein_flags, &slab, target_done));
     GMMVI_TRY(gmmvi_flush_pending_riders(ctx));
-    SteinSlab slab{nullptr, nullptr, 0};
-    GMMVI_TRY(gmmvi_stein_partials(ctx, K, D, p->packed, xa, Na, a.ld, a.qgrad, a.bg, tgrad_a, p->stein_flags, &slab));
     GMMVI_TRY(gmmvi_update_components_kl_from_slab(ctx, K, D, slab, Na, p->stein_flags, p->packed, a.H, a.g, p->means, p->chols,
                                                    p->stepsizes, p->temperature, p->l2_init, p->last_eta, p->l2, p->num_updates,
                                                    p->success_out ? p->success_out : a.success, p->packed_new));
@@ -172,9 +185,22 @@
         sj.seed = p->seed; sj.first_index = p->first_index + (uint64_t)N;
         sj.X = x + (size_t)N * D; sj.mapping = p->db_mapping + N; sj.mapping_base = p->mapping_base + K;
         ctx->riders.sample_blocks = K * ((max_pc + 255) / 256);
+        TargetJob& tj = ctx->riders.target;
+        tj = TargetJob();
+        if (p->early_target_next) {
+            GMMVI_ARG_CHECK(ctx, gmmvi_samtron_early_target_ok(ctx, p) == 1);
+            gmmvi_target_rider_geometry(ctx, p->target_K, D, N, &tj.nw, &tj.lds_bytes);
+            tj.on = 1; tj.family = p->target_family; tj.K = p->target_K; tj.nu = p->target_nu;
+            tj.packed = p->target_packed; tj.logw = p->target_logw;
+            tj.tlp = p->db_tlp + N; tj.tgrad = p->db_tgrad + (size_t)N * D;
+        }
+    } else {
+        GMMVI_ARG_CHECK(ctx, !p->early_target_next);
     }
     GMMVI_TRY(gmmvi_expected_log_ratios(ctx, K, Na, a.ld, a.bg, tlp_a, a.lq, p->temperature, p->logw,
                                         (p->stein_flags & GMMVI_SELF_NORMALIZED) ? 1 : 0, a.E, p->reward_next, nullptr));
+    ctx->riders.target = TargetJob();
+    GMMVI_ARG_CHECK(ctx, !p->early_target_next || ctx->riders.sample_blocks == 0);
     GMMVI_TRY(gmmvi_flush_pending_riders(ctx));
     if (K > 1) {
         GMMVI_TRY(gmmvi_update_weights_internal(ctx, p->weight_update_mode == 0 ? 0 : 1, K, p->logw, a.E, p->wstate,
diff --git a/gmmvi_amd/csrc/mixture_tile.h b/gmmvi_amd/csrc/mixture_tile.h
--- /dev/null
+++ b/gmmvi_amd/csrc/mixture_tile.h
@@ -0,0 +1,196 @@
+#pragma once
+#include "common.h"
+#include "subst_phased.h"
+
+typedef float me_f32x4 __attribute__((ext_vector_type(4)));
+#define ME_LDS_BARRIER()                                       \
+    do {                                                       \
+        asm volatile("s_waitcnt lgkmcnt(0)" ::: "memory");     \
+        __builtin_amdgcn_s_barrier();                          \
+        asm volatile("" ::: "memory");                         \
+    } while (0)
+
+template <int DP, int FAMILY, bool GRAD, bool GUEST>
+__device__ __forceinline__ void me_tile(float* sm, float nu, int k_lo, int K, int D, const float* __restrict__ packed,
+                                        const float* __restrict__ logw, const float* __restrict__ X, int N, int n0, int n_end,
+                                        int nwaves, float* __restrict__ ld_out, float* __restrict__ lp_out,
+                                        float* __restrict__ grad_out, const float* __restrict__ logw2,
+                                        float* __restrict__ lp2_out) {
+    using PK = Pack<DP>;
+    const int lane = threadIdx.x & 63;
+    const int wave = __builtin_amdgcn_readfirstlane(threadIdx.x >> 6);
+    const int n_here = min(64, n_end - n0);
+    const bool idle = GUEST && wave >= nwaves;
+    const int n = n0 + lane;
+    const bool valid = lane < n_here;
+    float* sm_merge = sm;
+#ifdef GMMVI_ME_STAMPS
+    if (threadIdx.x == 0) {
+        g_me_wg[2 * (blockIdx.y * gridDim.x + blockIdx.x)] = wall_clock64();
+        unsigned hw, xcc;
+        asm volatile("s_getreg_b32 %0, hwreg(HW_REG_HW_ID)" : "=s"(hw));
+        asm volatile("s_getreg_b32 %0, hwreg(HW_REG_XCC_ID)" : "=s"(xcc));
+        g_me_hw[blockIdx.y * gridDim.x + blockIdx.x] = ((unsigned long long)xcc << 32) | hw;
+    }
+    unsigned long long stamp[16];
+    int nstamp = 0, nbackward = 0;
+    const long long wc0 = wall_clock64();
+#define ME_STAMP() do { asm volatile("s_waitcnt lgkmcnt(0)" ::: "memory"); if (nstamp < 16) stamp[nstamp++] = __builtin_amdgcn_s_memtime(); } while (0)
+    ME_STAMP();
+#else
+#define ME_STAMP()
+#endif
+
+    const int ldx = D | 1;
+    float x[DP];
+    if (DP % 4 == 0 && D == DP && (reinterpret_cast<uintptr_t>(X) & 15) == 0) {
+        const float4* xrow = reinterpret_cast<const float4*>(X + (size_t)min(n, n_end - 1) * D);
+#pragma unroll
+        for (int q4 = 0; q4 < DP / 4; ++q4) {
+            const float4 v4 = xrow[q4];
+            x[4 * q4] = v4.x; x[4 * q4 + 1] = v4.y; x[4 * q4 + 2] = v4.z; x[4 * q4 + 3] = v4.w;
+        }
+        if (!valid) {
+#pragma unroll
+            for (int i = 0; i < DP; ++i) x[i] = 0.f;
+        }
+    } else if (DP % 2 == 0 && D == DP && (reinterpret_cast<uintptr_t>(X) & 7) == 0) {
+        const float2* xrow = reinterpret_cast<const float2*>(X + (size_t)min(n, n_end - 1) * D);
+#pragma unroll
+        for (int q2 = 0; q2 < DP / 2; ++q2) {
+            const float2 v2 = xrow[q2];
+            x[2 * q2] = v2.x; x[2 * q2 + 1] = v2.y;
+        }
+        if (!valid) {
+#pragma unroll
+            for (int i = 0; i < DP; ++i) x[i] = 0.f;
+        }
+    } else {
+        for (int e = threadIdx.x; e < n_here * D; e += blockDim.x) sm_merge[(e / D) * ldx + (e % D)] = X[(size_t)n0 * D + e];
+        __syncthreads();
+#pragma unroll
+        for (int i = 0; i < DP; ++i) x[i] = (valid && i < D) ? sm_merge[lane * ldx + i] : 0.f;
+        __syncthreads();
+    }
+
+    float m = -3.0e38f, s = 0.f;
+    float m2 = -3.0e38f, s2 = 0.f;
+    const bool dual = logw2 != nullptr;
+    float acc[GRAD ? DP : 1];
+    if (GRAD) {
+#pragma unroll
+        for (int i = 0; i < DP; ++i) acc[i] = 0.f;
+    }
+    const float nud = nu + (float)D;
+    ME_STAMP();
+
+    for (int k = idle ? K : k_lo + wave; k < K; k += nwaves) {
+        ME_STAMP();
+        const sp_block_ptr blk = sp_block(packed + (size_t)k * PK::STRIDE);
+        const float lw = ((sp_const_f32)(uintptr_t)logw)[k];
+        const float lw2 = dual ? ((sp_const_f32)(uintptr_t)logw2)[k] : 0.f;
+        float z[DP], vrd[DP], q, cst;
+        float pc[2][32];
+        SpPass<DP>::forward(blk, x, z, vrd, q, cst, pc);
+        sp_block_ptr blkb = blk;
+        asm volatile("" : "+s"(blkb));
+        if constexpr (GRAD) SpPass<DP>::backward_prefetch(blkb, pc);
+        float ld, coef;
+        if (FAMILY == GMMVI_GAUSS) {
+            ld = fmaf(-0.5f, q, cst);
+            coef = -1.f;
+        } else {
+            ld = cst - 0.5f * nud * log1pf(q / nu);
+            coef = -nud / (nu + q);
+        }
+        const float a = ld + lw;
+        const float mn = fmaxf(m, a);
+        const float sc = __expf(m - mn);
+        const float e = __expf(a - mn);
+        s = fmaf(s, sc, e);
+        m = mn;
+        if (dual) {
+            const float a2 = ld + lw2;
+            const float mn2 = fmaxf(m2, a2);
+            s2 = fmaf(s2, __expf(m2 - mn2), __expf(a2 - mn2));
+            m2 = mn2;
+        }
+        if constexpr (GRAD) {
+            SpPass<DP>::backward(blkb, z, vrd, pc);
+            const float ec = e * coef;
+#pragma unroll
+            for (int i = 0; i < DP; ++i) acc[i] = fmaf(acc[i], sc, ec * z[i]);
+            sp_pin<DP>(acc);
+        }
+        if (ld_out != nullptr && valid) ld_out[(size_t)k * N + n] = ld;
+    }
+    ME_STAMP();
+    if (lp_out == nullptr && !GRAD) return;
+
+    constexpr int NQ = (DP + 3) / 4;
+    float* sm_m = sm_merge;
+    float* sm_s = sm_merge + nwaves * 64;
+    me_f32x4* sm_acc = reinterpret_cast<me_f32x4*>(sm_merge + 2 * nwaves * 64);
+    float* outt = sm_merge + 2 * nwaves * 64 + (GRAD ? (size_t)nwaves * NQ * 256 : 0);
+    float* sm_m2 = outt + (GRAD ? 64 * ldx : 0);
+    float* sm_s2 = sm_m2 + nwaves * 64;
+    if (!idle) {
+        sm_m[wave * 64 + lane] = m;
+        if (dual) sm_m2[wave * 64 + lane] = m2;
+    }
+    ME_LDS_BARRIER();
+    ME_STAMP();
+    float M = -3.0e38f, M2 = -3.0e38f;
+    for (int w = 0; w < nwaves; ++w) M = fmaxf(M, sm_m[w * 64 + lane]);
+    const float f = __expf(m - M);
+    if (!idle) sm_s[wave * 64 + lane] = s * f;
+    if (dual) {
+        for (int w = 0; w < nwaves; ++w) M2 = fmaxf(M2, sm_m2[w * 64 + lane]);
+        if (!idle) sm_s2[wave * 64 + lane] = s2 * __expf(m2 - M2);
+    }
+    if (GRAD && !idle) {
+#pragma unroll
+        for (int q4 = 0; q4 < NQ; ++q4) {
+            me_f32x4 v4;
+#pragma unroll
+            for (int c = 0; c < 4; ++c) v4[c] = 4 * q4 + c < DP ? acc[4 * q4 + c] * f : 0.f;
+            sm_acc[(wave * NQ + q4) * 64 + lane] = v4;
+        }
+    }
+    ME_STAMP();
+    ME_LDS_BARRIER();
+    ME_STAMP();
+    float S = 0.f;
+    for (int w = 0; w < nwaves; ++w) S += sm_s[w * 64 + lane];
+    if (wave == 0 && valid && lp_out != nullptr) lp_out[n] = M + __logf(S);
+    if (dual && wave == (nwaves > 1 ? 1 : 0) && valid && lp2_out != nullptr) {
+        float S2 = 0.f;
+        for (int w = 0; w < nwaves; ++w) S2 += sm_s2[w * 64 + lane];
+        lp2_out[n] = M2 + __logf(S2);
+    }
+    if (GRAD && grad_out != nullptr) {
+        const float inv = 1.f / S;
+        for (int q4 = idle ? NQ : wave; q4 < NQ; q4 += nwaves) {
+            me_f32x4 g4 = {0.f, 0.f, 0.f, 0.f};
+            for (int w = 0; w < nwaves; ++w) g4 += sm_acc[(w * NQ + q4) * 64 + lane];
+#pragma unroll
+            for (int c = 0; c < 4; ++c)
+                if (4 * q4 + c < D) outt[lane * ldx + 4 * q4 + c] = g4[c] * inv;
+        }
+        ME_STAMP();
+        ME_LDS_BARRIER();
+        ME_STAMP();
+        for (int e = threadIdx.x; e < n_here * D; e += blockDim.x)
+            grad_out[(size_t)n0 * D + e] = outt[(e / D) * ldx + (e % D)];
+    }
+#ifdef GMMVI_ME_STAMPS
+    ME_STAMP();
+    if (threadIdx.x == 0) g_me_wg[2 * (blockIdx.y * gridDim.x + blockIdx.x) + 1] = wall_clock64();
+    if (GRAD && logw2 && blockIdx.x == 60 && blockIdx.y == 1 && threadIdx.x == 64 * 3 && (g_me_wg[2 * 8192 - 1]++ & 15) == 12) {
+        const long long wc1 = wall_clock64();
+        printf("me stamps (shader cycles; kernel %lld x 10 ns by the 100 MHz clock):", wc1 - wc0);
+        for (int i = 1; i < nstamp; ++i) printf(" %llu", stamp[i] - stamp[i - 1]);
+        printf("  total %llu, backward passes %d\n", stamp[nstamp - 1] - stamp[0], nbackward);
+    }
+#endif
+}
diff --git a/gmmvi_amd/csrc/stein.hip b/gmmvi_amd/csrc/stein.hip
--- a/gmmvi_amd/csrc/stein.hip
+++ b/gmmvi_amd/csrc/stein.hip
@@ -3,6 +3,7 @@
 #include "wave_reduce.h"
 #include "stein_finalize.h"
 #include "stein_tile.h"
+#include "riders.h"
 #include <cstdlib>
 
 typedef float f32x4 __attribute__((ext_vector_type(4)));
@@ -67,7 +68,8 @@
 void stein_moment_kernel(int K, int D_rt, int N, int wave_range, int stacks, int R, const float* __restrict__ packed,
                          const float* __restrict__ X, const float* __restrict__ TG, const float* __restrict__ QG,
                          const float* __restrict__ ld, const float* __restrict__ bg, const int32_t* __restrict__ mapping,
-                         int map_offset, int own_rt, float* __restrict__ part, float* __restrict__ part_m) {
+                         int map_offset, int own_rt, float* __restrict__ part, float* __restrict__ part_m, Riders riders) {
+    if (riders_carried_prep(riders)) return;
     using ST = SteinTile<DP>;
     constexpr int MT = ST::MT, NT = ST::NT, NB = ST::NB;
     constexpr bool EXACT = VW > 1;
@@ -273,7 +275,7 @@
 template <int DP, int VW>
 static int launch_stein_moment(gmmvi_ctx* ctx, int K, int D, const float* packed, const float* X, int N, const float* ld,
                                const float* qgrad, const float* bg, const float* tgrad, const int32_t* mapping,
-                               int map_offset, int flags, float* H_neg, float* g_neg, SteinSlab* slab_out) {
+                               int map_offset, int flags, float* H_neg, float* g_neg, SteinSlab* slab_out, bool carry_prep) {
     using ST = SteinTile<DP>;
     const int D1 = D + 1;
     const int stacks = (K + ST::NB - 1) / ST::NB;
@@ -301,9 +303,15 @@
             attr = shmem;
         }
         GMMVI_PROF(ctx, "stein_partial");
-        hipLaunchKernelGGL((stein_moment_kernel<DP, VW>), dim3(8 * per_xcd), dim3(256), shmem, ctx->stream, K, D, N, wave_range,
-                           stacks, R, packed, X, tgrad, qgrad, ld, bg, mapping, map_offset,
-                           (flags & GMMVI_OWN_SAMPLES_ONLY) ? 1 : 0, part, part_m);
+        Riders riders;
+        if (carry_prep) {
+            riders = gmmvi_take_pending_riders(ctx, 8 * per_xcd, 256, true);
+            const int free_cus = ctx->num_cus - 8 * per_xcd % ctx->num_cus;
+            if (riders.prep_blocks > free_cus) riders.prep_blocks = free_cus;
+        }
+        hipLaunchKernelGGL((stein_moment_kernel<DP, VW>), dim3(8 * per_xcd + riders.prep_blocks), dim3(256), shmem, ctx->stream, K,
+                           D, N, wave_range, stacks, R, packed, X, tgrad, qgrad, ld, bg, mapping, map_offset,
+                           (flags & GMMVI_OWN_SAMPLES_ONLY) ? 1 : 0, part, part_m, riders);
     }
     GMMVI_LAUNCH_CHECK(ctx);
     if (slab_out != nullptr) {
@@ -315,7 +323,7 @@
 
 static int stein_moment(gmmvi_ctx* ctx, int K, int D, const float* packed, const float* X, int N, const float* ld,
                         const float* qgrad, const float* bg, const float* tgrad, const int32_t* mapping, int map_offset,
-                        int flags, float* H_neg, float* g_neg, SteinSlab* slab_out) {
+                        int flags, float* H_neg, float* g_neg, SteinSlab* slab_out, bool carry_prep = false) {
     const int dp = gmmvi_padded_dim(D);
     const uintptr_t bases = reinterpret_cast<uintptr_t>(X) | reinterpret_cast<uintptr_t>(tgrad) | reinterpret_cast<uintptr_t>(qgrad);
     const int vw_nat = (dp % 4 == 0) ? 4 : 2;
@@ -324,8 +332,8 @@
     case DPV:                                                                                                          \
         if (fast)                                                                                                      \
             return launch_stein_moment<DPV, (DPV % 4 == 0 ? 4 : 2)>(ctx, K, D, packed, X, N, ld, qgrad, bg, tgrad, mapping, \
-                                                                    map_offset, flags, H_neg, g_neg, slab_out);         \
-        return launch_stein_moment<DPV, 1>(ctx, K, D, packed, X, N, ld, qgrad, bg, tgrad, mapping, map_offset, flags, H_neg, g_neg, slab_out)
+                                                                    map_offset, flags, H_neg, g_neg, slab_out, carry_prep); \
+        return launch_stein_moment<DPV, 1>(ctx, K, D, packed, X, N, ld, qgrad, bg, tgrad, mapping, map_offset, flags, H_neg, g_neg, slab_out, carry_prep)
     switch (dp) {
         GMMVI_SM(2); GMMVI_SM(4); GMMVI_SM(8); GMMVI_SM(10); GMMVI_SM(12); GMMVI_SM(16); GMMVI_SM(20); GMMVI_SM(24);
         GMMVI_SM(32); GMMVI_SM(40); GMMVI_SM(50); GMMVI_SM(64);
@@ -351,11 +359,12 @@
 }
 
 int gmmvi_stein_partials(gmmvi_ctx* ctx, int K, int D, const float* packed_dev, const float* X_dev, int N, const float* ld_dev,
-                         const float* qgrad_dev, const float* bg_dev, const float* tgrad_dev, int flags, SteinSlab* slab) {
+                         const float* qgrad_dev, const float* bg_dev, const float* tgrad_dev, int flags, SteinSlab* slab,
+                         bool carry_prep) {
     GMMVI_ARG_CHECK(ctx, K >= 1 && D >= 1 && D < GMMVI_MAX_DIM && !gmmvi_is_blocked_dim(D) && N >= 1 && slab != nullptr);
     GMMVI_ARG_CHECK(ctx, packed_dev && X_dev && qgrad_dev && tgrad_dev && ld_dev && bg_dev && !(flags & GMMVI_OWN_SAMPLES_ONLY));
     return stein_moment(ctx, K, D, packed_dev, X_dev, N, ld_dev, qgrad_dev, bg_dev, tgrad_dev, nullptr, 0, flags, nullptr, nullptr,
-                        slab);
+                        slab, carry_prep);
 }
 
 int gmmvi_stein_finalize_slab(gmmvi_ctx* ctx, int K, int D, const SteinSlab& slab, int N, int flags, const float* packed_dev,
diff --git a/gmmvi_amd/csrc/weights.hip b/gmmvi_amd/csrc/weights.hip
--- a/gmmvi_amd/csrc/weights.hip
+++ b/gmmvi_amd/csrc/weights.hip
@@ -1,5 +1,7 @@
 #include "common.h"
 #include "riders.h"
+#undef GMMVI_ME_STAMPS
+#include "mixture_tile.h"
 #include "stepsize_rules.h"
 #include "wave_reduce.h"
 #include "combine.h"
@@ -110,6 +112,28 @@
 }
 
 template <int DP>
+__device__ __forceinline__ void target_rider(const Riders& r, float* sm) {
+    const TargetJob& t = r.target;
+    const int i = (int)blockIdx.x - r.first_block - r.prep_blocks;
+    if (!t.on || blockIdx.y != 0 || blockIdx.z != 0 || i < 0 || i >= r.sample_blocks) return;
+    const SampleJob& s = r.sample;
+    const int k = i % s.K, chunk = i / s.K;
+    const int begin = s.uniform_count > 0 ? k * s.uniform_count : s.offsets[k];
+    const int end = s.uniform_count > 0 ? begin + s.uniform_count : s.offsets[k + 1];
+    const int base = begin + chunk * 256;
+    const int stop = min(end, base + 256);
+    for (int n0 = base; n0 < stop; n0 += 64) {
+        __syncthreads();
+        if (t.family == GMMVI_GAUSS)
+            me_tile<DP, GMMVI_GAUSS, true, true>(sm, t.nu, 0, t.K, s.D, t.packed, t.logw, s.X, 0, n0, stop, t.nw, nullptr, t.tlp,
+                                                 t.tgrad, nullptr, nullptr);
+        else
+            me_tile<DP, GMMVI_STUDENT_T, true, true>(sm, t.nu, 0, t.K, s.D, t.packed, t.logw, s.X, 0, n0, stop, t.nw, nullptr,
+                                                     t.tlp, t.tgrad, nullptr, nullptr);
+    }
+}
+
+template <int DP>
 __global__ __launch_bounds__(1024) void elr_riders_kernel(int N, const float* __restrict__ ld, const float* __restrict__ bg,
                                                           const float* __restrict__ tlp, const float* __restrict__ logq,
                                                           int logq_R, float beta, const float* __restrict__ logw,
@@ -117,7 +141,10 @@
                                                           float* __restrict__ reward_out, float* __restrict__ ess_out,
                                                           Riders riders) {
     extern __shared__ __align__(16) float sm_riders[];
-    if (riders_carried<DP>(riders, sm_riders)) return;
+    if (riders_carried<DP>(riders, sm_riders)) {
+        if constexpr (DP < GMMVI_MFMA_DENSITY_FROM_DP) target_rider<DP>(riders, sm_riders);
+        return;
+    }
     elr_body(N, ld, bg, tlp, logq, logq_R, beta, logw, self_normalized, E_out, reward_out, ess_out);
 }
 
@@ -326,6 +353,10 @@
     const Riders riders = gmmvi_take_pending_riders(ctx, K, 1024);
     if (riders.prep_blocks + riders.sample_blocks > 0) {
         const int dp = gmmvi_padded_dim(riders.sample_blocks > 0 ? riders.sample.D : 2);
+        if (riders_lds_bytes(riders) > 64 * 1024)
+            GMMVI_DISPATCH_DP(dp, GMMVI_HIP_CHECK(ctx, hipFuncSetAttribute((const void*)elr_riders_kernel<DP>,
+                                                                           hipFuncAttributeMaxDynamicSharedMemorySize,
+                                                                           (int)riders_lds_bytes(riders))));
         GMMVI_DISPATCH_DP(dp, hipLaunchKernelGGL((elr_riders_kernel<DP>), dim3(K + riders.prep_blocks + riders.sample_blocks),
                                                  dim3(1024), riders_lds_bytes(riders), ctx->stream, N, ld_dev, bg_dev, tlp_dev,
                                                  logq_dev, logq_R, beta, logw_dev, self_normalized, E_out_dev, reward_out_dev,
diff --git a/gmmvi_amd/optimization/fused.py b/gmmvi_amd/optimization/fused.py
--- a/gmmvi_amd/optimization/fused.py
+++ b/gmmvi_amd/optimization/fused.py
@@ -36,6 +36,7 @@
         ("weight_update_mode", _i), ("stein_flags", _i), ("presample_next", _i), ("presampled", _i), ("phase", _i),
         ("logreg_A", _p), ("logreg_M", _i), ("logreg_prior_mean", _f), ("logreg_prior_std", _f),
         ("talos_model", _p), ("talos_context", _p),
+        ("early_target_next", _i), ("early_target", _i),
     ]
 
 
@@ -56,6 +57,9 @@
         lib.gmmvi_train_iter_samtron.restype = C.c_int
         lib.gmmvi_train_iter_samtron.argtypes = [C.c_void_p, C.POINTER(SamtronPlan)]
         self._fn = lib.gmmvi_train_iter_samtron
+        lib.gmmvi_samtron_early_target_ok.restype = C.c_int
+        lib.gmmvi_samtron_early_target_ok.argtypes = [C.c_void_p, C.POINTER(SamtronPlan)]
+        self._early_target_ok = lib.gmmvi_samtron_early_target_ok
 
     def _check_static(self):
         g = self.g
@@ -230,7 +234,8 @@
         presample_next = (self.presample and n_old == 0 and sel.reused_samples_per_component == 0
                           and type(g.num_component_adapter) is FixedComponentAdaptation
                           and (db.max_samples is None or db._samples.n + 2 * n <= db.max_samples))
-        for grow, rows in ((db._samples, 2 * n if presample_next else n), (db._target_lnpdfs, n), (db._target_grads, n),
+        for grow, rows in ((db._samples, 2 * n if presample_next else n), (db._target_lnpdfs, 2 * n if presample_next else n),
+                           (db._target_grads, 2 * n if presample_next else n),
                            (db._mapping_dev, 2 * n if presample_next else n), (db._means, k), (db._chols, k), (db._packed, k)):
             grow.reserve(rows)
         s0, c0 = db._samples.n, db._means.n
@@ -268,6 +273,10 @@
         tok, self._presample_token = self._presample_token, None
         p.presampled = int(tok is not None and n_old == 0 and tok[0] == here and tok[1] is model._packed)
         p.presample_next = int(presample_next)
+        target_rows = (db._target_lnpdfs.buf.ptr, db._target_grads.buf.ptr)
+        p.early_target = int(bool(p.presampled) and tok[2] == target_rows)
+        p.early_target_next = 0
+        p.early_target_next = int(presample_next and self._early_target_ok(ctx.handle, C.byref(p)) == 1)
 
         prefetch_next = self.prefetch_counts and sel.reused_samples_per_component > 0
         p.phase = 1 if prefetch_next else 0
@@ -304,7 +313,7 @@
         if presample_next:
             self._presample_token = ((db._samples.buf.ptr, db._mapping_dev.buf.ptr, s0 + n, c0 + k, n, k, key,
                                       int(db._num_samples_written), int(model.seed), model.means.ptr, model.chol_cov.ptr,
-                                      offsets_dev.ptr), packed_new)
+                                      offsets_dev.ptr), packed_new, target_rows if p.early_target_next else None)
         g.ng_based_updater.last_success = success
         g.num_updates.assign_add(1)
         if self._prefetch is not None:
diff --git a/include/gmmvi_hip.h b/include/gmmvi_hip.h
--- a/include/gmmvi_hip.h
+++ b/include/gmmvi_hip.h
@@ -214,8 +214,11 @@
     float logreg_prior_mean, logreg_prior_std;
     const float* talos_model;
     const float* talos_context;
+    int32_t early_target_next, early_target;
 } gmmvi_samtron_plan;
 int gmmvi_train_iter_samtron(gmmvi_ctx* ctx, const gmmvi_samtron_plan* plan);
+int gmmvi_samtron_early_target_ok(gmmvi_ctx* ctx, const gmmvi_samtron_plan* plan);
+int gmmvi_debug_merge_tickets(gmmvi_ctx* ctx, unsigned* out_host, int n);
 
 typedef struct gmmvi_sharded_plan {
     int32_t n_ranks, rank;
```

Result: slower. 3.324 billion samples*components/s (-30.9%).
